# fxxJuses/MICFormer

Measured on AMD Instinct MI355X. Metric: train volumes/sec (128^3 CT+MRI pair), higher is better.
Workload: dtype bf16; 1 GPU; MicFormer base Head(embed_dim=48, depths 2-2-6-2, heads 3-6-12-24, window 2^3, 8 classes) full train step (fwd + MDiceLoss + bwd + Adam/cosine) on 128^3 CT+MR pairs, DropPath on; local_batch=2, global_batch=2, parallelism=dp1, launch=hipGraph replay (one graph)

## Files before the change

include/micformer_hip.h:

```cpp
#ifndef MICFORMER_HIP_H
#define MICFORMER_HIP_H

#include <stddef.h>
#include <stdint.h>

#ifdef __cplusplus
extern "C" {
#endif

typedef void* micf_stream_t;

#define MICF_OK 0
#define MICF_EINVAL (-1)
#define MICF_EUNSUPPORTED (-2)
#define MICF_ELAUNCH (-3)

#define MICF_ABI_VERSION 1

#define MICF_DTYPE_F32 0
#define MICF_DTYPE_BF16 1
#define MICF_DTYPE_BF16_ATTN_FP8 2

int micf_abi_version(void);
const char* micf_strerror(int code);
// ... 137 lines not shown
                            micf_stream_t stream);
int micf_conv_down_bwd_weight(const float* dy, const float* x, float* dw, float* dbias, int B, int D, int H, int W,
                              int C, int N, micf_stream_t stream);
int micf_space_to_depth(const float* x, float* a, int B, int D, int H, int W, int C, int k, int64_t batch_stride,
                        micf_stream_t stream);
int micf_depth_to_space(const float* a, const float* bias, float* y, int B, int D, int H, int W, int C, int k,
                        micf_stream_t stream);
int micf_depth_to_space_add(const float* a, const float* bias, const float* add, float* y, int B, int D, int H, int W, int C,
                            int k, micf_stream_t stream);
int micf_colsum(const float* x, float* out, int64_t M, int N, micf_stream_t stream);
int micf_conv_up_fwd(const float* x, const float* w, const float* bias, float* y, int B, int D, int H, int W, int C,
                     int N, int k, micf_stream_t stream);
int micf_conv_up_bwd_data(const float* dy, const float* w, float* dx, int B, int D, int H, int W, int C, int N, int k,
                          micf_stream_t stream);
int micf_conv_up_bwd_weight(const float* dy, const float* x, float* dw, float* dbias, int B, int D, int H, int W,
                            int C, int N, int k, micf_stream_t stream);

int micf_sw_window(const float* vol, float* win, int C, int D, int H, int W, int rd, int rh, int rw, int z0, int y0, int x0,
                   micf_stream_t stream);
int micf_sw_accumulate(const float* pred, float* out, float* count, int K, int D, int H, int W, int rd, int rh, int rw, int z0,
                       int y0, int x0, micf_stream_t stream);
int micf_sw_normalize(float* out, const float* count, int K, int64_t V, micf_stream_t stream);
int micf_sw_window_batch(const float* vol, float* win, const int32_t* coords, int n, int B, int C, int D, int H, int W, int rd,
                         int rh, int rw, micf_stream_t stream);
int micf_sw_accumulate_batch(const float* pred, float* out, float* count, const int32_t* coords, int n, int B, int K, int D, int H,
                             int W, int rd, int rh, int rw, micf_stream_t stream);

int micf_intensity_stats(const void* vol, int is_half, double* sums, int B, int Cm, int64_t V, micf_stream_t stream);
int micf_patch_rows_prepared(const void* vol, int is_half, const double* sums, const float* params, float* rows0, float* rows1, int B,
                             int Cm, int D, int H, int W, int k, micf_stream_t stream);
int micf_input_prepare(const void* vol, int is_half, const double* sums, const float* params, float* out, const uint8_t* label_in,
                       uint8_t* label_out, int B, int Cm, int D, int H, int W, micf_stream_t stream);

int micf_pad3d(const float* src, float* dst, int B, int D, int H, int W, int Dp, int Hp, int Wp, int C,
               micf_stream_t stream);
int micf_crop3d(const float* src, float* dst, int B, int D, int H, int W, int Dp, int Hp, int Wp, int C,
                int accumulate, micf_stream_t stream);
int micf_resize_trilinear_fwd(const float* src, float* dst, int B, int D, int H, int W, int Do, int Ho, int Wo, int C,
                              micf_stream_t stream);
int micf_resize_trilinear_bwd(const float* ddst, float* dsrc, int B, int D, int H, int W, int Do, int Ho, int Wo,
                              int C, micf_stream_t stream);

int micf_dice_bce_fwd(const float* logits, const float* target, double* sums, float* loss, int B, int K, int64_t V,
                      micf_stream_t stream);
int micf_dice_bce_bwd(const float* logits, const float* target, const double* sums, const float* grad_out,
                      float* dlogits, int B, int K, int64_t V, micf_stream_t stream);
int micf_dice_bce_label_fwd(const float* logits, const uint8_t* label, double* sums, float* loss, int B, int K, int64_t V,
                            micf_stream_t stream);
int micf_dice_bce_label_bwd(const float* logits, const uint8_t* label, const double* sums, const float* grad_out,
                            float* dlogits, int B, int K, int64_t V, micf_stream_t stream);
int micf_argmax_meandice(const float* logits, const uint8_t* label, uint8_t* mask_out, int64_t* counts, double* out,
                         int B, int K, int64_t V, micf_stream_t stream);

int micf_dice_metric(const float* logits, const void* target, int target_is_label, double* sums, float* out, int B, int K,
                     int64_t V, micf_stream_t stream);

int micf_adam_tick(void* state, double base_lr, double eta_min, int64_t t_max, micf_stream_t stream);
int micf_adam_step(float* p, const float* g, float* m, float* v, int64_t n, const void* state, float beta1,
                   float beta2, float eps, float grad_scale, void* p_bf16, micf_stream_t stream);


typedef struct micf_ln_pair_item {
  const float *x, *gamma, *beta;
  float *y, *mean, *rstd;
} micf_ln_pair_item;
typedef struct micf_ln_bwd_pair_item {
  const float *dy, *x, *mean, *rstd, *gamma;
  float *dx, *dgamma, *dbeta;
  const float* add;
  float* partials;
} micf_ln_bwd_pair_item;
int micf_layernorm_fwd_pair(const micf_ln_pair_item* items, int n, int64_t rows, int C, float eps, float* zero,
                            int64_t zero_floats, micf_stream_t stream);
int micf_layernorm_bwd_pair(const micf_ln_bwd_pair_item* items, int n, int64_t rows, int C, micf_stream_t stream);

typedef struct micf_offset_head_group {
  const float* xn;
  const float* xa;
  const float *conv_w, *conv_b;
  float* conv_ws;
  const float *ln_g, *ln_b, *w1;
  float *hid, *flow, *xs;
} micf_offset_head_group;
typedef struct micf_offset_head_bwd_group {
  const float* dxs;
  const float *hid, *flow, *xa, *ln_g, *ln_b, *w1, *conv_w;
  float* conv_ws;
  float* dxa;
  float* dxn;
  float* dhid;
  float *dln_g, *dln_b, *dw1;
} micf_offset_head_bwd_group;
int micf_offset_head_needs_zero(int B, int D, int H, int W, int C);
int micf_offset_head_fwd(const micf_offset_head_group* groups, int ngroups, int B, int D, int H, int W, int C, float eps,
                         int prepared, int hid_zeroed, int dtype, micf_stream_t stream);
int64_t micf_offset_head_bwd_workspace(int ngroups, int B, int D, int H, int W);
int micf_offset_head_bwd(const micf_offset_head_bwd_group* groups, int ngroups, int B, int D, int H, int W, int C, float eps,
                         int prepared, float* workspace, int64_t workspace_floats, int dtype, int defer_finish, micf_stream_t stream);
int micf_offset_head_finish_deferrable(int B, int D, int H, int W);
int micf_offset_head_bwd_finish(const micf_offset_head_bwd_group* groups, int ngroups, int B, int D, int H, int W, int C,
                                float* workspace, int64_t workspace_floats, micf_stream_t stream);
typedef struct micf_offset_head_finish_call {
  const micf_offset_head_bwd_group* groups;
  int32_t ngroups, B, D, H, W, C;
  float* workspace;
  int64_t workspace_floats;
} micf_offset_head_finish_call;
int micf_offset_head_bwd_finish_grouped(const micf_offset_head_finish_call* calls, int ncalls, micf_stream_t stream);

typedef struct micf_block_fwd_group {
  const float* x;
  const float* kvsrc;
  const float *ln1_g, *ln1_b, *bq, *bkv, *bp, *ln2_g, *ln2_b, *b1, *b2;
  const void *wq, *wkv, *wp, *w1, *w2;
  const float *s1, *s2;
  float* y;
  float *xn, *q, *kv, *o, *x1, *xn2;
  void* h;
  float* g;
  float* stats;
  void* kvs16;
  const float* hid;
  const float* samp_src;
  const float *ln16_g, *ln16_b, *w1c;
  float* flow;
  float* xs32;
  const float *nln_g, *nln_b;
  float *nln_y, *nln_mean, *nln_rstd;
  float* zero16;
} micf_block_fwd_group;
int micf_block_fuses_sampler(int C, int heads);
int micf_block_saves_bf16(int C, int heads, int dtype);
typedef struct micf_block_bwd_group {
  const float* dy;
  const float *x, *x1, *stats, *q, *kv;
  const void* h;
  const float *ln1_g, *ln2_g;
  const void *wqt, *wkvt, *wpt, *w1t, *w2t;
  const float *s1, *s2;
  float* dx;
  float* dxs;
  float *dx1, *dh, *dq, *dkv;
  float *ln1_part, *ln2_part;
  float* dx1_copy;
  void* dy16;
  const float* xn2;
  const void* w1;
  const float* b1;
  const float* pre_d;
  const float* pre_x;
  const float *pre_mean, *pre_rstd;
  const float* pre_g;
  float* pre_part;
} micf_block_bwd_group;
int micf_block_recomputes_h(int C, int heads);
int micf_block_tile_tokens(int B, int D, int H, int W, int C, int heads, int hidden, int backward);
int micf_block_fwd_persistent_probe(const micf_block_fwd_group* groups, int ngroups, int B, int D, int H, int W, int C, int heads,
                                    int hidden, float eps, float scale, int dtype, int repeats, int* sync_ws, micf_stream_t stream);
int micf_probe_mfma_chain(const void* a, const void* b, const void* c, const void* d, float* out, int form, micf_stream_t stream);
typedef struct micf_weight_prep_item {
  const float* src;
  void* dst;
  void* dst_t;
  int32_t rows, cols, bf16 , reserved;
} micf_weight_prep_item;
int micf_weight_prep_grouped(const micf_weight_prep_item* items, int n, micf_stream_t stream);
int micf_block_fwd(const micf_block_fwd_group* groups, int ngroups, int B, int D, int H, int W, int C, int heads,
                   int hidden, float eps, float scale, int dtype, micf_stream_t stream);
int micf_block_bwd(const micf_block_bwd_group* groups, int ngroups, int B, int D, int H, int W, int C, int heads,
                   int hidden, float scale, int dtype, micf_stream_t stream);

int micf_zero(void* p, int64_t bytes, micf_stream_t stream);
int micf_drop_path_draw(void* rng, const float* keep, float* out, int n, int B, micf_stream_t stream);


int micf_grad_wire_pack(const float* src, int64_t n, void* dst, int64_t padded, micf_stream_t stream);
int micf_grad_wire_sum(const void* recv, int ranks, int64_t shard, void* out, micf_stream_t stream);
int micf_grad_wire_unpack(const void* src, float* dst, int64_t n, micf_stream_t stream);

#ifdef __cplusplus
}
#endif
#endif
```

micformer_amd/_lib.py:

```python
import ctypes
import os

_PKT = "DEBUG_CLR_GRAPH_PACKET_CAPTURE"
_pkt_before = os.environ.get(_PKT)
if os.environ.get("MICF_SEGMENTED", "0") == "1":
    os.environ.setdefault(_PKT, "0")

import torch

GRAPH_SEGMENTS_OK = os.environ.get(_PKT) == "0" and (_pkt_before == "0" or not torch.cuda.is_initialized())

_HERE = os.path.dirname(os.path.abspath(__file__))
LIB_PATH = os.environ.get("MICF_LIB") or os.path.join(_HERE, "libmicformer_hip.so")

_P, _I, _L, _F, _D = ctypes.c_void_p, ctypes.c_int, ctypes.c_int64, ctypes.c_float, ctypes.c_double
_T = {"p": _P, "i": _I, "l": _L, "f": _F, "d": _D}

SIGNATURES = {
    "micf_layernorm_fwd": "ppippppplifp",
    "micf_layernorm_bwd": "pppippppppplippp",
    "micf_layernorm_bwd_partial_rows": "lii",
    "micf_layernorm_bwd_finish": "pip",
    "micf_linear_fwd": "ppipppplppliiiip",
    "micf_linear_bwd_data": "pplppppiiliiip",
    "micf_linear_bwd_weight": "pplppiippliiplip",
    "micf_linear_bwd_weight_workspace": "lii",
    "micf_linear_bwd_weight_grouped": "piplip",
    "micf_linear_bwd_weight_grouped_workspace": "pi",
    "micf_head_tail_compose": "pppppiiiipp",
    "micf_head_tail_col2im": "pppiiiiiip",
    "micf_head_tail_im2col": "ppiiiiiip",
    "micf_head_tail_col2im_sw": "pppppiiiiiiiiiip",
    "micf_head_tail_decompose": "pppppppppiiiipp",
    "micf_head_tail_fused_supported": "iiiiiii",
    "micf_head_tail_pack_bytes": "ii",
    "micf_head_tail_pack": "pppppiiip",
    "micf_head_tail_fwd_fused": "pppiiiiiiip",
    "micf_head_tail_fwd_fused_sw": "pppppiiiiiiiiiiip",
    "micf_head_tail_loss_parts": "iiii",
    "micf_head_tail_fwd_loss_fused": "ppppipppiiiiiiip",
    "micf_head_tail_bwd_data_fused": "pppiiiiiiip",
    "micf_head_tail_bwd_weight_fused": "pppppliiiiiiip",
    "micf_head_tail_bwd_weight_fused_workspace": "iiiii",
    "micf_sw_window": "ppiiiiiiiiiip",
    "micf_sw_accumulate": "pppiiiiiiiiiip",
    "micf_sw_normalize": "ppilp",
    "micf_window_attn_fwd": "pippipiiiiiiiiiifp",
    "micf_window_attn_fwd_fp8": "pippipiiiiiiiiiifp",
    "micf_window_attn_bwd": "pippipipippiiiiiiiiiifp",
    "micf_conv3_fwd": "pipipppiiiiiipliip",
    "micf_conv3_fwd_workspace": "iii",
    "micf_conv3_bwd_data": "pippiipiiiiiiipliip",
    "micf_conv3_weight_prep_grouped": "pip",
    "micf_layernorm_fwd_pair": "pilifplp",
    "micf_layernorm_bwd_pair": "pilip",
    "micf_offset_head_needs_zero": "iiiii",
    "micf_offset_head_fwd": "piiiiiifiiip",
    "micf_offset_head_bwd_workspace": "iiiii",
    "micf_offset_head_bwd": "piiiiiifipliip",
    "micf_offset_head_finish_deferrable": "iiii",
    "micf_offset_head_bwd_finish": "piiiiiiplp",
    "micf_offset_head_bwd_finish_grouped": "pip",
    "micf_conv3_bwd_data_workspace": "iii",
    "micf_conv3_bwd_weight": "pipipippiiiiiplip",
    "micf_conv3_bwd_weight_workspace": "iiiiiii",
    "micf_conv3_bwd_weight_grouped": "piiiiiiiiplip",
    "micf_conv3_bwd_weight_grouped_workspace": "iiiiiiii",
    "micf_offset_sample_fwd": "pppppppiiiiifp",
    "micf_offset_sample_bwd": "ppppppppppppiiiiifplp",
    "micf_offset_sample_bwd_workspace": "iiii",
    "micf_stn_fwd": "pppiiiiip",
    "micf_stn_bwd": "pppppiiiiip",
    "micf_patch_embed_fwd": "piipppiiiiiip",
    "micf_patch_embed_bwd_weight": "ppiippiiiiiip",
    "micf_conv_down_fwd": "ppppiiiiiip",
    "micf_conv_down_bwd_data": "pppiiiiiip",
    "micf_conv_down_bwd_weight": "ppppiiiiiip",
    "micf_conv_up_fwd": "ppppiiiiiiip",
    "micf_conv_up_bwd_data": "pppiiiiiiip",
    "micf_conv_up_bwd_weight": "ppppiiiiiiip",
    "micf_space_to_depth": "ppiiiiiilp",
    "micf_depth_to_space": "pppiiiiiip",
    "micf_depth_to_space_add": "ppppiiiiiip",
    "micf_colsum": "pplip",
    "micf_pad3d": "ppiiiiiiiip",
    "micf_crop3d": "ppiiiiiiiiip",
    "micf_resize_trilinear_fwd": "ppiiiiiiiip",
    "micf_resize_trilinear_bwd": "ppiiiiiiiip",
    "micf_dice_bce_fwd": "ppppiilp",
    "micf_dice_bce_bwd": "pppppiilp",
    "micf_dice_bce_label_fwd": "ppppiilp",
    "micf_dice_bce_label_bwd": "pppppiilp",
    "micf_argmax_meandice": "pppppiilp",
    "micf_adam_tick": "pddlp",
    "micf_adam_step": "pppplpffffpp",
    "micf_block_tile_tokens": "iiiiiiii",
    "micf_block_saves_bf16": "iii",
    "micf_block_fuses_sampler": "ii",
    "micf_block_recomputes_h": "ii",
    "micf_weight_prep_grouped": "pip",
    "micf_grad_wire_pack": "plplp",
    "micf_grad_wire_sum": "pilpp",
    "micf_grad_wire_unpack": "pplp",
    "micf_block_fwd": "piiiiiiiiffip",
    "micf_block_bwd": "piiiiiiiifip",
    "micf_block_fwd_persistent_probe": "piiiiiiiiffiipp",
    "micf_probe_mfma_chain": "pppppip",
    "micf_dice_metric": "ppippiilp",
    "micf_sw_window_batch": "pppiiiiiiiiip",
    "micf_sw_accumulate_batch": "ppppiiiiiiiiip",
    "micf_intensity_stats": "pipiilp",
    "micf_input_prepare": "pipppppiiiiip",
    "micf_patch_rows_prepared": "pippppiiiiiip",
    "micf_zero": "plp",
    "micf_drop_path_draw": "pppiip",
}


class WgradItem(ctypes.Structure):
    _fields_ = [("a", ctypes.c_void_p), ("dy", ctypes.c_void_p), ("dp_scale", ctypes.c_void_p), ("dw", ctypes.c_void_p),
                ("dbias", ctypes.c_void_p), ("M", ctypes.c_int64), ("rows_per_sample", ctypes.c_int64),
                ("N", ctypes.c_int32), ("K", ctypes.c_int32), ("operand_dtype", ctypes.c_int32), ("ldw", ctypes.c_int32)]


class Conv3WgradItem(ctypes.Structure):
    _fields_ = [("dy", ctypes.c_void_p), ("x1", ctypes.c_void_p), ("x2", ctypes.c_void_p), ("dw", ctypes.c_void_p),
                ("dbias", ctypes.c_void_p)]


class LnFinishItem(ctypes.Structure):
    _fields_ = [("partials", ctypes.c_void_p), ("dgamma", ctypes.c_void_p), ("dbeta", ctypes.c_void_p),
                ("blocks", ctypes.c_int32), ("C", ctypes.c_int32)]


_VP = ctypes.c_void_p


class BlockFwdGroup(ctypes.Structure):
    FIELDS = ("x", "kvsrc", "ln1_g", "ln1_b", "bq", "bkv", "bp", "ln2_g", "ln2_b", "b1", "b2", "wq", "wkv", "wp", "w1", "w2",
              "s1", "s2", "y", "xn", "q", "kv", "o", "x1", "xn2", "h", "g", "stats", "kvs16", "hid", "samp_src", "ln16_g", "ln16_b", "w1c", "flow", "xs32",
              "nln_g", "nln_b", "nln_y", "nln_mean", "nln_rstd", "zero16")
    _fields_ = [(n, _VP) for n in FIELDS]


class BlockBwdGroup(ctypes.Structure):
    FIELDS = ("dy", "x", "x1", "stats", "q", "kv", "h", "ln1_g", "ln2_g", "wqt", "wkvt", "wpt", "w1t", "w2t", "s1", "s2",
              "dx", "dxs", "dx1", "dh", "dq", "dkv", "ln1_part", "ln2_part", "dx1_copy", "dy16", "xn2", "w1", "b1",
              "pre_d", "pre_x", "pre_mean", "pre_rstd", "pre_g", "pre_part")
    _fields_ = [(n, _VP) for n in FIELDS]


class WeightPrepItem(ctypes.Structure):
    _fields_ = [("src", _VP), ("dst", _VP), ("dst_t", _VP), ("rows", ctypes.c_int32), ("cols", ctypes.c_int32),
                ("bf16", ctypes.c_int32), ("reserved", ctypes.c_int32)]


class LnPairItem(ctypes.Structure):
    FIELDS = ("x", "gamma", "beta", "y", "mean", "rstd")
    _fields_ = [(n, _VP) for n in FIELDS]


class LnBwdPairItem(ctypes.Structure):
    FIELDS = ("dy", "x", "mean", "rstd", "gamma", "dx", "dgamma", "dbeta", "add", "partials")
    _fields_ = [(n, _VP) for n in FIELDS]


class OffsetHeadGroup(ctypes.Structure):
    FIELDS = ("xn", "xa", "conv_w", "conv_b", "conv_ws", "ln_g", "ln_b", "w1", "hid", "flow", "xs")
    _fields_ = [(n, _VP) for n in FIELDS]


class OffsetHeadBwdGroup(ctypes.Structure):
    FIELDS = ("dxs", "hid", "flow", "xa", "ln_g", "ln_b", "w1", "conv_w", "conv_ws", "dxa", "dxn", "dhid", "dln_g", "dln_b", "dw1")
    _fields_ = [(n, _VP) for n in FIELDS]


class OffsetHeadFinishCall(ctypes.Structure):
    _fields_ = [("groups", _VP), ("ngroups", ctypes.c_int32), ("B", ctypes.c_int32), ("D", ctypes.c_int32), ("H", ctypes.c_int32),
                ("W", ctypes.c_int32), ("C", ctypes.c_int32), ("workspace", _VP), ("workspace_floats", ctypes.c_int64)]


class Conv3PrepItem(ctypes.Structure):
    _fields_ = [("w", _VP), ("fwd", _VP), ("bwd", _VP), ("N", ctypes.c_int32), ("Cin", ctypes.c_int32)]


class MicfError(RuntimeError):
    pass


def _load():
    if not os.path.exists(LIB_PATH):
        raise ImportError(
            f"{LIB_PATH} not found: build it with `python micformer_amd/build.py` (hipcc, gfx950). "
            "micformer_amd has no CPU / PyTorch fallback path.")
    lib = ctypes.CDLL(LIB_PATH)
    for name, sig in SIGNATURES.items():
        fn = getattr(lib, name)
        fn.argtypes = [_T[c] for c in sig]
        fn.restype = _I
    lib.micf_linear_bwd_weight_workspace.restype = _L
    lib.micf_linear_bwd_weight_grouped_workspace.restype = _L
    lib.micf_conv3_bwd_data_workspace.restype = _L
    lib.micf_offset_sample_bwd_workspace.restype = _L
    lib.micf_conv3_bwd_weight_workspace.restype = _L
    lib.micf_conv3_bwd_weight_grouped_workspace.restype = _L
    lib.micf_head_tail_pack_bytes.restype = _L
    lib.micf_head_tail_loss_parts.restype = _L
    lib.micf_head_tail_loss_parts.argtypes = [_I] * 4
    lib.micf_head_tail_bwd_weight_fused_workspace.restype = _L
    lib.micf_conv3_fwd_workspace.restype = _L
    lib.micf_offset_head_bwd_workspace.restype = _L
    lib.micf_block_tile_tokens.argtypes = [_I] * 8
    lib.micf_block_saves_bf16.argtypes = [_I] * 3
    lib.micf_offset_head_finish_deferrable.argtypes = [_I] * 4
    lib.micf_block_fuses_sampler.argtypes = [_I] * 2
    lib.micf_block_recomputes_h.argtypes = [_I] * 2
    lib.micf_strerror.argtypes = [_I]
    lib.micf_strerror.restype = ctypes.c_char_p
    lib.micf_set_option.argtypes = [ctypes.c_char_p, _I]
    lib.micf_set_option.restype = _I
    lib.micf_get_option.argtypes = [ctypes.c_char_p, ctypes.POINTER(_I)]
    lib.micf_get_option.restype = _I
    lib.micf_abi_version.argtypes = []
    lib.micf_abi_version.restype = _I
    if lib.micf_abi_version() != 1:
        raise ImportError("libmicformer_hip.so ABI version mismatch")
    return lib


lib = _load()


def get_option(name):
    v = _I(0)
    if lib.micf_get_option(name.encode(), ctypes.byref(v)) != 0:
        raise KeyError(f"unknown micformer option {name!r}")
    return v.value


def set_option(name, value):
    prev = get_option(name)
    if lib.micf_set_option(name.encode(), int(value)) != 0:
        raise KeyError(f"unknown micformer option {name!r}")
    return prev


class option:

    def __init__(self, name, value):
        self.name, self.value = name, value

    def __enter__(self):
        self.prev = set_option(self.name, self.value)

    def __exit__(self, *exc):
        set_option(self.name, self.prev)
        return False


def ptr(t):
    if t is None:
        return None
    if not t.is_cuda:
        raise MicfError("micformer_amd ops need CUDA (ROCm) tensors: there is no CPU path")
    if not t.is_contiguous():
        raise MicfError("micformer_amd ops need contiguous tensors")
    return t.data_ptr()


_raw_stream = getattr(torch._C, "_cuda_getCurrentRawStream", None)
_cur_device = getattr(torch._C, "_cuda_getDevice", None)


def stream():
    if _raw_stream is not None and _cur_device is not None:
        return _raw_stream(_cur_device())
    return torch.cuda.current_stream().cuda_stream


PROFILE = None
BLOCK_DEPTH = 0
UNIT = None


def set_unit(kind, groups, tokens, channels):
    global UNIT
    if PROFILE is not None:
        UNIT = f"{kind}|{groups}x{tokens}x{channels}"


class block_region:

    def __enter__(self):
        global BLOCK_DEPTH
        BLOCK_DEPTH += 1

    def __exit__(self, *exc):
        global BLOCK_DEPTH, UNIT
        BLOCK_DEPTH -= 1
        if BLOCK_DEPTH == 0:
            UNIT = None
# ... 58 lines not shown
```

micformer_amd/csrc/block_bwd.hip:

```cpp
#include "block_fused.h"
#include "attn_fp8.h"

namespace micf {

struct BlkBwdArgs {
  micf_block_bwd_group g[2];
  TileGeo geo;
  int G, tiles, C, heads, hidden;
  float scale;
  int attn_mfma;
};

template <int TM, int NW, int X4>
struct RowRegs {
  static constexpr int RPP = 4 * NW, NPASS = (TM + RPP - 1) / RPP, K = (X4 + 15) / 16;
  float4 v[NPASS][K];
  template <class Addr>
  __device__ __forceinline__ void load(const int* tok, int tk0, const Addr addr) {
    const int lane = threadIdx.x & 63, wave = threadIdx.x >> 6, l16 = lane & 15, rg = lane >> 4;
#pragma unroll
    for (int pass = 0; pass < NPASS; ++pass) {
      const int row = pass * RPP + wave * 4 + rg;
      const int tk = row < TM ? tok[row] : -1;
#pragma unroll
      for (int k = 0; k < K; ++k) {
        const int c4 = l16 + 16 * k;
        const bool ok = tk >= 0 && c4 < X4;
        const float4 t = ld4g(addr(tk >= 0 ? (uint32_t)(tk - tk0) : 0u, (uint32_t)(c4 < X4 ? c4 : X4 - 1)));
        v[pass][k] = ok ? t : make_float4(0.f, 0.f, 0.f, 0.f);
      }
    }
  }
  __device__ __forceinline__ void commit(float* dst, int stride) const {
    const int lane = threadIdx.x & 63, wave = threadIdx.x >> 6, l16 = lane & 15, rg = lane >> 4;
#pragma unroll
    for (int pass = 0; pass < NPASS; ++pass) {
      const int row = pass * RPP + wave * 4 + rg;
      if (row >= TM) continue;
#pragma unroll
      for (int k = 0; k < K; ++k) {
        const int c4 = l16 + 16 * k;
        if (c4 < X4) *reinterpret_cast<float4*>(dst + row * stride + 4 * c4) = v[pass][k];
      }
    }
  }
  __device__ __forceinline__ void store_b16(const int* tok, int tk0, void* base) const {
    const int lane = threadIdx.x & 63, wave = threadIdx.x >> 6, l16 = lane & 15, rg = lane >> 4;
#pragma unroll
    for (int pass = 0; pass < NPASS; ++pass) {
      const int row = pass * RPP + wave * 4 + rg;
      const int tk = row < TM ? tok[row] : -1;
      if (tk < 0) continue;
#pragma unroll
      for (int k = 0; k < K; ++k) {
        const int c4 = l16 + 16 * k;
        if (c4 < X4) st_h4_32<true>(base, (uint32_t)(tk - tk0) * (4 * X4) + 4 * c4, v[pass][k]);
      }
    }
  }
};
template <int TM, int NW, int X4, bool BF16>
struct HRegs {
  static constexpr int RPP = 4 * NW, NPASS = (TM + RPP - 1) / RPP, K = (X4 + 15) / 16, ES = BF16 ? 2 : 4;
  using V = typename std::conditional<BF16, uint2, float4>::type;
  V v[NPASS][K];
  __device__ __forceinline__ void load(const int* tok, int tk0, const char* base, uint32_t ld) {
    const int lane = threadIdx.x & 63, wave = threadIdx.x >> 6, l16 = lane & 15, rg = lane >> 4;
#pragma unroll
    for (int pass = 0; pass < NPASS; ++pass) {
      const int row = pass * RPP + wave * 4 + rg;
      const int tk = row < TM ? tok[row] : -1;
      const uint32_t rel = tk >= 0 ? (uint32_t)(tk - tk0) : 0u;
#pragma unroll
      for (int k = 0; k < K; ++k) {
        const int c4 = l16 + 16 * k;
        const bool ok = tk >= 0 && c4 < X4;
        const V t = *reinterpret_cast<const V*>(base + (rel * ld + 4u * (uint32_t)(c4 < X4 ? c4 : X4 - 1)) * (uint32_t)ES);
        v[pass][k] = ok ? t : V{};
      }
    }
  }
  __device__ __forceinline__ void commit(float* dst, int stride) const {
    const int lane = threadIdx.x & 63, wave = threadIdx.x >> 6, l16 = lane & 15, rg = lane >> 4;
#pragma unroll
    for (int pass = 0; pass < NPASS; ++pass) {
      const int row = pass * RPP + wave * 4 + rg;
      if (row >= TM) continue;
#pragma unroll
      for (int k = 0; k < K; ++k) {
        const int c4 = l16 + 16 * k;
        if (c4 >= X4) continue;
        float4 f;
        if constexpr (BF16) f = unpack4_bf16(v[pass][k]); else f = v[pass][k];
        *reinterpret_cast<float4*>(dst + row * stride + 4 * c4) = f;
      }
    }
  }
};
template <int TM, int NW, int C>
struct LnRegs {
  RowRegs<TM, NW, C / 4> x;
  float mu[RowRegs<TM, NW, C / 4>::NPASS], rs[RowRegs<TM, NW, C / 4>::NPASS];
  float4 gm[(C + 63) / 64];
  __device__ __forceinline__ void load(const int* tok, int tk0, const float* __restrict__ xsrc, const float* __restrict__ mean,
                                       const float* __restrict__ rstd, const float* __restrict__ gamma) {
    constexpr int RPP = 4 * NW, NPASS = RowRegs<TM, NW, C / 4>::NPASS;
    const int lane = threadIdx.x & 63, wave = threadIdx.x >> 6, l16 = lane & 15, rg = lane >> 4;
    x.load(tok, tk0, [&](uint32_t rel, uint32_t c4) { return at32(xsrc, (rel * C + 4 * c4) * 4u); });
#pragma unroll
    for (int pass = 0; pass < NPASS; ++pass) {
      const int row = pass * RPP + wave * 4 + rg;
      const int tk = row < TM ? tok[row] : -1;
      const uint32_t rel = tk >= 0 ? (uint32_t)(tk - tk0) : 0u;
      const float m = *at32(mean, rel * 4u), r = *at32(rstd, rel * 4u);
      mu[pass] = tk >= 0 ? m : 0.f; rs[pass] = tk >= 0 ? r : 0.f;
    }
#pragma unroll
    for (int k = 0; k < (C + 63) / 64; ++k) {
      const int c4 = l16 + 16 * k;
      const float4 t = ld4g(gamma + 4 * (c4 < C / 4 ? c4 : C / 4 - 1));
      gm[k] = c4 < C / 4 ? t : make_float4(0.f, 0.f, 0.f, 0.f);
    }
  }
  __device__ __forceinline__ void park(float* stash) const {
    constexpr int NPASS = RowRegs<TM, NW, C / 4>::NPASS;
    x.commit(stash, C);
    float* mine = stash + TM * C + threadIdx.x;
#pragma unroll
    for (int pass = 0; pass < NPASS; ++pass) { mine[(2 * pass) * 64 * NW] = mu[pass]; mine[(2 * pass + 1) * 64 * NW] = rs[pass]; }
  }
  __device__ __forceinline__ void unpark(const float* stash, const float* __restrict__ gamma) {
    constexpr int RPP = 4 * NW, NPASS = RowRegs<TM, NW, C / 4>::NPASS, K = RowRegs<TM, NW, C / 4>::K;
    const int lane = threadIdx.x & 63, wave = threadIdx.x >> 6, l16 = lane & 15, rg = lane >> 4;
    const float* mine = stash + TM * C + threadIdx.x;
#pragma unroll
    for (int pass = 0; pass < NPASS; ++pass) {
      const int row = pass * RPP + wave * 4 + rg;
      mu[pass] = mine[(2 * pass) * 64 * NW]; rs[pass] = mine[(2 * pass + 1) * 64 * NW];
#pragma unroll
      for (int k = 0; k < K; ++k) {
        const int c4 = l16 + 16 * k;
        x.v[pass][k] = (row < TM && c4 < C / 4) ? *reinterpret_cast<const float4*>(stash + row * C + 4 * c4) : make_float4(0.f, 0.f, 0.f, 0.f);
      }
    }
#pragma unroll
    for (int k = 0; k < (C + 63) / 64; ++k) {
      const int c4 = l16 + 16 * k;
      const float4 t = ld4g(gamma + 4 * (c4 < C / 4 ? c4 : C / 4 - 1));
      gm[k] = c4 < C / 4 ? t : make_float4(0.f, 0.f, 0.f, 0.f);
    }
  }
};

template <int TJ, int VPL, int NW, int C, bool H16 = false>
__device__ __forceinline__ void ln_bwd_tile(const float* D, float* A, int S, const LnRegs<16 * TJ, NW, C>& in, const int* tok,
                                            int tk0, void* __restrict__ hout, float* __restrict__ hout2, float* scratch,
                                            float* __restrict__ part) {
  constexpr int TM = 16 * TJ, NTHR = 64 * NW, RPP = 4 * NW, NPASS = (TM + RPP - 1) / RPP, NPR = RPP < TM ? RPP : TM;
  const int tid = threadIdx.x, lane = tid & 63, wave = tid >> 6, l16 = lane & 15, rg = lane >> 4;
  constexpr int C4 = C >> 2;
  const float invC = 1.0f / (float)C;
  float4 ag[VPL], ab[VPL], gm[VPL];
#pragma unroll
// ... 302 lines not shown
          const float ds = p[j] * (dp[j] - dot);
          if (j / (8 / SP) == sub) {
            PS[pair * 16 + j] = p[j];
            PS[pair * 16 + 8 + j] = ds;
          }
          const float* kp = U + (r0 + j) * SU + C + hoff;
          const float dss = ds * a.scale;
#pragma unroll
          for (int d = 0; d < HP; d += 4) {
            const float4 t = *reinterpret_cast<const float4*>(kp + d);
            dq[d] += dss * t.x; dq[d + 1] += dss * t.y; dq[d + 2] += dss * t.z; dq[d + 3] += dss * t.w;
          }
        }
      }
      lds_barrier();
      if (active) {
#pragma unroll
        for (int d = 0; d < HP; ++d) { dk[d] = 0.f; dv[d] = 0.f; }
        const int base = pair - i * heads;
#pragma unroll
        for (int m = 0; m < 8; ++m) {
          const float pm = PS[(base + m * heads) * 16 + i];
          const float dsm = PS[(base + m * heads) * 16 + 8 + i] * a.scale;
          const float* qp = U + (r0 + m) * SU + hoff;
          const float* dop = A2 + (r0 + m) * S + hoff;
#pragma unroll
          for (int d = 0; d < HP; d += 4) {
            const float4 t = *reinterpret_cast<const float4*>(qp + d);
            dk[d] += dsm * t.x; dk[d + 1] += dsm * t.y; dk[d + 2] += dsm * t.z; dk[d + 3] += dsm * t.w;
            const float4 u = *reinterpret_cast<const float4*>(dop + d);
            dv[d] += pm * u.x; dv[d + 1] += pm * u.y; dv[d + 2] += pm * u.z; dv[d + 3] += pm * u.w;
          }
        }
      }
      lds_barrier();
      if (active) {
#pragma unroll
        for (int d = 0; d < HP; d += 4) {
          *reinterpret_cast<float4*>(U + row * SU + hoff + d) = make_float4(dq[d], dq[d + 1], dq[d + 2], dq[d + 3]);
          *reinterpret_cast<float4*>(U + row * SU + C + hoff + d) = make_float4(dk[d], dk[d + 1], dk[d + 2], dk[d + 3]);
          *reinterpret_cast<float4*>(U + row * SU + 2 * C + hoff + d) = make_float4(dv[d], dv[d + 1], dv[d + 2], dv[d + 3]);
        }
      }
      lds_barrier();
    }
  }

#pragma unroll 1
  for (int pass = 0; pass < NPASS; ++pass) {
    const int row = pass * RPP + wave * 4 + rg;
    if (row >= TM) continue;
    const int tk = tok[row];
    if (tk < 0) continue;
    const uint32_t rel = (uint32_t)(tk - tk0);
    for (int c4 = l16; c4 < 3 * C4; c4 += 16) {
      const float4 v = *reinterpret_cast<const float4*>(U + row * SU + 4 * c4);
      if (c4 < C4) st_h4_32<BF16>(dq0, rel * C + 4 * c4, v);
      else st_h4_32<BF16>(dkv0, rel * 2 * C + 4 * (c4 - C4), v);
    }
  }

  if (!g.dxs) {
    if (PARK) r_ln1.unpark(stash, g.ln1_g);
    gemm_phase<TJ, NSLK, NKK, C, NW, BF16>(wqt, C, U, nullptr, 0, nullptr, SU, A2, S, EpiStore{});
    gemm_phase<TJ, NSLK, 2 * NKK, 2 * C, NW, BF16>(wkvt, C, U + C, nullptr, 0, nullptr, SU, A2, S, EpiAcc{});
    ln_bwd_tile<TJ, VPL, NW, C>(A2, A1, S, r_ln1, tok, tk0, dx0, nullptr, U, g.ln1_part ? g.ln1_part + (int64_t)tile * 2 * C : nullptr);
  } else {
    gemm_phase<TJ, NSLK, NKK, C, NW, BF16>(wqt, C, U, nullptr, 0, nullptr, SU, A2, S, EpiStore{});
#pragma unroll 1
    for (int pass = 0; pass < NPASS; ++pass) {
      const int row = pass * RPP + wave * 4 + rg;
      if (row >= TM) continue;
      const int tk = tok[row];
      if (tk < 0) continue;
      for (int c4 = l16; c4 < C4; c4 += 16)
        st4g(at32(dx0, ((uint32_t)(tk - tk0) * C + 4 * c4) * 4u), *reinterpret_cast<const float4*>(A2 + row * S + 4 * c4));
    }
    lds_barrier();
    gemm_phase<TJ, NSLK, 2 * NKK, 2 * C, NW, BF16>(wkvt, C, U + C, nullptr, 0, nullptr, SU, A2, S, EpiStore{});
#pragma unroll 1
    for (int pass = 0; pass < NPASS; ++pass) {
      const int row = pass * RPP + wave * 4 + rg;
      if (row >= TM) continue;
      const int tk = tok[row];
      if (tk < 0) continue;
      for (int c4 = l16; c4 < C4; c4 += 16)
        st4g(at32(g.dxs + (int64_t)tk0 * C, ((uint32_t)(tk - tk0) * C + 4 * c4) * 4u), *reinterpret_cast<const float4*>(A2 + row * S + 4 * c4));
    }
  }
}

template <int C, int HD, int TJ>
static int launch_bwd(const BlkBwdArgs& a, int dtype, hipStream_t s) {
  constexpr int TM = 16 * TJ, NW = C >= 192 ? 8 : 4;
  const bool recomp = a.g[0].h == nullptr;
  const size_t lds = block_lds_floats(TM, C, block_bwd_scratch_floats(TM, C / HD, 64 * NW),
                                      block_bwd_park_floats(TM, C, 64 * NW) + (recomp ? 4 * C : 0)) * sizeof(float);
  if (lds > 160 * 1024) return MICF_EUNSUPPORTED;
  const unsigned grid = a.G == 2 ? (unsigned)((a.tiles + 3) / 4 * 8) : (unsigned)a.tiles;
  static std::once_flag once;
  std::call_once(once, [] {
    (void)hipFuncSetAttribute(reinterpret_cast<const void*>(&block_bwd_kernel<C, HD, TJ, NW, true, false>), hipFuncAttributeMaxDynamicSharedMemorySize, 160 * 1024);
    (void)hipFuncSetAttribute(reinterpret_cast<const void*>(&block_bwd_kernel<C, HD, TJ, NW, false, false>), hipFuncAttributeMaxDynamicSharedMemorySize, 160 * 1024);
    (void)hipFuncSetAttribute(reinterpret_cast<const void*>(&block_bwd_kernel<C, HD, TJ, NW, true, true>), hipFuncAttributeMaxDynamicSharedMemorySize, 160 * 1024);
    (void)hipFuncSetAttribute(reinterpret_cast<const void*>(&block_bwd_kernel<C, HD, TJ, NW, false, true>), hipFuncAttributeMaxDynamicSharedMemorySize, 160 * 1024);
  });
  if (dtype == MICF_DTYPE_BF16) {
    if (recomp) hipLaunchKernelGGL((block_bwd_kernel<C, HD, TJ, NW, true, true>), dim3(grid), dim3(64 * NW), lds, s, a);
    else hipLaunchKernelGGL((block_bwd_kernel<C, HD, TJ, NW, true, false>), dim3(grid), dim3(64 * NW), lds, s, a);
  } else {
    if (recomp) hipLaunchKernelGGL((block_bwd_kernel<C, HD, TJ, NW, false, true>), dim3(grid), dim3(64 * NW), lds, s, a);
    else hipLaunchKernelGGL((block_bwd_kernel<C, HD, TJ, NW, false, false>), dim3(grid), dim3(64 * NW), lds, s, a);
  }
  MICF_RETURN_LAUNCH();
}

}

#include "block_wave_bwd.h"

using namespace micf;

extern "C" int micf_block_bwd(const micf_block_bwd_group* groups, int ngroups, int B, int D, int H, int W, int C, int heads,
                              int hidden, float scale, int dtype, micf_stream_t stream) {
  if (!groups || ngroups < 1 || ngroups > 2) return MICF_EINVAL;
  const int TM = micf_block_tile_tokens(B, D, H, W, C, heads, hidden, 1);
  if (TM == 0) return MICF_EUNSUPPORTED;
  if (dtype != MICF_DTYPE_F32 && dtype != MICF_DTYPE_BF16) return MICF_EINVAL;
  BlkBwdArgs a;
  for (int i = 0; i < ngroups; ++i) {
    const micf_block_bwd_group& g = groups[i];
    const void* need[] = {g.dy, g.x1, g.stats, g.q, g.kv, g.ln2_g, g.wqt, g.wkvt, g.wpt, g.w1t, g.w2t, g.dx, g.dx1, g.dh, g.dq, g.dkv};
    for (const void* p : need)
      if (!p || (reinterpret_cast<uintptr_t>(p) & 15)) return MICF_EINVAL;
    if (g.h) {
      if (reinterpret_cast<uintptr_t>(g.h) & 15) return MICF_EINVAL;
    } else {
      const void* re[] = {g.xn2, g.w1, g.b1};
      for (const void* p : re)
        if (!p || (reinterpret_cast<uintptr_t>(p) & 15)) return MICF_EINVAL;
      if (!micf_block_recomputes_h(C, heads)) return MICF_EINVAL;
    }
    if (i > 0 && (g.h == nullptr) != (groups[0].h == nullptr)) return MICF_EINVAL;
    if (g.pre_d) {
      const void* pr[] = {g.pre_d, g.pre_x, g.pre_mean, g.pre_rstd, g.pre_g, g.pre_part, g.dy16};
      for (const void* p : pr)
        if (!p || (reinterpret_cast<uintptr_t>(p) & 15)) return MICF_EINVAL;
      if (g.dxs || dtype != MICF_DTYPE_BF16 || block_wide_tile_tokens(C, C / heads)) return MICF_EINVAL;
    }
    if (!g.dxs && (!g.x || !g.ln1_g)) return MICF_EINVAL;
    const void* opt[] = {g.x, g.ln1_g, g.dxs, g.ln1_part, g.ln2_part, g.dx1_copy, g.dy16};
    for (const void* p : opt)
      if (p && (reinterpret_cast<uintptr_t>(p) & 15)) return MICF_EINVAL;
    a.g[i] = g;
  }
  if (ngroups == 1) a.g[1] = a.g[0];
  a.geo = make_tile_geo(B, D, H, W);
  a.G = ngroups; a.C = C; a.heads = heads; a.hidden = hidden; a.scale = scale;
  a.tiles = (a.geo.nwin + TM / 8 - 1) / (TM / 8);
  a.attn_mfma = dtype == MICF_DTYPE_BF16 ? 1 : 0;
  hipStream_t s = (hipStream_t)stream;
  const int hd = C / heads, tj = TM / 16;
  if ((int64_t)2 * H * W * (TM / 8 + 1) * hidden * (int64_t)sizeof(float) >= (int64_t)1 << 32) return MICF_EUNSUPPORTED;
  if (block_wide_tile_tokens(C, hd)) return block_bwd_wide(groups, ngroups, B, D, H, W, C, heads, scale, dtype, s);
  {
    if (options().block_wave != 0 && C == 48 && hd == 16 && tj == 2 && dtype == MICF_DTYPE_BF16 && a.attn_mfma && a.g[0].h && a.g[1].h && (a.g[0].dxs != nullptr) == (a.g[1].dxs != nullptr) &&
        (a.g[0].pre_d != nullptr) == (a.g[1].pre_d != nullptr) && !(a.g[0].dxs && a.g[0].pre_d) &&
        a.geo.T * (int64_t)hidden * 2 < ((int64_t)1 << 31))
    {
      if (options().block_debug & 1) a.attn_mfma |= 2;
      return wave48::launch_bwd_wave48(a, s);
    }
  }
#define MICF_BB(C_, HD_, TJ_) if (C == C_ && hd == HD_ && tj == TJ_) return launch_bwd<C_, HD_, TJ_>(a, dtype, s)
  MICF_BB(48, 16, 2); MICF_BB(96, 16, 2); MICF_BB(192, 16, 1);
  MICF_BB(96, 32, 1); MICF_BB(192, 32, 1); MICF_BB(384, 32, 1);
#undef MICF_BB
  return MICF_EUNSUPPORTED;
}
```

micformer_amd/csrc/block_wave_bwd.h:

```cpp
#pragma once

#include "block_wave.h"

namespace micf {
namespace wave48 {

constexpr int kB2 = 0;
constexpr int kB2h = kB2 + 12 * 1024;
constexpr int kB1 = kB2h + 12 * 512;
constexpr int kBP = kB1 + 18 * 1024;
constexpr int kBPh = kBP + 3 * 1024;
constexpr int kBQ = kBPh + 3 * 512;
constexpr int kBKV = kBQ + 9 * 512;
constexpr int kBVec = kBKV + 18 * 512;
constexpr int kBPark = kBVec + 3 * C * 4;
constexpr int kParkFloats = 4 * (16 * 12 + 8);
constexpr int kBwdLdsBytes = kBPark + NWAVE * kParkFloats * 4;

__device__ __forceinline__ void stage_weights_bwd(char* lds, const micf_block_bwd_group& g) {
  const uint16_t* wqt = static_cast<const uint16_t*>(g.wqt), *wkvt = static_cast<const uint16_t*>(g.wkvt), *wpt = static_cast<const uint16_t*>(g.wpt),
                 *w1t = static_cast<const uint16_t*>(g.w1t), *w2t = static_cast<const uint16_t*>(g.w2t);
  const int tid = threadIdx.x;
  for (int s = tid; s < 12 * 64; s += NTHR) {
    const int j = s >> 6, li = s & 15, lr = (s >> 4) & 3, row = row_p192(j, li);
    *reinterpret_cast<u32x4v*>(lds + kB2 + s * 16) = *reinterpret_cast<const u32x4v*>(w2t + k16(row, 8 * lr, 3));
    *reinterpret_cast<u32x2v*>(lds + kB2h + s * 8) = *reinterpret_cast<const u32x2v*>(w2t + k16(row, 32 + 4 * lr, 3));
  }
  for (int s = tid; s < 18 * 64; s += NTHR) {
    const int f = s >> 6, j = f / 6, kc = f - 6 * j, li = s & 15, lr = (s >> 4) & 3;
    *reinterpret_cast<u32x4v*>(lds + kB1 + s * 16) = *reinterpret_cast<const u32x4v*>(w1t + k16(row_p48(j, li), 32 * kc + 8 * lr, 12));
  }
  for (int s = tid; s < 3 * 64; s += NTHR) {
    const int j = s >> 6, li = s & 15, lr = (s >> 4) & 3, row = 16 * j + li;
    *reinterpret_cast<u32x4v*>(lds + kBP + s * 16) = *reinterpret_cast<const u32x4v*>(wpt + k16(row, 8 * lr, 3));
    *reinterpret_cast<u32x2v*>(lds + kBPh + s * 8) = *reinterpret_cast<const u32x2v*>(wpt + k16(row, 32 + 4 * lr, 3));
  }
  for (int s = tid; s < 9 * 64; s += NTHR) {
    const int f = s >> 6, j = f / 3, h = f - 3 * j, li = s & 15, lr = (s >> 4) & 3;
    *reinterpret_cast<u32x2v*>(lds + kBQ + s * 8) = *reinterpret_cast<const u32x2v*>(wqt + k16(row_p48(j, li), 16 * h + 4 * lr, 3));
  }
  for (int s = tid; s < 18 * 64; s += NTHR) {
    const int f = s >> 6, j = f / 6, h = f - 6 * j, li = s & 15, lr = (s >> 4) & 3;
    *reinterpret_cast<u32x2v*>(lds + kBKV + s * 8) = *reinterpret_cast<const u32x2v*>(wkvt + k16(row_p48(j, li), 16 * h + 4 * lr, 6));
  }
  float* PV = reinterpret_cast<float*>(lds + kBVec);
  for (int e = tid; e < 3 * C; e += NTHR) {
    const float* src = e < C ? g.ln1_g : (e < 2 * C ? g.ln2_g : g.pre_g);
    PV[e] = src ? src[e % C] : 0.f;
  }
}

__device__ __forceinline__ void park12(float* tile, int lr, int li, const float (&v)[12]) {
  float* p = tile + lr * 200 + li * 12;
  *reinterpret_cast<float4*>(p) = make_float4(v[0], v[1], v[2], v[3]);
  *reinterpret_cast<float4*>(p + 4) = make_float4(v[4], v[5], v[6], v[7]);
  *reinterpret_cast<float4*>(p + 8) = make_float4(v[8], v[9], v[10], v[11]);
}
__device__ __forceinline__ void unpark12(const float* tile, int lr, int li, float (&v)[12]) {
  const float* p = tile + lr * 200 + li * 12;
  const float4 a = *reinterpret_cast<const float4*>(p), b = *reinterpret_cast<const float4*>(p + 4), c = *reinterpret_cast<const float4*>(p + 8);
  v[0] = a.x; v[1] = a.y; v[2] = a.z; v[3] = a.w; v[4] = b.x; v[5] = b.y; v[6] = b.z; v[7] = b.w; v[8] = c.x; v[9] = c.y; v[10] = c.z; v[11] = c.w;
}
__device__ __forceinline__ float colsum16(const float* tile, int lane) {
  const int c = lane < 48 ? lane : 0;
  const float* p = tile + (c < 32 ? (c >> 3) * 200 + (c & 7) : ((c - 32) >> 2) * 200 + 8 + (c & 3));
  float s0 = 0.f, s1 = 0.f;
#pragma unroll
  for (int t = 0; t < 16; t += 2) { s0 += p[12 * t]; s1 += p[12 * t + 12]; }
  return s0 + s1;
}

__device__ __forceinline__ void ln_bwd12(const float (&d)[12], const Row12& xin, float mu, float rs, const float* gam, int lr, int li,
                                         int lane, float* tile, const Row12& add, Row12& out, float& pg, float& pb) {
  float gm[12], dxh[12];
  vec12(gam, lr, gm);
  float sa = 0.f, sb = 0.f;
#pragma unroll
  for (int e = 0; e < 12; e += 4) {
    float g4[4], xh[4];
#pragma unroll
    for (int r = 0; r < 4; ++r) { xh[r] = (xin.v[e + r] - mu) * rs; g4[r] = gm[e + r] * d[e + r]; dxh[e + r] = d[e + r] * xh[r]; }
    sa += (g4[0] + g4[1]) + (g4[2] + g4[3]);
    sb += (g4[0] * xh[0] + g4[1] * xh[1]) + (g4[2] * xh[2] + g4[3] * xh[3]);
  }
  const float Am = sum4(sa) * (1.0f / C), Bm = sum4(sb) * (1.0f / C);
  park12(tile, lr, li, dxh);
#pragma unroll
  for (int e = 0; e < 12; ++e) out.v[e] = add.v[e] + rs * (gm[e] * d[e] - Am - ((xin.v[e] - mu) * rs) * Bm);
  pg += colsum16(tile, lane);
  asm volatile("" : "+v"(pg));
  park12(tile, lr, li, d);
  pb += colsum16(tile, lane);
  asm volatile("" : "+v"(pb));
}

__device__ __forceinline__ void unpack8(const u32x4v& u, float (&o)[8]) {
#pragma unroll
  for (int w = 0; w < 4; ++w) { o[2 * w] = __uint_as_float(u[w] << 16); o[2 * w + 1] = __uint_as_float(u[w] & 0xFFFF0000u); }
}

template <bool CROSS, bool PRE>
__global__ void __launch_bounds__(NTHR) __attribute__((amdgpu_waves_per_eu(4, 4))) block_bwd_wave48_kernel(const BlkBwdArgs a) {
  extern __shared__ __attribute__((aligned(1024))) char wlds[];
  const unsigned bid = blockIdx.x;
  int grp, wg, nwg;
  if (a.G == 2) { const int xcd = bid & 7; grp = xcd >> 2; wg = (int)(bid >> 3) * 4 + (xcd & 3); nwg = (int)(gridDim.x >> 3) * 4; }
  else { grp = 0; wg = bid; nwg = gridDim.x; }
  const micf_block_bwd_group& g = a.g[grp];
  stage_weights_bwd(wlds, g);
  const int tid = threadIdx.x, lane0 = tid & 63, wave = __builtin_amdgcn_readfirstlane(tid >> 6);
  const float* PV = reinterpret_cast<const float*>(wlds + kBVec);
  const float *p_ln1g = PV, *p_ln2g = PV + C, *p_preg = PV + 2 * C;
  const uint32_t T = (uint32_t)a.geo.T;
  const int ngroup16 = (a.geo.nwin + 1) >> 1;
  constexpr bool cross = CROSS, pre = PRE;
  const f32x4 z4 = {0.f, 0.f, 0.f, 0.f};
  lds_barrier();

  for (int unit = wg * NWAVE + wave; unit < a.tiles; unit += nwg * NWAVE) {
    float pg_pre = 0.f, pb_pre = 0.f, pg2 = 0.f, pb2 = 0.f, pg1 = 0.f, pb1 = 0.f;
#pragma unroll 1
    for (int sub = 0; sub < 2; ++sub) {
      const int gt = 2 * unit + sub;
      if (gt >= ngroup16) break;
      asm volatile("" ::: "memory");
      int lane = lane0;
      asm volatile("" : "+v"(lane));
      const int li = lane & 15, lr = lane >> 4;
      const bf16x4_t ident = pack4_bf16v(4 * lr == li ? 1.f : 0.f, 4 * lr + 1 == li ? 1.f : 0.f, 4 * lr + 2 == li ? 1.f : 0.f, 4 * lr + 3 == li ? 1.f : 0.f);
      const bool valid = (lr >> 1) == (li >> 3);
      float* tile = reinterpret_cast<float*>(wlds + kBPark) + wave * kParkFloats;
      const int win = 2 * gt + (li >> 3);
      const bool live0 = win < a.geo.nwin, live = live0 && !(a.attn_mfma & 2);
      int b = 0, d_ = 0, hh = 0, w = 0;
      a.geo.coords(live0 ? win : 0, li & 7, b, d_, hh, w);
      const uint32_t tk = (uint32_t)(((b * a.geo.D + d_) * a.geo.H + hh) * a.geo.W + w);
      const float s1v = g.s1 ? g.s1[b] : 1.f, s2v = g.s2 ? g.s2[b] : 1.f;
      const uint32_t rowC = tk * C;

      Row12 dy;
      dy.load(at32(g.dy, rowC * 4u), lr);
      if (!live) dy.zero();
      if (pre) {
        Row12 pd, px;
        pd.load(at32(g.pre_d, rowC * 4u), lr);
        px.load(at32(g.pre_x, rowC * 4u), lr);
        float pm = *at32(g.pre_mean, tk * 4u), pr = *at32(g.pre_rstd, tk * 4u);
        if (!live) { pd.zero(); px.zero(); pm = 0.f; pr = 0.f; }
        Row12 t;
        ln_bwd12(pd.v, px, pm, pr, p_preg, lr, li, lane, tile, dy, t, pg_pre, pb_pre);
        dy = t;
        if (!live) dy.zero();
      }
      const bf16x8 dyA = dy.lo();
      const bf16x4_t dyB = dy.hi();
      park12(tile, lr, li, dy.v);
      u32x4v hreg[6];
      {
        const uint16_t* hp = static_cast<const uint16_t*>(g.h);
#pragma unroll
        for (int c = 0; c < 6; ++c) {
          hreg[c] = *reinterpret_cast<const u32x4v*>(at32(hp, (tk * HID + 32 * c + 8 * lr) * 2u));
          if (!live) hreg[c] = u32x4v{0u, 0u, 0u, 0u};
        }
      }

      f32x4 dn2[3] = {z4, z4, z4};
      bf16x8 dhs[6];
      {
#pragma unroll
        for (int c = 0; c < 6; ++c) {
          float h8[8];
          unpack8(hreg[c], h8);
          float4 dv[2];
#pragma unroll
          for (int u = 0; u < 2; ++u) {
            const int j = 2 * c + u;
            const f32x4 acc = mfma48(frag32(wlds, kB2, j, lane), frag16(wlds, kB2h, j, lane), dyA, dyB);
            dv[u] = make_float4(s2v * acc[0] * gelu_grad_t<true>(h8[4 * u]), s2v * acc[1] * gelu_grad_t<true>(h8[4 * u + 1]),
                                s2v * acc[2] * gelu_grad_t<true>(h8[4 * u + 2]), s2v * acc[3] * gelu_grad_t<true>(h8[4 * u + 3]));
          }
          dhs[c] = to_bf16x8(dv[0], dv[1]);
#pragma unroll
          for (int j = 0; j < 3; ++j) dn2[j] = mfma32(frag32(wlds, kB1, 6 * j + c, lane), dhs[c], dn2[j]);
          __builtin_amdgcn_sched_barrier(0);
        }
      }
      const uint16_t* qp = reinterpret_cast<const uint16_t*>(g.q);
      const uint16_t* kp = reinterpret_cast<const uint16_t*>(g.kv);
      bf16x4_t qn, kn, vn;
      auto load_head = [&](int h) {
        qn = *reinterpret_cast<const bf16x4_t*>(at32(qp, (rowC + 16 * h + 4 * lr) * 2u));
        kn = *reinterpret_cast<const bf16x4_t*>(at32(kp, (2 * rowC + 16 * h + 4 * lr) * 2u));
        vn = *reinterpret_cast<const bf16x4_t*>(at32(kp, (2 * rowC + C + 16 * h + 4 * lr) * 2u));
        if (!live) { qn = bf16x4_t{0, 0, 0, 0}; kn = qn; vn = qn; }
      };
      load_head(0);
      Row12 x1;
      x1.load(at32(g.x1, rowC * 4u), lr);
      float mu2 = *at32(g.stats, (2 * T + tk) * 4u), rs2 = *at32(g.stats, (3 * T + tk) * 4u);
      if (!live) { x1.zero(); mu2 = 0.f; rs2 = 0.f; }
      Row12 x;
      float mu1 = 0.f, rs1 = 0.f;

      asm volatile("" ::: "memory");
      if (live) {
        if (g.dy16) {
          uint16_t* o = static_cast<uint16_t*>(g.dy16);
          st4u(at32(o, (rowC + 8 * lr) * 2u), dyA); st2u(at32(o, (rowC + 32 + 4 * lr) * 2u), dyB);
        }
        uint16_t* dho = reinterpret_cast<uint16_t*>(g.dh);
#pragma unroll
        for (int c = 0; c < 6; ++c) st4u(at32(dho, (tk * HID + 32 * c + 8 * lr) * 2u), dhs[c]);
      }

      __builtin_amdgcn_sched_barrier(0);
      Row12 dx1;
      {
        float d[12];
#pragma unroll
        for (int j = 0; j < 3; ++j)
#pragma unroll
          for (int r = 0; r < 4; ++r) d[4 * j + r] = dn2[j][r];
        Row12 dyp;
        unpark12(tile, lr, li, dyp.v);
        ln_bwd12(d, x1, mu2, rs2, p_ln2g, lr, li, lane, tile, dyp, dx1, pg2, pb2);
        if (!live) dx1.zero();
      }
      const bf16x8 d1A = dx1.lo();
      const bf16x4_t d1B = dx1.hi();
      if (live) {
        uint16_t* o = reinterpret_cast<uint16_t*>(g.dx1);
        st4u(at32(o, (rowC + 8 * lr) * 2u), d1A); st2u(at32(o, (rowC + 32 + 4 * lr) * 2u), d1B);
        if (g.dx1_copy) dx1.store(at32(g.dx1_copy, rowC * 4u), lr);
      }

      bf16x4_t dqf[3], dkf[3], dvf[3];
      {
        uint16_t* dqo = reinterpret_cast<uint16_t*>(g.dq);
        uint16_t* dko = reinterpret_cast<uint16_t*>(g.dkv);
#pragma unroll
        for (int h = 0; h < 3; ++h) {
          const bf16x4_t qcur = qn, kf = kn, vf = vn;
          if (h < 2) load_head(h + 1);
          else if (!cross) {
            x.load(at32(g.x, rowC * 4u), lr);
            mu1 = *at32(g.stats, tk * 4u); rs1 = *at32(g.stats, (T + tk) * 4u);
            if (!live) { x.zero(); mu1 = 0.f; rs1 = 0.f; }
          }
          const f32x4 dacc = mfma48(frag32(wlds, kBP, h, lane), frag16(wlds, kBPh, h, lane), d1A, d1B);
          const bf16x4_t of = pack4_bf16v(s1v * dacc[0], s1v * dacc[1], s1v * dacc[2], s1v * dacc[3]);
          const uint2 qu = __builtin_bit_cast(uint2, qcur);
          const bf16x4_t qf = pack4_bf16v(__uint_as_float(qu.x << 16) * a.scale, __uint_as_float(qu.x & 0xFFFF0000u) * a.scale,
                                          __uint_as_float(qu.y << 16) * a.scale, __uint_as_float(qu.y & 0xFFFF0000u) * a.scale);
          const f32x4 s1 = mfma16(kf, qf, z4);
          const f32x4 p1 = mfma16(vf, of, z4);
          const f32x4 s2 = mfma16(qf, kf, z4);
          const f32x4 p2 = mfma16(of, vf, z4);
          float m = valid ? fmaxf(fmaxf(s1[0], s1[1]), fmaxf(s1[2], s1[3])) : -INFINITY;
          m = fmaxf(m, __shfl_xor(m, 16, 64));
          float e[4];
#pragma unroll
          for (int r = 0; r < 4; ++r) e[r] = valid ? expf(s1[r] - m) : 0.f;
          float sum = (e[0] + e[1]) + (e[2] + e[3]);
          sum += __shfl_xor(sum, 16, 64);
          const float inv = valid ? 1.0f / sum : 0.f;
          float dot = 0.f;
#pragma unroll
          for (int r = 0; r < 4; ++r) { e[r] *= inv; dot += valid ? e[r] * p1[r] : 0.f; }
          dot += __shfl_xor(dot, 16, 64);
          float ds1[4];
#pragma unroll
          for (int r = 0; r < 4; ++r) ds1[r] = valid ? e[r] * (p1[r] - dot) : 0.f;
          const bf16x4_t dsf1 = pack4_bf16v(ds1[0], ds1[1], ds1[2], ds1[3]);
          float e2[4], ds2[4];
#pragma unroll
          for (int r = 0; r < 4; ++r) {
            const int qi = 4 * lr + r, src = qi + 16 * (2 * (qi >> 3));
            const float mq = __shfl(m, src, 64), iq = __shfl(inv, src, 64), dq_ = __shfl(dot, src, 64);
            e2[r] = valid ? expf(s2[r] - mq) * iq : 0.f;
            ds2[r] = valid ? e2[r] * (p2[r] - dq_) : 0.f;
          }
          const bf16x4_t pf2 = pack4_bf16v(e2[0], e2[1], e2[2], e2[3]);
          const bf16x4_t dsf2 = pack4_bf16v(ds2[0], ds2[1], ds2[2], ds2[3]);
          const bf16x4_t kt = pack4q(mfma16(kf, ident, z4)), qt = pack4q(mfma16(qf, ident, z4)), ot = pack4q(mfma16(of, ident, z4));
          const f32x4 ga = mfma16(kt, dsf1, z4);
          const f32x4 gb = mfma16(qt, dsf2, z4);
          const f32x4 gc = mfma16(ot, pf2, z4);
          dqf[h] = pack4_bf16v(ga[0] * a.scale, ga[1] * a.scale, ga[2] * a.scale, ga[3] * a.scale);
          dkf[h] = pack4q(gb);
          dvf[h] = pack4q(gc);
          if (live) {
            st2u(at32(dqo, (rowC + 16 * h + 4 * lr) * 2u), dqf[h]);
            st2u(at32(dko, (2 * rowC + 16 * h + 4 * lr) * 2u), dkf[h]);
            st2u(at32(dko, (2 * rowC + C + 16 * h + 4 * lr) * 2u), dvf[h]);
          }
          __builtin_amdgcn_sched_barrier(0);
        }
      }

      __builtin_amdgcn_sched_barrier(0);
      if (!cross) {
        float d[12];
#pragma unroll
        for (int j = 0; j < 3; ++j) {
          f32x4 acc = z4;
#pragma unroll
          for (int h = 0; h < 3; ++h) acc = mfma16(frag16(wlds, kBQ, 3 * j + h, lane), dqf[h], acc);
#pragma unroll
          for (int h = 0; h < 6; ++h) acc = mfma16(frag16(wlds, kBKV, 6 * j + h, lane), h < 3 ? dkf[h] : dvf[h - 3], acc);
#pragma unroll
          for (int r = 0; r < 4; ++r) d[4 * j + r] = acc[r];
        }
        Row12 dx;
        ln_bwd12(d, x, mu1, rs1, p_ln1g, lr, li, lane, tile, dx1, dx, pg1, pb1);
        if (live) dx.store(at32(g.dx, rowC * 4u), lr);
      } else {
        Row12 dxq, dxs;
#pragma unroll
        for (int j = 0; j < 3; ++j) {
          f32x4 acc = z4, acs = z4;
#pragma unroll
          for (int h = 0; h < 3; ++h) acc = mfma16(frag16(wlds, kBQ, 3 * j + h, lane), dqf[h], acc);
#pragma unroll
          for (int h = 0; h < 6; ++h) acs = mfma16(frag16(wlds, kBKV, 6 * j + h, lane), h < 3 ? dkf[h] : dvf[h - 3], acs);
#pragma unroll
          for (int r = 0; r < 4; ++r) { dxq.v[4 * j + r] = acc[r]; dxs.v[4 * j + r] = acs[r]; }
        }
        if (live) {
          dxq.store(at32(g.dx, rowC * 4u), lr);
          dxs.store(at32(g.dxs, rowC * 4u), lr);
        }
      }
    }
    if (lane0 < C) {
      const int64_t row = (int64_t)unit * 2 * C;
      if (g.ln2_part) { g.ln2_part[row + lane0] = pg2; g.ln2_part[row + C + lane0] = pb2; }
      if (!cross && g.ln1_part) { g.ln1_part[row + lane0] = pg1; g.ln1_part[row + C + lane0] = pb1; }
      if (pre) { g.pre_part[row + lane0] = pg_pre; g.pre_part[row + C + lane0] = pb_pre; }
    }
  }
}

static int launch_bwd_wave48(const BlkBwdArgs& a, hipStream_t s) {
  int nwg = (a.tiles + NWAVE - 1) / NWAVE;
  if (nwg > 256) nwg = 256;
  const unsigned grid = a.G == 2 ? (unsigned)((nwg + 3) / 4 * 8) : (unsigned)nwg;
  static std::once_flag once;
  std::call_once(once, [] {
    (void)hipFuncSetAttribute(reinterpret_cast<const void*>(&block_bwd_wave48_kernel<true, false>), hipFuncAttributeMaxDynamicSharedMemorySize, 160 * 1024);
    (void)hipFuncSetAttribute(reinterpret_cast<const void*>(&block_bwd_wave48_kernel<false, true>), hipFuncAttributeMaxDynamicSharedMemorySize, 160 * 1024);
    (void)hipFuncSetAttribute(reinterpret_cast<const void*>(&block_bwd_wave48_kernel<false, false>), hipFuncAttributeMaxDynamicSharedMemorySize, 160 * 1024);
  });
  const bool cross = a.g[0].dxs != nullptr, pre = a.g[0].pre_d != nullptr;
  if (cross) hipLaunchKernelGGL((block_bwd_wave48_kernel<true, false>), dim3(grid), dim3(NTHR), kBwdLdsBytes, s, a);
  else if (pre) hipLaunchKernelGGL((block_bwd_wave48_kernel<false, true>), dim3(grid), dim3(NTHR), kBwdLdsBytes, s, a);
  else hipLaunchKernelGGL((block_bwd_wave48_kernel<false, false>), dim3(grid), dim3(NTHR), kBwdLdsBytes, s, a);
  MICF_RETURN_LAUNCH();
}

}
}
```

micformer_amd/csrc/common.h:

```cpp
#pragma once
#include <hip/hip_runtime.h>
#include <stdint.h>

#include "../../include/micformer_hip.h"
#include "gemm_core.h"

#define MICF_RETURN_LAUNCH()                          \
  do {                                                \
    return hipGetLastError() == hipSuccess ? MICF_OK : MICF_ELAUNCH; \
  } while (0)

namespace micf {

struct Options {
  int block_wave = 1;
  int block_recompute_h = 0;
  int block_debug = 0;
  int sample_tile = 1;
  int sample_e = -1;
  int cell_cap = -1;
  int tile_cap_hits = -1, tile_cap_cell = -1, tile_cap_voxel = -1;
};
Options& options();

struct Geo {
  int B, D, H, W;
  FastDiv fW, fH, fD;
  Geo() {}
  Geo(int B_, int D_, int H_, int W_) : B(B_), D(D_), H(H_), W(W_), fW((uint32_t)W_), fH((uint32_t)H_), fD((uint32_t)D_) {}
  __host__ __device__ int64_t tokens() const { return (int64_t)B * D * H * W; }
  __device__ __forceinline__ void decode(int t, int& b, int& d, int& h, int& w) const {
    uint32_t q, r;
    fW.divmod((uint32_t)t, q, r); w = (int)r;
    fH.divmod(q, q, r); h = (int)r;
    fD.divmod(q, q, r); d = (int)r; b = (int)q;
  }
  __device__ __forceinline__ int token(int b, int d, int h, int w) const { return ((b * D + d) * H + h) * W + w; }
};

__device__ __forceinline__ float wave_sum(float v) {
#pragma unroll
  for (int o = 32; o > 0; o >>= 1) v += __shfl_xor(v, o, 64);
  return v;
}

int colsum_atomic(const float* dy, const float* scale, int64_t rps, float* out, int64_t M, int N, hipStream_t s);

constexpr int kOffsetHidden = 16;
struct CellLists {
  int* count;
  int* ovf_count;
  int* list;
  int* ovf;
  int cap;
  float* w8;
};
struct SampleFwdSet { const float *h, *ln_g, *ln_b, *w1, *xa; float *flow, *xs; };
struct SampleBwdSet {
  const float *dxs, *h, *ln_g, *ln_b, *w1, *xa, *flow;
  float *dxa, *dh, *dln_g, *dln_b, *dw1;
  CellLists cl;
  float* partials;
};
int offset_sample_fwd_groups(const SampleFwdSet* sets, int n, int B, int D, int H, int W, int C, float eps, hipStream_t stream);
int offset_sample_bwd_groups(SampleBwdSet* sets, int n, int B, int D, int H, int W, int C, float eps, float* workspace,
                             int64_t workspace_floats, hipStream_t s, int phase = 0);
struct SampleFinishCall { const SampleBwdSet* sets; int n, B, D, H, W, C; float* workspace; int64_t workspace_floats; };
int offset_sample_finish_many(const SampleFinishCall* calls, int ncalls, hipStream_t s);

struct Conv3FwdSet { const float* x1; const float* x2; const float* w; const float* bias; float* y; float* wt; };
struct Conv3BwdSet { const float* dy; const float* w; float* wt; float* dx1; float* dx2; };
int conv3_fwd_x_groups(const Conv3FwdSet* sets, int n, int c1, int c2, int B, int D, int H, int W, int N, hipStream_t stream, int dtype,
                       int prepared, int y_zeroed);
bool conv3_fwd_x_splits(int B, int D, int H, int W, int c1, int c2);
int conv3_bwd_data_x_groups(const Conv3BwdSet* sets, int ng, int c1, int acc1, int c2, int acc2, int B, int D, int H, int W, int N,
                            hipStream_t stream, int dtype, int prepared);

int conv3_bwd_data_x(const float* dy, const float* w, float* wt, float* dx1, int c1, int acc1, float* dx2, int c2, int acc2, int B,
                     int D, int H, int W, int N, hipStream_t stream, int dtype = 0, int prepared = 0);

int64_t conv3_fwdx_workspace(int N, int c1, int c2);
int conv3_fwd_x(const float* x1, int c1, const float* x2, int c2, const float* w, const float* bias, float* y, float* wt, int B, int D,
                int H, int W, int N, hipStream_t stream, int dtype = 0, int prepared = 0);
int64_t conv3_wgradx_workspace(int B, int D, int H, int W, int N, int c1, int c2, int items = 1);
int conv3_wgradx_items(const float* const* dy, const float* const* x1, const float* const* x2, float* const* dw, float* const* dbias,
                       int n, int c1, int c2, int B, int D, int H, int W, int N, float* ws, int64_t ws_floats, hipStream_t stream,
                       int dtype);
int conv3_wgradx(const float* dy, const float* x1, int c1, const float* x2, int c2, float* dw, float* dbias, int B, int D, int H,
                 int W, int N, float* ws, int64_t ws_floats, hipStream_t stream, int dtype = 0);

}
```

micformer_amd/csrc/misc.hip:

```cpp
#include <hip/hip_fp16.h>

#include "common.h"
#include <string.h>

namespace micf {

__global__ void __launch_bounds__(256) pad3d_kernel(const float* __restrict__ src, float* __restrict__ dst, int B, int D, int H,
                                                    int W, int Dp, int Hp, int Wp, int C, int64_t total) {
  for (int64_t i = (int64_t)blockIdx.x * 256 + threadIdx.x; i < total; i += (int64_t)gridDim.x * 256) {
    int64_t t = i / C; const int c = (int)(i - t * C);
    const int w = (int)(t % Wp); t /= Wp; const int h = (int)(t % Hp); t /= Hp; const int d = (int)(t % Dp); const int b = (int)(t / Dp);
    dst[i] = (d < D && h < H && w < W) ? src[((((int64_t)b * D + d) * H + h) * W + w) * C + c] : 0.f;
  }
}
__global__ void __launch_bounds__(256) crop3d_kernel(const float* __restrict__ src, float* __restrict__ dst, int B, int D, int H,
                                                     int W, int Dp, int Hp, int Wp, int C, int accumulate, int64_t total) {
  for (int64_t i = (int64_t)blockIdx.x * 256 + threadIdx.x; i < total; i += (int64_t)gridDim.x * 256) {
    int64_t t = i / C; const int c = (int)(i - t * C);
    const int w = (int)(t % W); t /= W; const int h = (int)(t % H); t /= H; const int d = (int)(t % D); const int b = (int)(t / D);
    const float v = src[((((int64_t)b * Dp + d) * Hp + h) * Wp + w) * C + c];
    dst[i] = accumulate ? dst[i] + v : v;
  }
}

__device__ __forceinline__ void ac_coord(int o, int Sin, int Sout, int& i0, int& i1, float& f) {
  const float scale = Sout > 1 ? (float)(Sin - 1) / (float)(Sout - 1) : 0.f;
  const float s = scale * (float)o;
  i0 = (int)s; if (i0 > Sin - 1) i0 = Sin - 1;
  i1 = i0 + (i0 < Sin - 1 ? 1 : 0);
  f = s - (float)i0;
}
template <bool BWD>
__global__ void __launch_bounds__(256) resize_kernel(const float* __restrict__ a, float* __restrict__ o, int B, int D, int H, int W,
                                                     int Do, int Ho, int Wo, int C, int64_t total) {
  for (int64_t i = (int64_t)blockIdx.x * 256 + threadIdx.x; i < total; i += (int64_t)gridDim.x * 256) {
    int64_t t = i / C; const int c = (int)(i - t * C);
    const int w = (int)(t % Wo); t /= Wo; const int h = (int)(t % Ho); t /= Ho; const int d = (int)(t % Do); const int b = (int)(t / Do);
    int d0, d1, h0, h1, w0, w1; float fd, fh, fw;
    ac_coord(d, D, Do, d0, d1, fd); ac_coord(h, H, Ho, h0, h1, fh); ac_coord(w, W, Wo, w0, w1, fw);
    float acc = 0.f;
    const float gv = BWD ? a[i] : 0.f;
#pragma unroll
    for (int q = 0; q < 8; ++q) {
      const int dd = (q & 4) ? d1 : d0, hh = (q & 2) ? h1 : h0, ww = (q & 1) ? w1 : w0;
      const float wt = ((q & 4) ? fd : 1.f - fd) * ((q & 2) ? fh : 1.f - fh) * ((q & 1) ? fw : 1.f - fw);
      const int64_t s = ((((int64_t)b * D + dd) * H + hh) * W + ww) * C + c;
      if (BWD) atomicAdd(o + s, wt * gv); else acc += wt * a[s];
    }
    if (!BWD) o[i] = acc;
  }
}


__global__ void __launch_bounds__(256) sw_window_kernel(const float* __restrict__ vol, float* __restrict__ win, int C, int D, int H,
                                                        int W, int rd, int rh, int rw, int z0, int y0, int x0, int64_t total) {
  for (int64_t i = (int64_t)blockIdx.x * 256 + threadIdx.x; i < total; i += (int64_t)gridDim.x * 256) {
    const int x = (int)(i % rw); int64_t r = i / rw;
    const int y = (int)(r % rh); r /= rh;
    const int z = (int)(r % rd); const int c = (int)(r / rd);
    win[i] = vol[(((int64_t)c * D + z0 + z) * H + y0 + y) * W + x0 + x];
  }
}
__global__ void __launch_bounds__(256) sw_accumulate_kernel(const float* __restrict__ pred, float* __restrict__ out,
                                                            float* __restrict__ count, int K, int D, int H, int W, int rd, int rh,
                                                            int rw, int z0, int y0, int x0, int64_t total) {
  for (int64_t i = (int64_t)blockIdx.x * 256 + threadIdx.x; i < total; i += (int64_t)gridDim.x * 256) {
    const int x = (int)(i % rw); int64_t r = i / rw;
    const int y = (int)(r % rh); r /= rh;
    const int z = (int)(r % rd); const int k = (int)(r / rd);
    const int64_t v = ((int64_t)(z0 + z) * H + y0 + y) * W + x0 + x;
    out[(int64_t)k * D * H * W + v] += pred[i];
    if (k == 0) count[v] += 1.f;
  }
}
__global__ void __launch_bounds__(256) sw_normalize_kernel(float* __restrict__ out, const float* __restrict__ count, int64_t V,
                                                           int64_t total) {
  for (int64_t i = (int64_t)blockIdx.x * 256 + threadIdx.x; i < total; i += (int64_t)gridDim.x * 256) out[i] /= count[i % V];
}

}
using namespace micf;

extern "C" int micf_abi_version(void) { return MICF_ABI_VERSION; }

micf::Options& micf::options() {
  static Options o;
  return o;
}

static int* option_slot(const char* name) {
  if (!name) return nullptr;
  Options& o = micf::options();
  const struct { const char* n; int* v; } table[] = {
      {"block_wave", &o.block_wave}, {"block_recompute_h", &o.block_recompute_h}, {"block_debug", &o.block_debug},
      {"sample_tile", &o.sample_tile}, {"sample_e", &o.sample_e}, {"cell_cap", &o.cell_cap},
      {"tile_cap_hits", &o.tile_cap_hits}, {"tile_cap_cell", &o.tile_cap_cell}, {"tile_cap_voxel", &o.tile_cap_voxel}};
  for (const auto& e : table)
    if (!strcmp(name, e.n)) return e.v;
  return nullptr;
}

extern "C" int micf_set_option(const char* name, int value) {
  int* slot = option_slot(name);
  if (!slot) return MICF_EINVAL;
  *slot = value;
  return MICF_OK;
}

extern "C" int micf_get_option(const char* name, int* value) {
  const int* slot = option_slot(name);
  if (!slot || !value) return MICF_EINVAL;
  *value = *slot;
  return MICF_OK;
}

extern "C" const char* micf_strerror(int code) {
  switch (code) {
    case MICF_OK: return "ok";
    case MICF_EINVAL: return "invalid argument (null pointer, bad size or misaligned buffer)";
    case MICF_EUNSUPPORTED: return "shape not supported by the HIP kernels";
    case MICF_ELAUNCH: return "HIP kernel launch failed";
    default: return "unknown micf error code";
  }
}

static int grid_for(int64_t total) { int64_t b = (total + 255) / 256; return (int)(b > 16384 ? 16384 : (b < 1 ? 1 : b)); }

extern "C" int micf_pad3d(const float* src, float* dst, int B, int D, int H, int W, int Dp, int Hp, int Wp, int C,
                          micf_stream_t stream) {
  if (!src || !dst || B <= 0 || D <= 0 || H <= 0 || W <= 0 || C <= 0 || Dp < D || Hp < H || Wp < W) return MICF_EINVAL;
  const int64_t total = (int64_t)B * Dp * Hp * Wp * C;
  hipLaunchKernelGGL(pad3d_kernel, dim3(grid_for(total)), dim3(256), 0, (hipStream_t)stream, src, dst, B, D, H, W, Dp, Hp, Wp, C, total);
  MICF_RETURN_LAUNCH();
}
extern "C" int micf_crop3d(const float* src, float* dst, int B, int D, int H, int W, int Dp, int Hp, int Wp, int C, int accumulate,
                           micf_stream_t stream) {
  if (!src || !dst || B <= 0 || D <= 0 || H <= 0 || W <= 0 || C <= 0 || Dp < D || Hp < H || Wp < W) return MICF_EINVAL;
  const int64_t total = (int64_t)B * D * H * W * C;
  hipLaunchKernelGGL(crop3d_kernel, dim3(grid_for(total)), dim3(256), 0, (hipStream_t)stream, src, dst, B, D, H, W, Dp, Hp, Wp, C,
                     accumulate, total);
  MICF_RETURN_LAUNCH();
}
extern "C" int micf_resize_trilinear_fwd(const float* src, float* dst, int B, int D, int H, int W, int Do, int Ho, int Wo, int C,
                                         micf_stream_t stream) {
  if (!src || !dst || B <= 0 || D <= 0 || H <= 0 || W <= 0 || Do <= 0 || Ho <= 0 || Wo <= 0 || C <= 0) return MICF_EINVAL;
  const int64_t total = (int64_t)B * Do * Ho * Wo * C;
  hipLaunchKernelGGL(resize_kernel<false>, dim3(grid_for(total)), dim3(256), 0, (hipStream_t)stream, src, dst, B, D, H, W, Do, Ho, Wo, C, total);
  MICF_RETURN_LAUNCH();
}
extern "C" int micf_resize_trilinear_bwd(const float* ddst, float* dsrc, int B, int D, int H, int W, int Do, int Ho, int Wo, int C,
                                         micf_stream_t stream) {
  if (!ddst || !dsrc || B <= 0 || D <= 0 || H <= 0 || W <= 0 || Do <= 0 || Ho <= 0 || Wo <= 0 || C <= 0) return MICF_EINVAL;
  hipStream_t s = (hipStream_t)stream;
  if (hipMemsetAsync(dsrc, 0, sizeof(float) * (size_t)B * D * H * W * C, s) != hipSuccess) return MICF_ELAUNCH;
  const int64_t total = (int64_t)B * Do * Ho * Wo * C;
  hipLaunchKernelGGL(resize_kernel<true>, dim3(grid_for(total)), dim3(256), 0, s, ddst, dsrc, B, D, H, W, Do, Ho, Wo, C, total);
  MICF_RETURN_LAUNCH();
}

extern "C" int micf_sw_window(const float* vol, float* win, int C, int D, int H, int W, int rd, int rh, int rw, int z0, int y0,
                              int x0, micf_stream_t stream) {
  if (!vol || !win || C <= 0 || rd <= 0 || rh <= 0 || rw <= 0 || z0 < 0 || y0 < 0 || x0 < 0 || z0 + rd > D || y0 + rh > H ||
      x0 + rw > W)
    return MICF_EINVAL;
  const int64_t total = (int64_t)C * rd * rh * rw;
  hipLaunchKernelGGL(sw_window_kernel, dim3(grid_for(total)), dim3(256), 0, (hipStream_t)stream, vol, win, C, D, H, W, rd, rh, rw, z0,
                     y0, x0, total);
  MICF_RETURN_LAUNCH();
}
extern "C" int micf_sw_accumulate(const float* pred, float* out, float* count, int K, int D, int H, int W, int rd, int rh, int rw,
                                  int z0, int y0, int x0, micf_stream_t stream) {
  if (!pred || !out || !count || K <= 0 || rd <= 0 || rh <= 0 || rw <= 0 || z0 < 0 || y0 < 0 || x0 < 0 || z0 + rd > D ||
      y0 + rh > H || x0 + rw > W)
    return MICF_EINVAL;
  const int64_t total = (int64_t)K * rd * rh * rw;
  hipLaunchKernelGGL(sw_accumulate_kernel, dim3(grid_for(total)), dim3(256), 0, (hipStream_t)stream, pred, out, count, K, D, H, W, rd,
                     rh, rw, z0, y0, x0, total);
  MICF_RETURN_LAUNCH();
}
extern "C" int micf_sw_normalize(float* out, const float* count, int K, int64_t V, micf_stream_t stream) {
  if (!out || !count || K <= 0 || V <= 0) return MICF_EINVAL;
  const int64_t total = (int64_t)K * V;
  hipLaunchKernelGGL(sw_normalize_kernel, dim3(grid_for(total)), dim3(256), 0, (hipStream_t)stream, out, count, V, total);
  MICF_RETURN_LAUNCH();
}

extern "C" int micf_zero(void* p, int64_t bytes, micf_stream_t stream) {
  if (!p || bytes < 0) return MICF_EINVAL;
  if (bytes == 0) return MICF_OK;
  return hipMemsetAsync(p, 0, (size_t)bytes, (hipStream_t)stream) == hipSuccess ? MICF_OK : MICF_ELAUNCH;
}

namespace micf {
__device__ __forceinline__ uint64_t mix64(uint64_t z) {
  z += 0x9E3779B97F4A7C15ull;
  z = (z ^ (z >> 30)) * 0xBF58476D1CE4E5B9ull;
  z = (z ^ (z >> 27)) * 0x94D049BB133111EBull;
  return z ^ (z >> 31);
}
__global__ void __launch_bounds__(256) drop_path_draw_kernel(uint64_t* __restrict__ rng, const float* __restrict__ keep,
                                                             float* __restrict__ out, int n, int B) {
  const uint64_t seed = rng[0], ctr = rng[1];
  for (int e = threadIdx.x; e < n * B; e += 256) {
    const float k = keep[e / B];
    const uint64_t h = mix64(mix64(seed ^ mix64(ctr)) + (uint64_t)e);
    const float u = (float)(h >> 40) * (1.0f / 16777216.0f);
    out[e] = (u < k) ? 1.0f / k : 0.0f;
  }
  __syncthreads();
  if (threadIdx.x == 0) rng[1] = ctr + 1;
}
}

extern "C" int micf_drop_path_draw(void* rng, const float* keep, float* out, int n, int B, micf_stream_t stream) {
  if (!rng || !keep || !out || n < 0 || B <= 0) return MICF_EINVAL;
  if (n == 0) return MICF_OK;
  hipLaunchKernelGGL(micf::drop_path_draw_kernel, dim3(1), dim3(256), 0, (hipStream_t)stream, static_cast<uint64_t*>(rng), keep, out, n, B);
  MICF_RETURN_LAUNCH();
}

namespace micf {
constexpr int kPrepMax = 64;
struct PrepArgs {
  int n;
  int end[kPrepMax];
  const float* src[kPrepMax]; void* dst[kPrepMax]; void* dst_t[kPrepMax];
  int rows[kPrepMax], cols[kPrepMax], bf16[kPrepMax];
};
__device__ __forceinline__ unsigned pack_bf16(float a, float b) {
  typedef __bf16 bf16x2_hw __attribute__((ext_vector_type(2)));
  typedef float f32x2_hw __attribute__((ext_vector_type(2)));
  const f32x2_hw f = {a, b};
  return __builtin_bit_cast(unsigned, __builtin_convertvector(f, bf16x2_hw));
}
__device__ __forceinline__ void prep_store4(void* base, int64_t idx, bool bf16, bool vec, int valid, float4 v) {
  if (bf16) {
    uint16_t* d = static_cast<uint16_t*>(base) + idx;
    if (vec) { *reinterpret_cast<uint2*>(d) = make_uint2(pack_bf16(v.x, v.y), pack_bf16(v.z, v.w)); return; }
    const float e[4] = {v.x, v.y, v.z, v.w};
    for (int i = 0; i < valid; ++i) d[i] = (uint16_t)(pack_bf16(e[i], 0.f) & 0xFFFFu);
  } else {
    float* d = static_cast<float*>(base) + idx;
    if (vec) { *reinterpret_cast<float4*>(d) = v; return; }
    const float e[4] = {v.x, v.y, v.z, v.w};
    for (int i = 0; i < valid; ++i) d[i] = e[i];
  }
}
// ... 260 lines not shown
```

micformer_amd/csrc/offset_head.hip:

```cpp
#include "common.h"

using namespace micf;

extern "C" int micf_offset_head_needs_zero(int B, int D, int H, int W, int C) {
  if (B <= 0 || D <= 0 || H <= 0 || W <= 0 || C <= 0 || (C & 3) || W < 4) return 0;
  return conv3_fwd_x_splits(B, D, H, W, C, C) ? 1 : 0;
}

extern "C" int micf_offset_head_fwd(const micf_offset_head_group* groups, int ngroups, int B, int D, int H, int W, int C, float eps,
                                    int prepared, int hid_zeroed, int dtype, micf_stream_t stream) {
  if (!groups || ngroups < 1 || ngroups > 2 || B <= 0 || D <= 0 || H <= 0 || W <= 0 || C <= 0) return MICF_EINVAL;
  if (dtype != MICF_DTYPE_F32 && dtype != MICF_DTYPE_BF16) return MICF_EINVAL;
  hipStream_t s = (hipStream_t)stream;
  Conv3FwdSet cs[2];
  SampleFwdSet ss[2];
  bool conv_only = true;
  for (int i = 0; i < ngroups; ++i) {
    const micf_offset_head_group& g = groups[i];
    if (!g.xn || !g.xa || !g.conv_w || !g.hid) return MICF_EINVAL;
    conv_only = conv_only && !g.flow && !g.xs;
    if (!conv_only && (!g.ln_g || !g.ln_b || !g.w1 || !g.flow || !g.xs)) return MICF_EINVAL;
    cs[i] = Conv3FwdSet{g.xn, g.xa, g.conv_w, g.conv_b, g.hid, g.conv_ws};
    ss[i] = SampleFwdSet{g.hid, g.ln_g, g.ln_b, g.w1, g.xa, g.flow, g.xs};
  }
  int rc = MICF_EUNSUPPORTED;
  if (groups[0].conv_ws && (ngroups == 1 || groups[1].conv_ws))
    rc = conv3_fwd_x_groups(cs, ngroups, C, C, B, D, H, W, kOffsetHidden, s, dtype, prepared, hid_zeroed);
  if (rc == MICF_EUNSUPPORTED) {
    for (int i = 0; i < ngroups; ++i) {
      rc = micf_conv3_fwd(cs[i].x1, C, cs[i].x2, C, cs[i].w, cs[i].bias, cs[i].y, 0, B, D, H, W, kOffsetHidden, nullptr, 0, 0, dtype, stream);
      if (rc != MICF_OK) return rc;
    }
  }
  if (rc != MICF_OK || conv_only) return rc;
  return offset_sample_fwd_groups(ss, ngroups, B, D, H, W, C, eps, s);
}

extern "C" int64_t micf_offset_head_bwd_workspace(int ngroups, int B, int D, int H, int W) {
  return ngroups > 0 ? ngroups * micf_offset_sample_bwd_workspace(B, D, H, W) : 0;
}

static int head_bwd_sets(const micf_offset_head_bwd_group* groups, int ngroups, SampleBwdSet* ss) {
  for (int i = 0; i < ngroups; ++i) {
    const micf_offset_head_bwd_group& g = groups[i];
    if (!g.dxs || !g.hid || !g.flow || !g.xa || !g.ln_g || !g.ln_b || !g.w1 || !g.conv_w || !g.dxa || !g.dxn || !g.dhid || !g.dln_g ||
        !g.dln_b || !g.dw1)
      return MICF_EINVAL;
    ss[i] = SampleBwdSet{g.dxs, g.hid, g.ln_g, g.ln_b, g.w1, g.xa, g.flow, g.dxa, g.dhid, g.dln_g, g.dln_b, g.dw1,
                         CellLists{nullptr, nullptr, nullptr, nullptr, 0, nullptr}, nullptr};
  }
  return MICF_OK;
}

extern "C" int micf_offset_head_bwd_finish(const micf_offset_head_bwd_group* groups, int ngroups, int B, int D, int H, int W, int C,
                                           float* workspace, int64_t workspace_floats, micf_stream_t stream) {
  if (!groups || ngroups < 1 || ngroups > 2 || !micf_offset_head_finish_deferrable(B, D, H, W)) return MICF_EINVAL;
  SampleBwdSet ss[2];
  const int rc = head_bwd_sets(groups, ngroups, ss);
  if (rc != MICF_OK) return rc;
  return offset_sample_bwd_groups(ss, ngroups, B, D, H, W, C, 0.f, workspace, workspace_floats, (hipStream_t)stream, 2);
}

extern "C" int micf_offset_head_bwd_finish_grouped(const micf_offset_head_finish_call* calls, int ncalls, micf_stream_t stream) {
  constexpr int kMax = 16;
  if (!calls || ncalls < 1 || ncalls > kMax) return MICF_EINVAL;
  SampleBwdSet ss[kMax][2];
  SampleFinishCall fc[kMax];
  for (int c = 0; c < ncalls; ++c) {
    const micf_offset_head_finish_call& q = calls[c];
    if (!q.groups || q.ngroups < 1 || q.ngroups > 2 || !micf_offset_head_finish_deferrable(q.B, q.D, q.H, q.W)) return MICF_EINVAL;
    const int rc = head_bwd_sets(q.groups, q.ngroups, ss[c]);
    if (rc != MICF_OK) return rc;
    fc[c] = SampleFinishCall{ss[c], q.ngroups, q.B, q.D, q.H, q.W, q.C, q.workspace, q.workspace_floats};
  }
  return offset_sample_finish_many(fc, ncalls, (hipStream_t)stream);
}

extern "C" int micf_offset_head_bwd(const micf_offset_head_bwd_group* groups, int ngroups, int B, int D, int H, int W, int C,
                                    float eps, int prepared, float* workspace, int64_t workspace_floats, int dtype,
                                    int defer_finish, micf_stream_t stream) {
  if (!groups || ngroups < 1 || ngroups > 2 || B <= 0 || D <= 0 || H <= 0 || W <= 0 || C <= 0) return MICF_EINVAL;
  if (dtype != MICF_DTYPE_F32 && dtype != MICF_DTYPE_BF16) return MICF_EINVAL;
  hipStream_t s = (hipStream_t)stream;
  SampleBwdSet ss[2];
  Conv3BwdSet cs[2];
  for (int i = 0; i < ngroups; ++i) {
    const micf_offset_head_bwd_group& g = groups[i];
    if (!g.dxs || !g.hid || !g.flow || !g.xa || !g.ln_g || !g.ln_b || !g.w1 || !g.conv_w || !g.dxa || !g.dxn || !g.dhid || !g.dln_g ||
        !g.dln_b || !g.dw1)
      return MICF_EINVAL;
    ss[i] = SampleBwdSet{g.dxs, g.hid, g.ln_g, g.ln_b, g.w1, g.xa, g.flow, g.dxa, g.dhid, g.dln_g, g.dln_b, g.dw1,
                         CellLists{nullptr, nullptr, nullptr, nullptr, 0, nullptr}, nullptr};
    cs[i] = Conv3BwdSet{g.dhid, g.conv_w, g.conv_ws, g.dxn, g.dxa};
  }
  int rc = offset_sample_bwd_groups(ss, ngroups, B, D, H, W, C, eps, workspace, workspace_floats, s, defer_finish ? 1 : 0);
  if (rc != MICF_OK) return rc;
  rc = MICF_EUNSUPPORTED;
  if (groups[0].conv_ws && (ngroups == 1 || groups[1].conv_ws))
    rc = conv3_bwd_data_x_groups(cs, ngroups, C, 1, C, 1, B, D, H, W, kOffsetHidden, s, dtype, prepared);
  if (rc == MICF_EUNSUPPORTED) {
    for (int i = 0; i < ngroups; ++i) {
      rc = micf_conv3_bwd_data(cs[i].dy, 0, cs[i].w, cs[i].dx1, C, 1, cs[i].dx2, C, 1, B, D, H, W, kOffsetHidden, nullptr, 0, 0, dtype, stream);
      if (rc != MICF_OK) return rc;
    }
  }
  return rc;
}
```

micformer_amd/csrc/offset_sample.hip:

```cpp
#include <stdio.h>
#include <stdlib.h>

#include "common.h"
#include "sampler_common.h"

namespace micf {

static inline int tok_per_wave(int64_t T) { return T >= 32768 ? 8 : (T >= 4096 ? 2 : 1); }
static inline int quads_per_wave(int64_t T) { return T >= 32768 ? 2 : 1; }
static inline int quad_waves_per_block(int64_t T) { return T >= 16384 ? 4 : 1; }

__device__ __forceinline__ void offset_sample_fwd_body(const float* __restrict__ h, const float* __restrict__ ln_g,
                                                                const float* __restrict__ ln_b, const float* __restrict__ w1,
                                                                const float* __restrict__ xa, float* __restrict__ flow_out,
                                                                float* __restrict__ xs, Geo g, int C, float eps, int tpw) {
  const int lane = threadIdx.x & 63, wave = threadIdx.x >> 6, k = lane & 15;
  const int64_t T = g.tokens();
  for (int it = 0; it < tpw; ++it) {
    const int64_t t = ((int64_t)blockIdx.x * 4 + wave) * tpw + it;
    if (t >= T) return;
    float xh, rs, ln, gl, off[3];
    head_fwd(h + t * kHid, ln_g, ln_b, w1, eps, k, xh, rs, ln, gl, off);
    int b, d, hh, w; g.decode((int)t, b, d, hh, w);
    float fl[3];
// ... 460 lines not shown
  const int z_lo = max(oz - E, 0), y_lo = max(oy - E, 0), x_lo = max(ox - E, 0);
  const int nzc = min(oz + ez - 1 + E, g.D - 1) - z_lo + 1, nyc = min(oy + ey - 1 + E, g.H - 1) - y_lo + 1,
            nxc = min(ox + ex - 1 + E, g.W - 1) - x_lo + 1, ncand = nzc * nyc * nxc;
  const float fz0 = (float)oz, fz1 = (float)(oz + ez - 1), fy0 = (float)oy, fy1 = (float)(oy + ey - 1), fx0 = (float)ox,
              fx1 = (float)(ox + ex - 1);
  bool spilled = false;
  for (int i0 = tid; i0 < ncand; i0 += 256 * 4) {
    int tk[4], cd[4], ch[4], cw[4];
    float fl[4][3];
#pragma unroll
    for (int u = 0; u < 4; ++u) {
      const int i = i0 + 256 * u, ic = i < ncand ? i : i0;
      const int x = ic % nxc, r = ic / nxc;
      cd[u] = z_lo + r / nyc; ch[u] = y_lo + r % nyc; cw[u] = x_lo + x;
      tk[u] = g.token(b, cd[u], ch[u], cw[u]);
      const float* f = q.flow + (int64_t)tk[u] * 3;
      fl[u][0] = f[0]; fl[u][1] = f[1]; fl[u][2] = f[2];
    }
#pragma unroll
    for (int u = 0; u < 4; ++u) {
      if (i0 + 256 * u >= ncand) continue;
      const Taps tp = make_taps(cd[u], ch[u], cw[u], fl[u], g.D, g.H, g.W);
      if (!near_token(tp, cd[u], ch[u], cw[u], E)) continue;
      if (!(tp.z0 + 1.f >= fz0 && tp.z0 <= fz1 && tp.y0 + 1.f >= fy0 && tp.y0 <= fy1 && tp.x0 + 1.f >= fx0 && tp.x0 <= fx1)) continue;
      const float4 hr = make_float4(__int_as_float(tk[u]), tp.cz, tp.cy, tp.cx);
      const int slot = atomicAdd(cnt, 1);
      if (slot < ts.hit_cap) {
        hits[slot] = hr;
        const int cell = (((int)tp.z0 - oz + 1) * cy_n + ((int)tp.y0 - oy + 1)) * cx_n + ((int)tp.x0 - ox + 1);
        const int cs = atomicAdd(ccnt + cell, 1);
        if (cs < ts.cell_cap) clist[cell * kCellCap2 + cs] = (unsigned short)slot;
        continue;
      }
      spilled = true;
      const int64_t boff = (int64_t)b * g.D * g.H * g.W * C;
#pragma unroll
      for (int c = 0; c < 8; ++c) {
        const int dz = c >> 2, dy = (c >> 1) & 1, dx = c & 1;
        const float z = tp.z0 + dz, y = tp.y0 + dy, xx = tp.x0 + dx;
        if (!(z >= fz0 && z <= fz1 && y >= fy0 && y <= fy1 && xx >= fx0 && xx <= fx1)) continue;
        const float wq = corner_weight(hr, dz, dy, dx);
        float* dst = q.dxa + boff + (int64_t)(((int)z * g.H + (int)y) * g.W + (int)xx) * C;
        const float* src = q.dxs + (int64_t)tk[u] * C;
        for (int cc = 0; cc < C; ++cc) atomicAdd(dst + cc, wq * src[cc]);
      }
    }
  }
  if (__syncthreads_or(spilled)) __threadfence();
  const int nh = min(cnt[0], ts.hit_cap);
  for (int i = tid; i < 2 * nvox; i += 256) {
    const int v = i >> 1, dz = i & 1;
    const int lx = v % ex, r = v / ex;
    const int ly = r % ey, lz = r / ey;
    float2* seg = vlist + (v * 2 + dz) * kVoxSeg;
    int n = 0;
    bool over = false;
#pragma unroll
    for (int c = 0; c < 4; ++c) {
      const int dy = c >> 1, dx = c & 1;
      const int cell = ((lz - dz + 1) * cy_n + (ly - dy + 1)) * cx_n + (lx - dx + 1);
      const int cn = ccnt[cell];
      over = over || cn > ts.cell_cap;
      for (int j = 0; j < min(cn, ts.cell_cap); ++j) {
        const float4 hr = hits[clist[cell * kCellCap2 + j]];
        if (n < ts.seg_cap) seg[n] = make_float2(hr.x, corner_weight(hr, dz, dy, dx));
        ++n;
      }
    }
    vcnt[v * 2 + dz] = (over || n > ts.seg_cap) ? -1 : n;
  }
  __syncthreads();
  const int nitem = nvox * q4;
  for (int i0 = tid; i0 < nitem; i0 += 512) {
    float4 acc[2];
    int vv[2], cc4[2];
#pragma unroll
    for (int w = 0; w < 2; ++w) {
      const int i = i0 + 256 * w < nitem ? i0 + 256 * w : i0;
      vv[w] = i / q4; cc4[w] = (i - vv[w] * q4) * 4;
      acc[w] = make_float4(0.f, 0.f, 0.f, 0.f);
    }
    const int n00 = vcnt[2 * vv[0]], n01 = vcnt[2 * vv[0] + 1], n10 = vcnt[2 * vv[1]], n11 = vcnt[2 * vv[1] + 1];
    if (n00 >= 0 && n01 >= 0 && n10 >= 0 && n11 >= 0) {
      const int na = n00 + n01, nb = n10 + n11;
      for (int base = 0; base < max(na, nb); base += 8) {
        float4 go[2][8]; float wq[2][8];
#pragma unroll
        for (int w = 0; w < 2; ++w) {
          const float2* l0 = vlist + vv[w] * 2 * kVoxSeg;
          const int n0 = w ? n10 : n00, n = w ? nb : na;
#pragma unroll
          for (int u = 0; u < 8; ++u) {
            const int idx = base + u;
            const bool on = idx < n;
            const float2 e = l0[on ? (idx < n0 ? idx : kVoxSeg + idx - n0) : 0];
            wq[w][u] = on ? e.y : 0.f;
            go[w][u] = ld4(q.dxs + (int64_t)(on ? __float_as_int(e.x) : 0) * C + cc4[w]);
          }
        }
#pragma unroll
        for (int w = 0; w < 2; ++w)
#pragma unroll
          for (int u = 0; u < 8; ++u) {
            acc[w].x += wq[w][u] * go[w][u].x; acc[w].y += wq[w][u] * go[w][u].y;
            acc[w].z += wq[w][u] * go[w][u].z; acc[w].w += wq[w][u] * go[w][u].w;
          }
      }
    } else {
#pragma unroll
      for (int w = 0; w < 2; ++w) {
        const int lx = vv[w] % ex, r = vv[w] / ex;
        const float vz = (float)(oz + r / ey), vy = (float)(oy + r % ey), vx = (float)(ox + lx);
        for (int j = 0; j < nh; ++j) {
          const float4 hr = hits[j];
          const float dz = vz - floorf(hr.y), dy = vy - floorf(hr.z), dx = vx - floorf(hr.w);
          if (!(dz >= 0.f && dz <= 1.f && dy >= 0.f && dy <= 1.f && dx >= 0.f && dx <= 1.f)) continue;
          const float wq = corner_weight(hr, (int)dz, (int)dy, (int)dx);
          const float4 go = ld4(q.dxs + (int64_t)__float_as_int(hr.x) * C + cc4[w]);
          acc[w].x += wq * go.x; acc[w].y += wq * go.y; acc[w].z += wq * go.z; acc[w].w += wq * go.w;
        }
      }
    }
#pragma unroll
    for (int w = 0; w < 2; ++w) {
      if (i0 + 256 * w >= nitem) continue;
      const int lx = vv[w] % ex, r = vv[w] / ex;
      const int64_t tok = g.token(b, oz + r / ey, oy + r % ey, ox + lx);
      float4* dst = reinterpret_cast<float4*>(q.dxa + tok * C + cc4[w]);
      float4 o = *dst;
      o.x += acc[w].x; o.y += acc[w].y; o.z += acc[w].z; o.w += acc[w].w;
      *dst = o;
    }
  }
}

__global__ void __launch_bounds__(256) sample_gather_tile_kernel(const SampleBwdSets p, Geo g, int C, TileShape ts) {
  gather_tile_body(p.s[blockIdx.y], g, C, ts, (int)blockIdx.x);
}

template <bool QUAD>
__global__ void __launch_bounds__(256) sample_bwd_fused_kernel(const SampleBwdSets p, Geo g, int C, float eps, int tpw, int nwaves,
                                                               TileShape ts, int token_blocks) {
  const SampleBwdSet& q = p.s[blockIdx.y];
  if ((int)blockIdx.x >= token_blocks)
    gather_tile_body(q, g, C, ts, (int)blockIdx.x - token_blocks);
  else if (QUAD)
    offset_sample_bwd4_body<kTile>(q.dxs, q.h, q.ln_g, q.ln_b, q.w1, q.xa, q.flow, q.dxa, q.dh, q.dln_g, q.dln_b, q.dw1, g, C, eps, tpw, q.cl,
                                   q.partials, nwaves, ts.e, (int)blockIdx.x);
  else
    offset_sample_bwd_body<kTile>(q.dxs, q.h, q.ln_g, q.ln_b, q.w1, q.xa, q.flow, q.dxa, q.dh, q.dln_g, q.dln_b, q.dw1, g, C, eps, tpw, q.cl,
                                  q.partials, nwaves, ts.e, (int)blockIdx.x);
}

__global__ void __launch_bounds__(256) sample_gather_kernel(const SampleBwdSets p, Geo g, int C) {
  const SampleBwdSet& q = p.s[blockIdx.y];
  sample_gather_body(q.dxs, q.flow, q.dxa, g, C, q.cl);
}
__global__ void __launch_bounds__(256) sample_finish_kernel(const SampleBwdSets p, Geo g, int C, int nwaves) {
  const SampleBwdSet& q = p.s[blockIdx.y];
  sample_finish_body(q.dxs, q.flow, q.dxa, g, C, q.cl, q.partials, nwaves, q.dw1, q.dln_g, q.dln_b);
}

constexpr int kFinishMany = 32;
struct FinishSets { const float* partials[kFinishMany]; float* dw1[kFinishMany]; float* dln_g[kFinishMany]; float* dln_b[kFinishMany]; int nwaves[kFinishMany]; };
__global__ void __launch_bounds__(256) sample_finish_many_kernel(const FinishSets f, const Geo unit) {
  const int k = blockIdx.y;
  const CellLists none{nullptr, nullptr, nullptr, nullptr, 0, nullptr};
  sample_finish_body(nullptr, nullptr, nullptr, unit, 0, none, f.partials[k], f.nwaves[k], f.dw1[k], f.dln_g[k], f.dln_b[k]);
}

__global__ void __launch_bounds__(256) stn_fwd_kernel(const float* __restrict__ src, const float* __restrict__ flow,
                                                      float* __restrict__ out, Geo g, int C) {
  const int lane = threadIdx.x & 63, wave = threadIdx.x >> 6;
  const int64_t t = (int64_t)blockIdx.x * 4 + wave;
  if (t >= g.tokens()) return;
  int b, d, hh, w; g.decode((int)t, b, d, hh, w);
  const float fl[3] = {flow[t * 3 + 0], flow[t * 3 + 1], flow[t * 3 + 2]};
  const Taps tp = make_taps(d, hh, w, fl, g.D, g.H, g.W);
  const float* base = src + (int64_t)b * g.D * g.H * g.W * C;
  int lin[8]; float wgt[8]; bool ok[8];
#pragma unroll
  for (int q = 0; q < 8; ++q) {
    const int dz = q >> 2, dy = (q >> 1) & 1, dx = q & 1;
    ok[q] = tp.finite && corner(tp, dz, dy, dx, g.D, g.H, g.W, lin[q]);
    const float wx = dx ? tp.cx - tp.x0 : (tp.x0 + 1.f) - tp.cx;
    const float wy = dy ? tp.cy - tp.y0 : (tp.y0 + 1.f) - tp.cy;
    const float wz = dz ? tp.cz - tp.z0 : (tp.z0 + 1.f) - tp.cz;
    wgt[q] = wx * wy * wz;
  }
  for (int c = lane; c < C; c += 64) {
    float acc = 0.f;
#pragma unroll
    for (int q = 0; q < 8; ++q)
      if (ok[q]) acc += base[(int64_t)lin[q] * C + c] * wgt[q];
    out[t * C + c] = acc;
  }
}

__global__ void __launch_bounds__(256) stn_bwd_kernel(const float* __restrict__ dout, const float* __restrict__ src,
                                                      const float* __restrict__ flow, float* __restrict__ dsrc,
                                                      float* __restrict__ dflow, Geo g, int C) {
  const int lane = threadIdx.x & 63, wave = threadIdx.x >> 6;
  const int64_t t = (int64_t)blockIdx.x * 4 + wave;
  if (t >= g.tokens()) return;
  int b, d, hh, w; g.decode((int)t, b, d, hh, w);
  const float fl[3] = {flow[t * 3 + 0], flow[t * 3 + 1], flow[t * 3 + 2]};
  const Taps tp = make_taps(d, hh, w, fl, g.D, g.H, g.W);
  const int64_t boff = (int64_t)b * g.D * g.H * g.W * C;
  int lin[8]; bool ok[8]; float wx[8], wy[8], wz[8];
#pragma unroll
  for (int q = 0; q < 8; ++q) {
    const int dz = q >> 2, dy = (q >> 1) & 1, dx = q & 1;
    ok[q] = tp.finite && corner(tp, dz, dy, dx, g.D, g.H, g.W, lin[q]);
    wx[q] = dx ? tp.cx - tp.x0 : (tp.x0 + 1.f) - tp.cx;
    wy[q] = dy ? tp.cy - tp.y0 : (tp.y0 + 1.f) - tp.cy;
    wz[q] = dz ? tp.cz - tp.z0 : (tp.z0 + 1.f) - tp.cz;
  }
  float gz = 0.f, gy = 0.f, gx = 0.f;
  for (int c = lane; c < C; c += 64) {
    const float go = dout[t * C + c];
#pragma unroll
    for (int q = 0; q < 8; ++q) {
      if (!ok[q]) continue;
      const int dz = q >> 2, dy = (q >> 1) & 1, dx = q & 1;
      const int64_t a = boff + (int64_t)lin[q] * C + c;
      if (dsrc) atomicAdd(dsrc + a, wx[q] * wy[q] * wz[q] * go);
      const float val = src[a] * go;
      gx += (dx ? val : -val) * wy[q] * wz[q];
      gy += (dy ? val : -val) * wx[q] * wz[q];
      gz += (dz ? val : -val) * wx[q] * wy[q];
    }
  }
  gz = wave_sum(gz); gy = wave_sum(gy); gx = wave_sum(gx);
  if (dflow && lane == 0) {
    dflow[t * 3 + 0] = (2.f * ((float)g.D / 2.f * gz)) / (float)(g.D - 1);
    dflow[t * 3 + 1] = (2.f * ((float)g.H / 2.f * gy)) / (float)(g.H - 1);
    dflow[t * 3 + 2] = (2.f * ((float)g.W / 2.f * gx)) / (float)(g.W - 1);
  }
}

}
using namespace micf;

int micf::offset_sample_fwd_groups(const SampleFwdSet* sets, int n, int B, int D, int H, int W, int C, float eps, hipStream_t stream) {
  if (!sets || n < 1 || n > 2 || B <= 0 || D <= 0 || H <= 0 || W <= 0 || C <= 0) return MICF_EINVAL;
  SampleFwdSets p;
  bool al = true;
  for (int i = 0; i < 2; ++i) {
    p.s[i] = sets[i < n ? i : 0];
    const SampleFwdSet& q = p.s[i];
    if (!q.h || !q.ln_g || !q.ln_b || !q.w1 || !q.xa || !q.flow || !q.xs) return MICF_EINVAL;
    al = al && aligned16(q.xa) && aligned16(q.xs);
  }
  const Geo g{B, D, H, W};
  if (g.tokens() >= (1LL << 31)) return MICF_EUNSUPPORTED;
  if (g.tokens() >= 4096 && C % 4 == 0 && al) {
    const int qpw = quads_per_wave(g.tokens());
    const int wpb = quad_waves_per_block(g.tokens());
    hipLaunchKernelGGL(offset_sample_fwd4_kernel, dim3(ceil_div(g.tokens(), 4 * wpb * qpw), n), dim3(64 * wpb), 0, stream, p, g, C, eps, qpw);
    MICF_RETURN_LAUNCH();
  }
  const int tpw = tok_per_wave(g.tokens());
  const int blocks = ceil_div(g.tokens(), 4 * tpw);
  hipLaunchKernelGGL(offset_sample_fwd_kernel, dim3(blocks, n), dim3(256), 0, stream, p, g, C, eps, tpw);
  MICF_RETURN_LAUNCH();
}

extern "C" int micf_offset_sample_fwd(const float* h, const float* ln_g, const float* ln_b, const float* w1,
                                      const float* xa, float* flow, float* xs, int B, int D, int H, int W, int C,
                                      float eps, micf_stream_t stream) {
  const SampleFwdSet one{h, ln_g, ln_b, w1, xa, flow, xs};
  return offset_sample_fwd_groups(&one, 1, B, D, H, W, C, eps, (hipStream_t)stream);
}

static int64_t cell_count(int B, int D, int H, int W) { return (int64_t)B * (D + 1) * (H + 1) * (W + 1); }
static int64_t partial_floats(int64_t T) {
  const int64_t waves = ceil_div(T, (int64_t)4 * tok_per_wave(T)) * 4;
  return (5 * kHid * waves + 3) / 4 * 4;
}
static bool use_cells(int64_t T) { return T >= 4096; }

static bool tile_shape(const Geo& g, int C, TileShape& ts, size_t& lds_bytes) {
  const Options& opt = options();
  if (opt.sample_tile == 0) return false;
  const bool e_hook = opt.sample_e >= 0;
  const int e_env = e_hook ? opt.sample_e : 3;
  const int64_t T = g.tokens();
  int td = 4, th = 4, tw = 8;
  if (T < 32768) td = 2;
  if (T < 4096) { th = 2; tw = 4; }
  ts.td = td < g.D ? td : g.D; ts.th = th < g.H ? th : g.H; ts.tw = tw < g.W ? tw : g.W;
  ts.e = e_env < 0 ? 0 : (e_env > 8 ? 8 : e_env);
  ts.whole = (!e_hook && (int64_t)g.D * g.H * g.W <= (int64_t)kHitCap) ? 1 : 0;
  if (ts.whole) ts.e = g.D > g.H ? (g.D > g.W ? g.D : g.W) : (g.H > g.W ? g.H : g.W);
  ts.nz = ceil_div(g.D, ts.td); ts.ny = ceil_div(g.H, ts.th); ts.nx = ceil_div(g.W, ts.tw);
  const int64_t nt = (int64_t)g.B * ts.nz * ts.ny * ts.nx;
  if (nt >= (1LL << 28)) return false;
  ts.ntiles = (int)nt;
  auto cap = [](int hook, int full) { return hook < 0 ? full : (hook > full ? full : hook); };
  ts.hit_cap = cap(opt.tile_cap_hits, kHitCap); ts.seg_cap = cap(opt.tile_cap_voxel, kVoxSeg); ts.cell_cap = cap(opt.tile_cap_cell, kCellCap2);
  const size_t maxvox = (size_t)ts.td * ts.th * ts.tw, maxcell = (size_t)(ts.td + 1) * (ts.th + 1) * (ts.tw + 1);
  lds_bytes = (size_t)kHitCap * 16 + maxvox * 2 * kVoxSeg * 8 + maxvox * 2 * 4 + maxcell * 4 + 16 + maxcell * kCellCap2 * 2 + 16;
  return true;
}

struct BwdShape { bool quad, tiles, fused; int tpw, wpb, blocks; TileShape ts; size_t tile_lds; };
static void bwd_shape(const Geo& g, int C, bool al, BwdShape& sh) {
  const int64_t T = g.tokens();
  sh.quad = T >= 4096 && (C % 4 == 0) && al;
  sh.tile_lds = 0;
  sh.tiles = (C % 4 == 0) && al && tile_shape(g, C, sh.ts, sh.tile_lds);
  sh.fused = sh.tiles && sh.ts.whole;
  sh.tpw = sh.quad ? quads_per_wave(T) : tok_per_wave(T);
  sh.wpb = sh.quad ? (sh.fused ? 4 : quad_waves_per_block(T)) : 4;
  sh.blocks = ceil_div(T, (sh.quad ? 4 * sh.wpb : 4) * sh.tpw);
}

extern "C" int64_t micf_offset_sample_bwd_workspace(int B, int D, int H, int W) {
  if (B <= 0 || D <= 0 || H <= 0 || W <= 0) return 0;
  const int64_t T = (int64_t)B * D * H * W;
  int64_t need = partial_floats(T);
  if (use_cells(T)) {
    const int64_t nc = (cell_count(B, D, H, W) + 3) / 4 * 4;
    need += nc + 4 + nc * kCellCap + T + 8 * T;
  }
  return need;
}

int micf::offset_sample_bwd_groups(SampleBwdSet* sets, int n, int B, int D, int H, int W, int C, float eps, float* workspace,
                             int64_t workspace_floats, hipStream_t s, int phase) {
  if (!sets || n < 1 || n > 2 || B <= 0 || D <= 0 || H <= 0 || W <= 0 || C <= 0) return MICF_EINVAL;
  const Geo g{B, D, H, W};
  const int64_t T = g.tokens();
  if (T >= (1LL << 31) / 4) return MICF_EUNSUPPORTED;
  if ((int64_t)D * H * W * C >= (1LL << 31)) return MICF_EUNSUPPORTED;
  bool al = true;
  for (int i = 0; i < n; ++i) {
    const SampleBwdSet& q = sets[i];
    if (!q.dxs || !q.h || !q.ln_g || !q.ln_b || !q.w1 || !q.xa || !q.flow || !q.dxa || !q.dh || !q.dln_g || !q.dln_b || !q.dw1)
      return MICF_EINVAL;
    al = al && aligned16(q.dxs) && aligned16(q.xa) && aligned16(q.dxa);
  }
  BwdShape sh;
  bwd_shape(g, C, al, sh);
  const bool quad = sh.quad, tiles = sh.tiles, fused = sh.fused;
  const int tpw = sh.tpw, wpb = sh.wpb, blocks = sh.blocks, nwaves = sh.blocks * sh.wpb;
  const TileShape& ts = sh.ts;
  const size_t tile_lds = sh.tile_lds;
  const CellLists none{nullptr, nullptr, nullptr, nullptr, 0, nullptr};
  const int64_t per = micf_offset_sample_bwd_workspace(B, D, H, W);
  const bool have_ws = workspace && workspace_floats >= per * n && aligned16(workspace);
  const bool cells = !tiles && have_ws && use_cells(T) && quad && cell_count(B, D, H, W) * kCellCap < (1LL << 31);
  SampleBwdSets p;
  const int64_t nc = (cell_count(B, D, H, W) + 3) / 4 * 4;
  int* counters = have_ws ? reinterpret_cast<int*>(workspace + n * partial_floats(T)) : nullptr;
  int* lists = counters ? counters + n * (nc + 4) : nullptr;
  int cap = options().cell_cap;
  cap = cap < 0 ? kCellCap : (cap > kCellCap ? kCellCap : cap);
  for (int i = 0; i < 2; ++i) {
    const int k = i < n ? i : 0;
    p.s[i] = sets[k];
    p.s[i].partials = have_ws ? workspace + k * partial_floats(T) : nullptr;
    p.s[i].cl = none;
    if (cells) {
      int* cnt = counters + k * (nc + 4);
      int* ls = lists + k * (nc * kCellCap + T);
      float* w8 = reinterpret_cast<float*>(lists + n * (nc * kCellCap + T)) + (int64_t)k * 8 * T;
      p.s[i].cl = CellLists{cnt, cnt + nc, ls, ls + nc * kCellCap, cap, w8};
    }
  }
  if (phase == 2) {
    if (!have_ws) return MICF_EINVAL;
    hipLaunchKernelGGL(sample_finish_kernel, dim3(5 * kHid, n), dim3(256), 0, s, p, g, C, nwaves);
    MICF_RETURN_LAUNCH();
  }
  if (cells && hipMemsetAsync(counters, 0, sizeof(int) * (size_t)(n * (nc + 4)), s) != hipSuccess) return MICF_ELAUNCH;
  const int mode = tiles ? kTile : (cells ? kCells : kScatter);
  const dim3 grid(blocks, n), blk(64 * wpb);
  if (fused) {
    const int tb = 8 * ((ts.ntiles + 7) / 8);
    if (quad) hipLaunchKernelGGL(sample_bwd_fused_kernel<true>, dim3(blocks + tb, n), dim3(256), tile_lds, s, p, g, C, eps, tpw, nwaves, ts, blocks);
    else hipLaunchKernelGGL(sample_bwd_fused_kernel<false>, dim3(blocks + tb, n), dim3(256), tile_lds, s, p, g, C, eps, tpw, nwaves, ts, blocks);
    if (hipGetLastError() != hipSuccess) return MICF_ELAUNCH;
    if (!have_ws || phase == 1) return MICF_OK;
    hipLaunchKernelGGL(sample_finish_kernel, dim3(5 * kHid, n), dim3(256), 0, s, p, g, C, nwaves);
    MICF_RETURN_LAUNCH();
  }
  if (quad) {
    if (mode == kTile) hipLaunchKernelGGL(offset_sample_bwd4_kernel<kTile>, grid, blk, 0, s, p, g, C, eps, tpw, nwaves, ts.e);
    else if (mode == kCells) hipLaunchKernelGGL(offset_sample_bwd4_kernel<kCells>, grid, blk, 0, s, p, g, C, eps, tpw, nwaves, 0);
    else hipLaunchKernelGGL(offset_sample_bwd4_kernel<kScatter>, grid, blk, 0, s, p, g, C, eps, tpw, nwaves, 0);
  } else {
    if (mode == kTile) hipLaunchKernelGGL(offset_sample_bwd_kernel<kTile>, grid, blk, 0, s, p, g, C, eps, tpw, nwaves, ts.e);
    else hipLaunchKernelGGL(offset_sample_bwd_kernel<kScatter>, grid, blk, 0, s, p, g, C, eps, tpw, nwaves, 0);
  }
  if (hipGetLastError() != hipSuccess) return MICF_ELAUNCH;
  if (tiles) {
    hipLaunchKernelGGL(sample_gather_tile_kernel, dim3((unsigned)(8 * ((ts.ntiles + 7) / 8)), n), dim3(256), tile_lds, s, p, g, C, ts);
    if (hipGetLastError() != hipSuccess) return MICF_ELAUNCH;
  }
  if (!have_ws) return MICF_OK;
  if (cells) {
    const int64_t threads = T * (C / 4);
    hipLaunchKernelGGL(sample_gather_kernel, dim3((unsigned)((threads + 255) / 256), n), dim3(256), 0, s, p, g, C);
    if (hipGetLastError() != hipSuccess) return MICF_ELAUNCH;
  }
  if (phase == 1) return MICF_OK;
  hipLaunchKernelGGL(sample_finish_kernel, dim3(5 * kHid, n), dim3(256), 0, s, p, g, C, nwaves);
  MICF_RETURN_LAUNCH();
}

extern "C" int micf_offset_head_finish_deferrable(int B, int D, int H, int W) {
  return (B <= 0 || D <= 0 || H <= 0 || W <= 0) ? 0 : 1;
}

extern "C" int micf_offset_sample_bwd(const float* dxs, const float* h, const float* ln_g, const float* ln_b,
                                      const float* w1, const float* xa, const float* flow, float* dxa, float* dh,
                                      float* dln_g, float* dln_b, float* dw1, int B, int D, int H, int W, int C, float eps,
                                      float* workspace, int64_t workspace_floats, micf_stream_t stream) {
  SampleBwdSet one{dxs, h, ln_g, ln_b, w1, xa, flow, dxa, dh, dln_g, dln_b, dw1, CellLists{nullptr, nullptr, nullptr, nullptr, 0, nullptr}, nullptr};
  return offset_sample_bwd_groups(&one, 1, B, D, H, W, C, eps, workspace, workspace_floats, (hipStream_t)stream);
}

extern "C" int micf_stn_fwd(const float* src, const float* flow, float* out, int B, int D, int H, int W, int C,
                            micf_stream_t stream) {
  if (!src || !flow || !out || B <= 0 || D <= 0 || H <= 0 || W <= 0 || C <= 0) return MICF_EINVAL;
  const Geo g{B, D, H, W};
  if (g.tokens() >= (1LL << 31)) return MICF_EUNSUPPORTED;
  hipLaunchKernelGGL(stn_fwd_kernel, dim3(ceil_div(g.tokens(), 4)), dim3(256), 0, (hipStream_t)stream, src, flow, out, g, C);
  MICF_RETURN_LAUNCH();
}

extern "C" int micf_stn_bwd(const float* dout, const float* src, const float* flow, float* dsrc, float* dflow, int B, int D,
                            int H, int W, int C, micf_stream_t stream) {
  if (!dout || !src || !flow || (!dsrc && !dflow) || B <= 0 || D <= 0 || H <= 0 || W <= 0 || C <= 0) return MICF_EINVAL;
  const Geo g{B, D, H, W};
  if (g.tokens() >= (1LL << 31)) return MICF_EUNSUPPORTED;
  hipLaunchKernelGGL(stn_bwd_kernel, dim3(ceil_div(g.tokens(), 4)), dim3(256), 0, (hipStream_t)stream, dout, src, flow, dsrc,
                     dflow, g, C);
  MICF_RETURN_LAUNCH();
}

int micf::offset_sample_finish_many(const SampleFinishCall* calls, int ncalls, hipStream_t s) {
  if (!calls || ncalls < 1) return MICF_EINVAL;
  FinishSets f;
  int total = 0;
  for (int c = 0; c < ncalls; ++c) {
    const SampleFinishCall& q = calls[c];
    if (!q.sets || q.n < 1 || q.n > 2 || q.B <= 0 || q.D <= 0 || q.H <= 0 || q.W <= 0) return MICF_EINVAL;
    const Geo g{q.B, q.D, q.H, q.W};
    const int64_t T = g.tokens();
    const int64_t per = micf_offset_sample_bwd_workspace(q.B, q.D, q.H, q.W);
    if (!q.workspace || q.workspace_floats < per * q.n || !aligned16(q.workspace)) return MICF_EINVAL;
    bool al = true;
    for (int i = 0; i < q.n; ++i) al = al && aligned16(q.sets[i].dxs) && aligned16(q.sets[i].xa) && aligned16(q.sets[i].dxa);
    BwdShape sh;
    bwd_shape(g, q.C, al, sh);
    const int blocks = sh.blocks, wpb = sh.wpb;
    for (int i = 0; i < q.n; ++i) {
      if (total == kFinishMany) {
        hipLaunchKernelGGL(sample_finish_many_kernel, dim3(5 * kHid, total), dim3(256), 0, s, f, Geo{1, 1, 1, 1});
        if (hipGetLastError() != hipSuccess) return MICF_ELAUNCH;
        total = 0;
      }
      f.partials[total] = q.workspace + i * partial_floats(T);
      f.dw1[total] = q.sets[i].dw1; f.dln_g[total] = q.sets[i].dln_g; f.dln_b[total] = q.sets[i].dln_b;
      f.nwaves[total] = blocks * wpb;
      ++total;
    }
  }
  hipLaunchKernelGGL(sample_finish_many_kernel, dim3(5 * kHid, total), dim3(256), 0, s, f, Geo{1, 1, 1, 1});
  MICF_RETURN_LAUNCH();
}
```

micformer_amd/functional.py:

```python
import torch

from . import ops
from . import _lib
from ._lib import block_region

_zl = torch.zeros_like


def _in_block(fn):
    import functools

    @functools.wraps(fn)
    def wrapped(*a, **k):
        with block_region():
            return fn(*a, **k)
    return wrapped


def effective_window(dims, window):
    return tuple(d if d <= w else w for d, w in zip(dims, window))


def _padded(dims, ws):
    return tuple(d + (-d) % w for d, w in zip(dims, ws))
# ... 875 lines not shown
        return 0
    return ops.block_tile_tokens(dims, C, heads, P["mlp.fc1.weight"].shape[0])


import os as _os
FUSE_BLOCKS = True


def _queue_block_wgrads(side, P, G, attn, sv, bo, dy, xn, kv_in, s1, s2, rps):
    if bo.get("dy16") is not None:
        dy, xn = bo["dy16"], sv["xn"]
        kv_in = sv["kvs16"] if sv.get("kvs16") is not None else sv["xn"]
    _lin_wgrad(side, dy, sv["g"], G["mlp.fc2.weight"], G["mlp.fc2.bias"], s2, rps)
    _lin_wgrad(side, bo["dh"], sv["xn2"], G["mlp.fc1.weight"], G["mlp.fc1.bias"])
    _lin_wgrad(side, bo["dx1"], sv["o"], G[f"{attn}.proj.weight"], G[f"{attn}.proj.bias"], s1, rps)
    _lin_wgrad(side, bo["dq"], xn, G[f"{attn}.q.weight"], G[f"{attn}.q.bias"])
    _lin_wgrad(side, bo["dkv"], kv_in, G[f"{attn}.kv.weight"], G[f"{attn}.kv.bias"])


def _ln_partials(side, part, tiles, C, dg, db):
    item = (part, tiles, C, dg, db)
    lst = _ln_defer(side)
    if lst is not None:
        lst.append(item)
    elif _LOCAL is not None:
        _LOCAL[1].append(item)
    else:
        ops.layernorm_bwd_finish([item])


FUSE_NEXT_LN = True


def _self_fwd_fused(xs, Ps, scales, dims, heads, eps, save=True, next_ln=None):
    C = xs[0].shape[1]
    groups = [{"x": x, "kvsrc": None, "P": P, "attn": "self_attn", "s1": s[0], "s2": s[1]} for x, P, s in zip(xs, Ps, scales)]
    if next_ln is None:
        return ops.block_fwd(groups, dims, C, heads, eps, (C // heads) ** -0.5, save=save)
    hid = None
    if ops.offset_head_needs_zero(dims, C):
        hid = torch.empty((len(xs), xs[0].shape[0], 16), dtype=torch.float32, device=xs[0].device)
    for i, gd in enumerate(groups):
        gd["next_ln"] = (next_ln[i][0], next_ln[i][1], hid[i] if hid is not None else None)
    return ops.block_fwd(groups, dims, C, heads, eps, (C // heads) ** -0.5, save=save), hid


LAZY_LN_DEFAULT = True


def lazy_ln_pending():
    return len(CTX.lazy_ln)


def _self_bwd_fused(dys, xs, svs, Ps, Gs, scales, dims, heads, sides):
    C = xs[0].shape[1]
    rps = dims[1] * dims[2] * dims[3]
    groups = [{"dy": dy, "x": x, "x1": sv["x1"], "stats": sv["stats"], "q": sv["q"], "kv": sv["kv"], "h": sv["h"], "xn2": sv["xn2"], "P": P,
               "attn": "self_attn", "s1": s[0], "s2": s[1], "cross": False} for dy, x, sv, P, s in zip(dys, xs, svs, Ps, scales)]
    pres = [CTX.lazy_ln.pop(dy.data_ptr(), None) for dy in dys]
    for gd, pre in zip(groups, pres):
        if pre is not None:
            if tuple(pre["d"].shape) != tuple(gd["dy"].shape):
                raise RuntimeError("parked LayerNorm backward does not match the gradient it was parked for")
            gd["pre"] = pre
    bos = ops.block_bwd(groups, dims, C, heads, (C // heads) ** -0.5)
    for bo, pre in zip(bos, pres):
        if pre is not None:
            _ln_partials(pre["side"], bo["pre_part"], bo["tiles"], C, pre["dgamma"], pre["dbeta"])
    for dy, sv, bo, P, G, s, side in zip(dys, svs, bos, Ps, Gs, scales, sides):
        _queue_block_wgrads(side, P, G, "self_attn", sv, bo, dy, sv["xn"], sv["xn"], s[0], s[1], rps)
        _ln_partials(side, bo["ln2_part"], bo["tiles"], C, G["norm2.weight"], G["norm2.bias"])
        _ln_partials(side, bo["ln1_part"], bo["tiles"], C, G["norm1.weight"], G["norm1.bias"])
    return [bo["dx"] for bo in bos]


_SV_KEYS = ("xn", "q", "kv", "o", "x1", "xn2", "h", "g", "stats")


class SelfPairFn(torch.autograd.Function):

    @staticmethod
    @_in_block
    def forward(ctx, x, xa, sa1, sa2, sb1, sb2, heads, eps, grad_mode, *params):
        n = len(SELF_KEYS)
        Ps = [dict(zip(SELF_KEYS, params[:n])), dict(zip(SELF_KEYS, params[n:]))]
        x, xa = _c(x), _c(xa)
        B, D, H, W, C = x.shape
        dims = (B, D, H, W)
        xs = [x.reshape(-1, C), xa.reshape(-1, C)]
        _lib.set_unit("self_fwd", 2, xs[0].shape[0], C)
        scales = [(sa1, sa2), (sb1, sb2)]
        save = bool(grad_mode) and any(ctx.needs_input_grad)
        nl, CTX.next_ln, CTX.next_ln_out = CTX.next_ln, None, None
        if nl is not None and FUSE_NEXT_LN and GROUP_CROSS_HEADS and ops.block_fuses_sampler(C, heads) \
                and all(t.numel() == C and t.device == x.device for pr in nl for t in pr):
            svs, hid = _self_fwd_fused(xs, Ps, scales, dims, heads, eps, save=save, next_ln=nl)
            CTX.next_ln_out = ((svs[0]["y"].data_ptr(), svs[1]["y"].data_ptr()), [svs[0]["nln"], svs[1]["nln"]], hid)
        else:
            svs = _self_fwd_fused(xs, Ps, scales, dims, heads, eps, save=save)
        if save:
            ctx.save_for_backward(*xs, *[sv[k] for sv in svs for k in _SV_KEYS], sa1, sa2, sb1, sb2, *params)
            ctx.meta = (dims, heads)
            ctx.tg = _targets(params)
        return svs[0]["y"].reshape(x.shape), svs[1]["y"].reshape(x.shape)

    @staticmethod
    @_in_block
    def backward(ctx, dy, dya):
        sv = ctx.saved_tensors
        dims, heads = ctx.meta
        n, m = len(SELF_KEYS), len(_SV_KEYS)
        xs = list(sv[:2])
        svs = [dict(zip(_SV_KEYS, sv[2:2 + m])), dict(zip(_SV_KEYS, sv[2 + m:2 + 2 * m]))]
        sa1, sa2, sb1, sb2 = sv[2 + 2 * m:6 + 2 * m]
        params = sv[6 + 2 * m:]
        Ps = [dict(zip(SELF_KEYS, params[:n])), dict(zip(SELF_KEYS, params[n:]))]
        tgs = [ctx.tg[:n], ctx.tg[n:]]
        Gs = [_grad_bufs(P, tg) for P, tg in zip(Ps, tgs)]
        sides = [all(t is not None for t in tg) for tg in tgs]
        C = xs[0].shape[1]
        _lib.set_unit("self_bwd", 2, xs[0].shape[0], C)
        dys = [_c(dy).reshape(-1, C), _c(dya).reshape(-1, C)]
        with _local_batch():
            dxs = _self_bwd_fused(dys, xs, svs, Ps, Gs, [(sa1, sa2), (sb1, sb2)], dims, heads, sides)
        shape = dims + (C,)
        grads = tuple(_ret(t, G[k]) for G, tg in zip(Gs, tgs) for k, t in zip(SELF_KEYS, tg))
        return (dxs[0].reshape(shape), dxs[1].reshape(shape), None, None, None, None, None, None, None) + grads


def _cross_head_fwd(xf, xaf, P, dims, eps):
    xn, m1, r1 = ops.layernorm_fwd(xf, P["norm1.weight"], P["norm1.bias"], eps)
    hid = ops.conv3_fwd(xn, P["conv_offset.0.weight"], P["conv_offset.0.bias"], dims, x2=xaf)
    flow, xs = ops.offset_sample_fwd(hid, P["conv_offset.1.norm.weight"], P["conv_offset.1.norm.bias"], P["conv_offset.3.weight"], xaf,
                                     dims, eps)
    return xn, m1, r1, hid, flow, xs


def _cross_head_bwd(side, P, G, dims, eps, xf, xaf, xn, m1, r1, hid, flow, dxq, dxs, dxa_acc, add, out=None):
    C = xf.shape[1]
    dhid = ops.offset_sample_bwd(dxs, hid, P["conv_offset.1.norm.weight"], P["conv_offset.1.norm.bias"], P["conv_offset.3.weight"],
                                 xaf, flow, dxa_acc, G["conv_offset.1.norm.weight"], G["conv_offset.1.norm.bias"],
                                 G["conv_offset.3.weight"], dims, eps)
    _defer_conv_wgrad(side, dhid, xn, xaf, G["conv_offset.0.weight"], G["conv_offset.0.bias"], dims)
    ops.conv3_bwd_data(dhid, P["conv_offset.0.weight"], dims, C, C, dx1=dxq, dx2=dxa_acc, acc1=True, acc2=True)
    return ops.layernorm_bwd(dxq, xf, m1, r1, P["norm1.weight"], G["norm1.weight"], G["norm1.bias"], add=add, defer=_ln_defer(side),
                             out=out)


_CSV_KEYS = ("q", "kv", "o", "x1", "xn2", "h", "g", "stats", "xn", "kvs16")

OVERLAP_CROSS_HEADS = True
GROUP_CROSS_HEADS = True
FUSE_SAMPLER = True


def _conv_offset_wgrad(side, dhid, xn, xa, G, dims):
    _defer_conv_wgrad(side, dhid, xn, xa, G["conv_offset.0.weight"], G["conv_offset.0.bias"], dims)
_SIDE = {}


def _side_stream(device):
    st = _SIDE.get(device)
    if st is None:
        st = _SIDE[device] = torch.cuda.Stream(device=device)
    return st


def _cross_head_adjoint(i, hds, bos, Ps, Gs, xs, acc, dims, eps, C, sides):
    xn, m1, r1, hid, flow, xsamp = hds[i]
    dhid = ops.offset_sample_bwd(bos[i]["dxs"], hid, Ps[i]["conv_offset.1.norm.weight"], Ps[i]["conv_offset.1.norm.bias"],
                                 Ps[i]["conv_offset.3.weight"], xs[1 - i], flow, acc[1 - i], Gs[i]["conv_offset.1.norm.weight"],
                                 Gs[i]["conv_offset.1.norm.bias"], Gs[i]["conv_offset.3.weight"], dims, eps)
    _defer_conv_wgrad(sides[i], dhid, xn, xs[1 - i], Gs[i]["conv_offset.0.weight"], Gs[i]["conv_offset.0.bias"], dims)
    ops.conv3_bwd_data(dhid, Ps[i]["conv_offset.0.weight"], dims, C, C, dx1=bos[i]["dx"], dx2=acc[1 - i], acc1=True, acc2=True)


class CrossPairFn(torch.autograd.Function):

    @staticmethod
    @_in_block
    def forward(ctx, x, xa, sa1, sa2, sb1, sb2, heads, eps, grad_mode, *params):
        n = len(CROSS_KEYS)
        Ps = [dict(zip(CROSS_KEYS, params[:n])), dict(zip(CROSS_KEYS, params[n:]))]
        x, xa = _c(x), _c(xa)
        ctx.lazy_ln = CTX.cross_after_self == (x.data_ptr(), xa.data_ptr())
        CTX.cross_after_self = None
        B, D, H, W, C = x.shape
        dims = (B, D, H, W)
        xs = [x.reshape(-1, C), xa.reshape(-1, C)]
        _lib.set_unit("cross_fwd", 2, xs[0].shape[0], C)
        fuse_sampler = GROUP_CROSS_HEADS and FUSE_SAMPLER and ops.block_fuses_sampler(C, heads)
        if GROUP_CROSS_HEADS:
            pre, CTX.next_ln_out = CTX.next_ln_out, None
            if pre is not None and pre[0] == (xs[0].data_ptr(), xs[1].data_ptr()):
                lns, hid = pre[1], pre[2]
            else:
                hid = None
                if ops.offset_head_needs_zero(dims, C):
                    hid = torch.empty((2, xs[0].shape[0], 16), dtype=torch.float32, device=x.device)
                lns = ops.layernorm_fwd_pair(xs, [P["norm1.weight"] for P in Ps], [P["norm1.bias"] for P in Ps], eps, zero=hid)
            outs = ops.offset_head_fwd([{"xn": lns[i][0], "xa": xs[1 - i], "P": Ps[i]} for i in (0, 1)], dims, eps, hid,
                                       sample=not fuse_sampler)
            heads_ = [lns[i] + outs[i] for i in (0, 1)]
        elif OVERLAP_CROSS_HEADS:
            main, side = torch.cuda.current_stream(), _side_stream(x.device)
            side.wait_stream(main)
            h0 = _cross_head_fwd(xs[0], xs[1], Ps[0], dims, eps)
            with torch.cuda.stream(side):
                h1 = _cross_head_fwd(xs[1], xs[0], Ps[1], dims, eps)
            main.wait_stream(side)
            for t in h1:
                t.record_stream(main)
            heads_ = [h0, h1]
        else:
            heads_ = [_cross_head_fwd(xs[i], xs[1 - i], Ps[i], dims, eps) for i in (0, 1)]
        scales = [(sa1, sa2), (sb1, sb2)]
        groups = [{"x": xs[i], "kvsrc": heads_[i][5], "P": Ps[i], "attn": "cross_attn", "s1": scales[i][0], "s2": scales[i][1],
                   "want_xn": False} for i in (0, 1)]
        if fuse_sampler:
            for i in (0, 1):
                groups[i].update(kvsrc=None, hid=heads_[i][3], samp_src=xs[1 - i])
        save = bool(grad_mode) and any(ctx.needs_input_grad)
        svs = ops.block_fwd(groups, dims, C, heads, eps, (C // heads) ** -0.5, save=save)
        if not save:
            return svs[0]["y"].reshape(x.shape), svs[1]["y"].reshape(x.shape)
        if fuse_sampler:
            heads_ = [heads_[i][:4] + (svs[i]["flow"], svs[i]["xs32"]) for i in (0, 1)]
        ctx.save_for_backward(*xs, *[t for hd in heads_ for t in hd], *[sv[k] for sv in svs for k in _CSV_KEYS], sa1, sa2, sb1, sb2,
                              *params)
        ctx.meta = (dims, heads, eps)
        ctx.tg = _targets(params)
        return svs[0]["y"].reshape(x.shape), svs[1]["y"].reshape(x.shape)

    @staticmethod
    @_in_block
    @_batched
    def backward(ctx, dy, dya):
        sv = ctx.saved_tensors
        dims, heads, eps = ctx.meta
        n, m = len(CROSS_KEYS), len(_CSV_KEYS)
        xs = list(sv[:2])
        hds = [sv[2:8], sv[8:14]]
        svs = [dict(zip(_CSV_KEYS, sv[14:14 + m])), dict(zip(_CSV_KEYS, sv[14 + m:14 + 2 * m]))]
        sa1, sa2, sb1, sb2 = sv[14 + 2 * m:18 + 2 * m]
        scales = [(sa1, sa2), (sb1, sb2)]
        params = sv[18 + 2 * m:]
        Ps = [dict(zip(CROSS_KEYS, params[:n])), dict(zip(CROSS_KEYS, params[n:]))]
        tgs = [ctx.tg[:n], ctx.tg[n:]]
        Gs = [_grad_bufs(P, tg) for P, tg in zip(Ps, tgs)]
        sides = [all(t is not None for t in tg) for tg in tgs]
        C = xs[0].shape[1]
        _lib.set_unit("cross_bwd", 2, xs[0].shape[0], C)
        rps = dims[1] * dims[2] * dims[3]
        dys = [_c(dy).reshape(-1, C), _c(dya).reshape(-1, C)]
        groups = [{"dy": dys[i], "x": None, "x1": svs[i]["x1"], "stats": svs[i]["stats"], "q": svs[i]["q"], "kv": svs[i]["kv"],
                   "h": svs[i]["h"], "xn2": svs[i]["xn2"], "P": Ps[i], "attn": "cross_attn", "s1": scales[i][0], "s2": scales[i][1], "cross": True,
                   "want_copy": True} for i in (0, 1)]
        bos = ops.block_bwd(groups, dims, C, heads, (C // heads) ** -0.5)
        acc = [bos[0]["dx1_copy"], bos[1]["dx1_copy"]]
        for i in (0, 1):
            xn, m1, r1, hid, flow, xsamp = hds[i]
            _queue_block_wgrads(sides[i], Ps[i], Gs[i], "cross_attn", svs[i], bos[i], dys[i], xn, xsamp, scales[i][0], scales[i][1], rps)
            _ln_partials(sides[i], bos[i]["ln2_part"], bos[i]["tiles"], C, Gs[i]["norm2.weight"], Gs[i]["norm2.bias"])
        if GROUP_CROSS_HEADS:
            hgroups = [{"dxs": bos[i]["dxs"], "hid": hds[i][3], "flow": hds[i][4], "xa": xs[1 - i], "P": Ps[i],
                        "G": Gs[i], "dxa": acc[1 - i], "dxn": bos[i]["dx"]} for i in (0, 1)]
            defer_ws = None
            if all(sides) and CTX.defer_calls and CTX.defer_wgrad and ops.offset_head_finish_deferrable(dims):
                defer_ws = torch.empty(ops.offset_head_bwd_workspace(2, dims), dtype=torch.float32, device=xs[0].device)
            dhids = ops.offset_head_bwd(hgroups, dims, eps, defer_ws=defer_ws)
            if defer_ws is not None:
                def fin():
                    ops.offset_head_bwd_finish(hgroups, dhids, dims, defer_ws)
                fin.finish = (hgroups, dhids, tuple(dims), defer_ws)
                _defer(True, fin, defer_ws, *dhids)
            for i in (0, 1):
                _conv_offset_wgrad(sides[i], dhids[i], hds[i][0], xs[1 - i], Gs[i], dims)
        else:
            main = torch.cuda.current_stream()
            side = _side_stream(dys[0].device) if OVERLAP_CROSS_HEADS else None
            if side is not None:
                side.wait_stream(main)
            for i in (0, 1):
                with torch.cuda.stream(side if (i == 1 and side is not None) else main):
                    _cross_head_adjoint(i, hds, bos, Ps, Gs, xs, acc, dims, eps, C, sides)
            if side is not None:
                main.wait_stream(side)
        lazy = (ctx.lazy_ln and CTX.lazy_ln_ok and GROUP_CROSS_HEADS and all(sides) and CTX.defer_wgrad and bos[0].get("dy16") is not None
                and ops.block_fuses_sampler(C, heads))
        if lazy:
            for i in (0, 1):
                CTX.lazy_ln[acc[i].data_ptr()] = {"d": bos[i]["dx"], "x": xs[i], "mean": hds[i][1], "rstd": hds[i][2],
                                               "gamma": Ps[i]["norm1.weight"], "dgamma": Gs[i]["norm1.weight"],
                                               "dbeta": Gs[i]["norm1.bias"], "side": sides[i]}
        elif GROUP_CROSS_HEADS:
            ops.layernorm_bwd_pair([{"dy": bos[i]["dx"], "x": xs[i], "mean": hds[i][1], "rstd": hds[i][2], "gamma": Ps[i]["norm1.weight"],
                                     "dgamma": Gs[i]["norm1.weight"], "dbeta": Gs[i]["norm1.bias"], "add": acc[i], "out": acc[i]}
                                    for i in (0, 1)], [_ln_defer(sides[i]) for i in (0, 1)])
        else:
            for i in (0, 1):
                xn, m1, r1 = hds[i][:3]
                ops.layernorm_bwd(bos[i]["dx"], xs[i], m1, r1, Ps[i]["norm1.weight"], Gs[i]["norm1.weight"], Gs[i]["norm1.bias"],
                                  add=acc[i], defer=_ln_defer(sides[i]), out=acc[i])
        shape = dims + (C,)
        grads = tuple(_ret(t, G[k]) for G, tg in zip(Gs, tgs) for k, t in zip(CROSS_KEYS, tg))
        return (acc[0].reshape(shape), acc[1].reshape(shape), None, None, None, None, None, None, None) + grads


PATCH_GEMM = True
class PatchEmbedFn(torch.autograd.Function):

    @staticmethod
    def forward(ctx, vol, mod, w, b, p):
        vol = _c(vol)
        B, nmod, D, H, W = vol.shape
        E = w.shape[0]
        if PATCH_GEMM and w.shape[1] == 1 and p in (2, 4):
            a = ops.space_to_depth(vol, (B, D, H, W), 1, p, batch_stride=nmod * D * H * W, offset=mod * D * H * W)
            y = ops.linear_fwd(a, w.reshape(E, p ** 3), b).reshape(B, -(-D // p), -(-H // p), -(-W // p), E)
            ctx.save_for_backward(a, w)
        else:
            y = ops.patch_embed_fwd(vol, mod, w, b, p)
            ctx.save_for_backward(vol, w)
        ctx.meta = (mod, p, PATCH_GEMM and w.shape[1] == 1 and p in (2, 4))
        ctx.tg = _targets((w, b))
        return y

    @staticmethod
    def backward(ctx, dy):
        vol, w = ctx.saved_tensors
        mod, p, gemm = ctx.meta
        dw = _grad_buf(ctx.tg[0], w)
        db = ctx.tg[1] if ctx.tg[1] is not None else torch.zeros(w.shape[0], dtype=w.dtype, device=w.device)
        dy = _c(dy)
        if gemm:
            _lin_wgrad(ctx.tg[0] is not None and ctx.tg[1] is not None, dy.reshape(-1, w.shape[0]), vol, dw.view(w.shape[0], -1), db)
        else:
            _defer(ctx.tg[0] is not None and ctx.tg[1] is not None, lambda: ops.patch_embed_bwd_weight(dy, vol, mod, dw, db, p), dy, vol)
        return None, None, _ret(ctx.tg[0], dw), _ret(ctx.tg[1], db), None


class PatchRowsEmbedFn(torch.autograd.Function):

    @staticmethod
    def forward(ctx, a, w, b):
        E = w.shape[0]
        ctx.save_for_backward(a, w)
        ctx.tg = _targets((w, b))
        return ops.linear_fwd(a, w.reshape(E, -1), b)

    @staticmethod
    def backward(ctx, dy):
        a, w = ctx.saved_tensors
        dw = _grad_buf(ctx.tg[0], w)
        db = ctx.tg[1] if ctx.tg[1] is not None else torch.zeros(w.shape[0], dtype=w.dtype, device=w.device)
        _lin_wgrad(ctx.tg[0] is not None and ctx.tg[1] is not None, _c(dy).reshape(-1, w.shape[0]), a, dw.view(w.shape[0], -1), db)
        return None, _ret(ctx.tg[0], dw), _ret(ctx.tg[1], db)


class PatchEmbedPairFn(torch.autograd.Function):

    @staticmethod
    def forward(ctx, vol, w, b, p):
        vol = _c(vol)
        B, nmod, D, H, W = vol.shape
        E = w.shape[0]
        rows = B * (-(-D // p)) * (-(-H // p)) * (-(-W // p))
        a = torch.empty((2 * rows, p ** 3), dtype=torch.float32, device=vol.device)
        for m in (0, 1):
            ops.space_to_depth(vol, (B, D, H, W), 1, p, batch_stride=nmod * D * H * W, offset=m * D * H * W, out=a[m * rows:(m + 1) * rows])
        ctx.save_for_backward(a, w)
        ctx.tg = _targets((w, b))
        return ops.linear_fwd(a, w.reshape(E, p ** 3), b).reshape(2 * B, -(-D // p), -(-H // p), -(-W // p), E)

    @staticmethod
    def backward(ctx, dy):
        a, w = ctx.saved_tensors
        dw = _grad_buf(ctx.tg[0], w)
        db = ctx.tg[1] if ctx.tg[1] is not None else torch.zeros(w.shape[0], dtype=w.dtype, device=w.device)
        _lin_wgrad(ctx.tg[0] is not None and ctx.tg[1] is not None, _c(dy).reshape(-1, w.shape[0]), a, dw.view(w.shape[0], -1), db)
        return None, _ret(ctx.tg[0], dw), _ret(ctx.tg[1], db), None


SKIP_MAIL = True


class _SkipToken:
    __slots__ = ("grad", "mailed", "received", "consumed")

    def __init__(self):
        self.grad = None
        self.mailed = self.received = 0
        self.consumed = False


def clear_skip_tokens():
    CTX.skip_tokens.clear()


def skip_token(t):
    return CTX.skip_tokens.get((t.data_ptr(), tuple(t.shape))) if SKIP_MAIL else None


class SkipMailFn(torch.autograd.Function):
    @staticmethod
    def forward(ctx, t, token):
        ctx.token = token
        token.mailed += 1
        return t.view_as(t)

    @staticmethod
    def backward(ctx, g):
        tok = ctx.token
        if tok.consumed:
            raise RuntimeError("SkipMailFn.backward ran after the PatchMerging backward that should have added its gradient "
                               "(set functional.SKIP_MAIL = False for backward passes in a non-standard order)")
        tok.grad = g if tok.grad is None else tok.grad + g
        tok.received += 1
        return None, None


class ConvDownFn(torch.autograd.Function):

# ... 207 lines not shown
```

micformer_amd/ops.py:

```python
import ctypes

import torch

from . import _lib
from ._lib import call, f32, ptr


DETAIL = False

_COMPUTE_DTYPE = "fp32"


def compute_dtype():
    return _COMPUTE_DTYPE


def _dt():
    return 1 if _COMPUTE_DTYPE == "bf16" else 0


def set_compute_dtype(name):
    global _COMPUTE_DTYPE, _ATTN_FP8
    if name not in ("fp32", "bf16", "bf16+fp8attn"):
        raise ValueError("compute dtype must be 'fp32', 'bf16' or 'bf16+fp8attn'")
# ... 302 lines not shown
    need = 0 if ncdhw else _lib.lib.micf_conv3_bwd_data_workspace(N, c1, c2)
    ws = _conv_layouts(w)[1] if need > 0 else None
    prepared = 1 if ws is not None else 0
    if ws is None and need > 0:
        ws = scratch(dy.device, need)
    call("micf_conv3_bwd_data", f32(dy), 1 if ncdhw else 0, f32(w), f32(dx1), c1, 1 if acc1 else 0, f32(dx2), c2,
         1 if acc2 else 0, B, D, H, W, N, f32(ws), ws.numel() if ws is not None else 0, prepared, _dt(),
         cost=_cost(2 * T * 27 * (c1 + c2) * N, dy, w, dx1, dx2))
    return dx1, dx2


def conv3_bwd_weight(dy, x1, dw, dbias, dims, x2=None, ncdhw=False):
    B, D, H, W = dims
    c1 = x1.shape[-1]
    c2 = x2.shape[-1] if x2 is not None else 0
    N = dw.shape[0]
    need = 0 if ncdhw else _lib.lib.micf_conv3_bwd_weight_workspace(B, D, H, W, N, c1, c2)
    ws = scratch(dy.device, need) if need > 0 else None
    call("micf_conv3_bwd_weight", f32(dy), 1 if ncdhw else 0, f32(x1), c1, f32(x2), c2, f32(dw), f32(dbias), B, D, H, W, N,
         f32(ws), ws.numel() if ws is not None else 0, _dt(),
         cost=_cost(2 * B * D * H * W * 27 * (c1 + c2) * N, dy, x1, x2, dw))


def conv3_bwd_weight_grouped(items, dims):
    if len(items) == 1:
        dy, x1, x2, dw, db = items[0]
        return conv3_bwd_weight(dy, x1, dw, db, dims, x2=x2)
    B, D, H, W = dims
    dy0, x10, x20, dw0, _ = items[0]
    c1 = x10.shape[-1]
    c2 = x20.shape[-1] if x20 is not None else 0
    N = dw0.shape[0]
    n = len(items)
    arr = (_lib.Conv3WgradItem * n)()
    for k, (dy, x1, x2, dw, db) in enumerate(items):
        assert dy.shape == dy0.shape and x1.shape == x10.shape and dw.shape == dw0.shape
        arr[k].dy, arr[k].x1, arr[k].x2 = f32(dy), f32(x1), f32(x2)
        arr[k].dw, arr[k].dbias = f32(dw), f32(db)
    need = _lib.lib.micf_conv3_bwd_weight_grouped_workspace(n, B, D, H, W, N, c1, c2)
    ws = scratch(dy0.device, need) if need > 0 else None
    flat = [t for it in items for t in it if t is not None]
    call("micf_conv3_bwd_weight_grouped", ctypes.addressof(arr), n, c1, c2, B, D, H, W, N, f32(ws),
         ws.numel() if ws is not None else 0, _dt(),
         cost=_cost(2 * n * B * D * H * W * 27 * (c1 + c2) * N, *flat))


def offset_sample_fwd(h, ln_g, ln_b, w1, xa, dims, eps):
    B, D, H, W = dims
    T, C = xa.shape
    flow = _new(xa, T, 3)
    xs = _new(xa, T, C)
    call("micf_offset_sample_fwd", f32(h), f32(ln_g), f32(ln_b), f32(w1), f32(xa), f32(flow), f32(xs), B, D, H, W, C,
         float(eps),
         cost=_cost(T * (16 * C + 400), h, xa, flow, xs))
    return flow, xs


def offset_sample_bwd(dxs, h, ln_g, ln_b, w1, xa, flow, dxa, dln_g, dln_b, dw1, dims, eps):
    B, D, H, W = dims
    T, C = xa.shape
    dh = _new(xa, T, h.shape[1])
    need = _lib.lib.micf_offset_sample_bwd_workspace(B, D, H, W)
    ws = scratch(xa.device, need) if need > 0 else None
    call("micf_offset_sample_bwd", f32(dxs), f32(h), f32(ln_g), f32(ln_b), f32(w1), f32(xa), f32(flow), f32(dxa), f32(dh),
         f32(dln_g), f32(dln_b), f32(dw1), B, D, H, W, C, float(eps), f32(ws), ws.numel() if ws is not None else 0,
         cost=_cost(T * (40 * C + 800), dxs, h, xa, flow, dxa, dxa, dh))
    return dh


def offset_head_bwd_workspace(n, dims):
    return int(_lib.lib.micf_offset_head_bwd_workspace(n, *dims))


def offset_head_needs_zero(dims, C):
    B, D, H, W = dims
    return bool(_lib.lib.micf_offset_head_needs_zero(B, D, H, W, C))


def offset_head_fwd(groups, dims, eps, hid=None, sample=True):
    B, D, H, W = dims
    T, C = groups[0]["xn"].shape
    n = len(groups)
    zeroed = hid is not None
    if hid is None:
        hid = _new(groups[0]["xn"], n, T, 16)
    arr = (_lib.OffsetHeadGroup * 2)()
    outs, keep, prepared = [], [], None
    for i, (it, gd) in enumerate(zip(arr, groups)):
        P = gd["P"]
        w = P["conv_offset.0.weight"]
        ws = _conv_layouts(w)[0]
        prepared = (ws is not None) if prepared is None else (prepared and ws is not None)
        if ws is None:
            need = _lib.lib.micf_conv3_fwd_workspace(16, C, C)
            ws = _new(w, need) if need > 0 else None
        keep.append(ws)
        flow, xs = (_new(gd["xn"], T, 3), _new(gd["xn"], T, C)) if sample else (None, None)
        it.xn, it.xa, it.conv_w, it.conv_b, it.conv_ws = f32(gd["xn"]), f32(gd["xa"]), f32(w), f32(P["conv_offset.0.bias"]), f32(ws)
        it.ln_g, it.ln_b, it.w1 = f32(P["conv_offset.1.norm.weight"]), f32(P["conv_offset.1.norm.bias"]), f32(P["conv_offset.3.weight"])
        it.hid, it.flow, it.xs = f32(hid[i]), f32(flow), f32(xs)
        outs.append((hid[i], flow, xs))
    if not prepared:
        for it, gd in zip(arr, groups):
            need = _lib.lib.micf_conv3_fwd_workspace(16, C, C)
            ws = _new(gd["xn"], need) if need > 0 else None
            keep.append(ws)
            it.conv_ws = f32(ws)
    call("micf_offset_head_fwd", ctypes.cast(arr, ctypes.c_void_p), n, B, D, H, W, C, float(eps), 1 if prepared else 0,
         1 if zeroed else 0, _dt(), cost=_cost(n * (2 * T * 27 * 2 * C * 16 + (T * (20 * C + 400) if sample else 0)), *[g["xn"] for g in groups],
                                                *[g["xa"] for g in groups], *[o[2] for o in outs], *[o[0] for o in outs]))
    del keep
    return outs


def offset_head_finish_deferrable(dims):
    return bool(_lib.lib.micf_offset_head_finish_deferrable(*dims))


def _head_bwd_array(groups, dhids):
    arr = (_lib.OffsetHeadBwdGroup * 2)()
    for it, gd, dhid in zip(arr, groups, dhids):
        P, G = gd["P"], gd["G"]
        it.dxs, it.hid, it.flow, it.xa = f32(gd["dxs"]), f32(gd["hid"]), f32(gd["flow"]), f32(gd["xa"])
        it.ln_g, it.ln_b, it.w1 = f32(P["conv_offset.1.norm.weight"]), f32(P["conv_offset.1.norm.bias"]), f32(P["conv_offset.3.weight"])
        it.conv_w = f32(P["conv_offset.0.weight"])
        it.dxa, it.dxn, it.dhid = f32(gd["dxa"]), f32(gd["dxn"]), f32(dhid)
        it.dln_g, it.dln_b, it.dw1 = f32(G["conv_offset.1.norm.weight"]), f32(G["conv_offset.1.norm.bias"]), f32(G["conv_offset.3.weight"])
    return arr


def offset_head_bwd_finish(groups, dhids, dims, ws):
    B, D, H, W = dims
    C = groups[0]["xa"].shape[1]
    arr = _head_bwd_array(groups, dhids)
    call("micf_offset_head_bwd_finish", ctypes.cast(arr, ctypes.c_void_p), len(groups), B, D, H, W, C, f32(ws), ws.numel())


def offset_head_bwd_finish_grouped(calls):
    for first in range(0, len(calls), 16):
        part = calls[first:first + 16]
        arr = (_lib.OffsetHeadFinishCall * len(part))()
        keep = []
        for it, (groups, dhids, dims, ws) in zip(arr, part):
            ga = _head_bwd_array(groups, dhids)
            keep.append(ga)
            it.groups = ctypes.cast(ga, ctypes.c_void_p)
            it.ngroups = len(groups)
            it.B, it.D, it.H, it.W = dims
            it.C = groups[0]["xa"].shape[1]
            it.workspace, it.workspace_floats = f32(ws), ws.numel()
        call("micf_offset_head_bwd_finish_grouped", ctypes.addressof(arr), len(part))


def offset_head_bwd(groups, dims, eps, defer_ws=None):
    B, D, H, W = dims
    T, C = groups[0]["xa"].shape
    n = len(groups)
    arr = (_lib.OffsetHeadBwdGroup * 2)()
    outs, keep, prepared = [], [], None
    for it, gd in zip(arr, groups):
        P, G = gd["P"], gd["G"]
        w = P["conv_offset.0.weight"]
        ws = _conv_layouts(w)[1]
        prepared = (ws is not None) if prepared is None else (prepared and ws is not None)
        keep.append(ws)
        dhid = _new(gd["xa"], T, 16)
        it.dxs, it.hid, it.flow, it.xa = f32(gd["dxs"]), f32(gd["hid"]), f32(gd["flow"]), f32(gd["xa"])
        it.ln_g, it.ln_b, it.w1 = f32(P["conv_offset.1.norm.weight"]), f32(P["conv_offset.1.norm.bias"]), f32(P["conv_offset.3.weight"])
        it.conv_w, it.conv_ws = f32(w), f32(ws)
        it.dxa, it.dxn, it.dhid = f32(gd["dxa"]), f32(gd["dxn"]), f32(dhid)
        it.dln_g, it.dln_b, it.dw1 = f32(G["conv_offset.1.norm.weight"]), f32(G["conv_offset.1.norm.bias"]), f32(G["conv_offset.3.weight"])
        outs.append(dhid)
    if not prepared:
        for it, gd in zip(arr, groups):
            need = _lib.lib.micf_conv3_bwd_data_workspace(16, C, C)
            ws = _new(gd["xa"], need) if need > 0 else None
            keep.append(ws)
            it.conv_ws = f32(ws)
    need = _lib.lib.micf_offset_head_bwd_workspace(n, B, D, H, W)
    ws = defer_ws if defer_ws is not None else (scratch(groups[0]["xa"].device, need) if need > 0 else None)
    call("micf_offset_head_bwd", ctypes.cast(arr, ctypes.c_void_p), n, B, D, H, W, C, float(eps), 1 if prepared else 0, f32(ws),
         ws.numel() if ws is not None else 0, _dt(), 1 if defer_ws is not None else 0,
         cost=_cost(n * (2 * T * 27 * 2 * C * 16 + T * (40 * C + 800)), *[g["dxs"] for g in groups], *[g["xa"] for g in groups],
                    *[g["dxa"] for g in groups], *[g["dxa"] for g in groups], *[g["dxn"] for g in groups]))
    del keep
    return outs


def stn_fwd(src, flow, dims):
    B, D, H, W = dims
    out = torch.empty_like(src)
    call("micf_stn_fwd", f32(src), f32(flow), f32(out), B, D, H, W, src.shape[1])
    return out


def stn_bwd(dout, src, flow, dims):
    B, D, H, W = dims
    dsrc = torch.zeros_like(src)
    dflow = torch.empty_like(flow)
    call("micf_stn_bwd", f32(dout), f32(src), f32(flow), f32(dsrc), f32(dflow), B, D, H, W, src.shape[1])
    return dsrc, dflow


def patch_embed_fwd(vol, mod, w, bias, p):
    B, nmod, D, H, W = vol.shape
    E = w.shape[0]
    Dc, Hc, Wc = -(-D // p), -(-H // p), -(-W // p)
    y = _new(vol, B, Dc, Hc, Wc, E)
    call("micf_patch_embed_fwd", f32(vol), nmod, mod, f32(w), f32(bias), f32(y), B, D, H, W, E, p,
         cost=_cost(2 * y.numel() * p ** 3, y, w) if _lib.PROFILE is not None else None)
    return y


def patch_embed_bwd_weight(dy, vol, mod, dw, dbias, p):
    B, nmod, D, H, W = vol.shape
    E = dw.shape[0]
    call("micf_patch_embed_bwd_weight", f32(dy), f32(vol), nmod, mod, f32(dw), f32(dbias), B, D, H, W, E, p,
         cost=_cost(2 * dy.numel() * p ** 3, dy, dw))


def conv_down_fwd(x, w, bias):
    B, D, H, W, C = x.shape
    N = w.shape[0]
    y = _new(x, B, -(-D // 2), -(-H // 2), -(-W // 2), N)
    call("micf_conv_down_fwd", f32(x), f32(w), f32(bias), f32(y), B, D, H, W, C, N,
         cost=_cost(2 * y.numel() * 8 * C, x, w, y))
    return y


def conv_down_bwd_data(dy, w, xshape):
    B, D, H, W, C = xshape
    N = w.shape[0]
    dx = _new(dy, B, D, H, W, C)
    call("micf_conv_down_bwd_data", f32(dy), f32(w), f32(dx), B, D, H, W, C, N,
         cost=_cost(2 * dy.numel() * 8 * C, dy, w, dx))
    return dx


def conv_down_bwd_weight(dy, x, dw, dbias):
    B, D, H, W, C = x.shape
    N = dw.shape[0]
    call("micf_conv_down_bwd_weight", f32(dy), f32(x), f32(dw), f32(dbias), B, D, H, W, C, N,
         cost=_cost(2 * dy.numel() * 8 * C, dy, x, dw))


def conv_up_fwd(x, w, bias, k):
    B, D, H, W, C = x.shape
    N = w.shape[1]
    y = _new(x, B, D * k, H * k, W * k, N)
    call("micf_conv_up_fwd", f32(x), f32(w), f32(bias), f32(y), B, D, H, W, C, N, k,
         cost=_cost(2 * y.numel() * C, x, w, y))
    return y


def head_tail_transposed_up(w_up):
    Ci = w_up.shape[0]
    src = w_up.reshape(Ci, -1)
    dst = _new(w_up, src.shape[1], Ci)
    WeightPrepPlan([(src, None, dst)]).launch()
    return dst


def head_tail_compose(w_up, b_up, w_out, w_up_t=None):
    Ci, Cm, P = w_up.shape[0], w_up.shape[1], w_up.shape[2]
    Co = w_out.shape[0]
    rows = (P + 2) ** 3 * Co
    wb, bf = _new(w_up, rows, Ci), _new(w_up, rows)
    call("micf_head_tail_compose", f32(w_up), f32(b_up), f32(w_out), f32(wb), f32(bf), Ci, Cm, Co, P, f32(w_up_t),
         cost=_cost(2 * rows * (Ci + 1) * Cm * 4, w_up, w_out, wb))
    return wb, bf


def head_tail_fused_supported(dims, Ci, Co, P):
    _, Dc, Hc, Wc = dims
    return bool(_lib.lib.micf_head_tail_fused_supported(Dc, Hc, Wc, Ci, Co, P, _dt()))


def head_tail_pack(wb, bf, b_out, P):
    Ci = wb.shape[1]
    Co = b_out.shape[0]
    pf = torch.empty(_lib.lib.micf_head_tail_pack_bytes(Ci, 0) // 2, dtype=torch.bfloat16, device=wb.device)
    pq = torch.empty(_lib.lib.micf_head_tail_pack_bytes(Ci, 1) // 2, dtype=torch.bfloat16, device=wb.device)
    call("micf_head_tail_pack", f32(wb), f32(bf), f32(b_out), ptr(pf), ptr(pq), Ci, Co, P, cost=_cost(0, wb, pf, pq))
    return pf, pq


def head_tail_fwd_fused(x, pack_fwd, dims, Co, P):
    B, Dc, Hc, Wc = dims
    Ci = x.shape[-1]
    y = _new(x, B, Co, Dc * P, Hc * P, Wc * P)
    call("micf_head_tail_fwd_fused", f32(x), ptr(pack_fwd), f32(y), B, Dc, Hc, Wc, Ci, Co, P,
         cost=_cost(2 * x.shape[0] * (P + 2) ** 3 * Co * Ci, x, y, tag=f"{x.shape[0]}x{Ci}"))
    return y


def head_tail_fwd_fused_sw(x, pack_fwd, out, count, coords, dims, Co, P):
    n, Dc, Hc, Wc = dims
    Ci = x.shape[-1]
    VB, _, VD, VH, VW = out.shape
    assert coords.dtype == torch.int32 and coords.is_contiguous() and tuple(coords.shape) == (n, 4)
    call("micf_head_tail_fwd_fused_sw", f32(x), ptr(pack_fwd), f32(out), f32(count), ptr(coords), n, Dc, Hc, Wc, Ci, Co, P, VB, VD, VH, VW,
         cost=_cost(2 * x.shape[0] * (P + 2) ** 3 * Co * Ci, x, tag=f"{x.shape[0]}x{Ci}"))


def head_tail_fwd_loss_fused(x, pack_fwd, dims, Co, P, target):
    B, Dc, Hc, Wc = dims
    Ci = x.shape[-1]
    y = _new(x, B, Co, Dc * P, Hc * P, Wc * P)
    nparts = int(_lib.lib.micf_head_tail_loss_parts(B, Dc, Hc, Wc))
    part = _new(x, nparts, 32)
    sums = _new(x, Co * 4, dtype=torch.float64)
    loss = _new(x, 1)
    call("micf_head_tail_fwd_loss_fused", f32(x), ptr(pack_fwd), f32(y), ptr(target), 1 if target.dtype == torch.uint8 else 0, f32(part),
         ptr(sums), f32(loss), B, Dc, Hc, Wc, Ci, Co, P,
         cost=_cost(2 * x.shape[0] * (P + 2) ** 3 * Co * Ci + 40 * y.numel(), x, y, target, tag=f"{x.shape[0]}x{Ci}"))
    return y, loss, sums


def head_tail_bwd_data_fused(dy, pack_bwd, dims, Ci, P):
    B, Dc, Hc, Wc = dims
    Co = dy.shape[1]
    dx = _new(dy, B * Dc * Hc * Wc, Ci)
    call("micf_head_tail_bwd_data_fused", f32(dy), ptr(pack_bwd), f32(dx), B, Dc, Hc, Wc, Ci, Co, P,
         cost=_cost(2 * dx.shape[0] * (P + 2) ** 3 * Co * Ci, dy, dx, tag=f"{dx.shape[0]}x{Ci}"))
    return dx


def head_tail_bwd_weight_fused(dy, x, dims, P):
    B, Dc, Hc, Wc = dims
    Ci, Co = x.shape[-1], dy.shape[1]
    need = _lib.lib.micf_head_tail_bwd_weight_fused_workspace(B, Dc, Hc, Wc, Ci)
    if need == 0 or not head_tail_fused_supported(dims, Ci, Co, P):
        return None
    rows = (P + 2) ** 3 * Co
    dwb, dbf = _new(x, rows, Ci), _new(x, rows)
# ... 193 lines not shown
        call("micf_grad_wire_unpack", ptr(src), f32(dst), dst.numel(), cost=_cost(0, dst, dst))


_DT = {"fp32": 0, "bf16": 1}

FWD_W = (("ln1_g", "norm1.weight"), ("ln1_b", "norm1.bias"), ("bq", "{a}.q.bias"), ("bkv", "{a}.kv.bias"), ("bp", "{a}.proj.bias"),
         ("ln2_g", "norm2.weight"), ("ln2_b", "norm2.bias"), ("b1", "mlp.fc1.bias"), ("b2", "mlp.fc2.bias"))
FWD_WM = (("wq", "{a}.q.weight"), ("wkv", "{a}.kv.weight"), ("wp", "{a}.proj.weight"), ("w1", "mlp.fc1.weight"), ("w2", "mlp.fc2.weight"))
BWD_W = (("ln1_g", "norm1.weight"), ("ln2_g", "norm2.weight"))
BWD_WT = (("wqt", "{a}.q.weight"), ("wkvt", "{a}.kv.weight"), ("wpt", "{a}.proj.weight"), ("w1t", "mlp.fc1.weight"),
          ("w2t", "mlp.fc2.weight"))


def block_tile_tokens(dims, C, heads, hidden, backward=False):
    B, D, H, W = dims
    return int(_lib.lib.micf_block_tile_tokens(B, D, H, W, C, heads, hidden, 1 if backward else 0))


def blocked16(w):
    R, Cn = w.shape
    return w.reshape(R // 16, 16, Cn // 16, 16).permute(0, 2, 1, 3).contiguous().reshape(R, Cn)


class WeightPrepPlan:

    def __init__(self, triples, blocked=False):
        self.triples = list(triples)
        self.n = len(self.triples)
        self.arr = (_lib.WeightPrepItem * max(self.n, 1))()
        self.nbytes = 0
        for it, (src, dst, dst_t) in zip(self.arr, self.triples):
            outs = [t for t in (dst, dst_t) if t is not None]
            assert outs and len({t.dtype for t in outs}) == 1 and outs[0].dtype in (torch.float32, torch.bfloat16)
            it.src, it.dst, it.dst_t, it.rows, it.cols = f32(src), ptr(dst), ptr(dst_t), src.shape[0], src.shape[1]
            it.bf16 = (2 if blocked else 1) if outs[0].dtype == torch.bfloat16 else (3 if blocked else 0)
            self.nbytes += src.numel() * (4 + sum(t.element_size() for t in outs))

    def launch(self):
        if self.n:
            call("micf_weight_prep_grouped", ctypes.cast(self.arr, ctypes.c_void_p), self.n,
                 cost=(self.nbytes, 0) if _lib.PROFILE is not None else None)


class Conv3PrepPlan:

    def __init__(self, triples):
        self.triples = list(triples)
        self.n = len(self.triples)
        self.arr = (_lib.Conv3PrepItem * max(self.n, 1))()
        for it, (w, fwd, bwd) in zip(self.arr, self.triples):
            it.w, it.fwd, it.bwd, it.N, it.Cin = f32(w), f32(fwd), f32(bwd), w.shape[0], w.shape[1]

    def launch(self):
        if self.n:
            call("micf_conv3_weight_prep_grouped", ctypes.cast(self.arr, ctypes.c_void_p), self.n)


def conv3_prepared_like(w):
    N, Cin = w.shape[0], w.shape[1]
    nf, nb = _lib.lib.micf_conv3_fwd_workspace(N, Cin, 0), _lib.lib.micf_conv3_bwd_data_workspace(N, Cin, 0)
    mk = lambda n: torch.empty(n, dtype=torch.float32, device=w.device) if n > 0 else None
    return mk(nf), mk(nb)


_SHADOW = {("fp32", False): ("_micf_w32", False, torch.float32), ("fp32", True): ("_micf_wt", True, torch.float32),
           ("bf16", False): ("_micf_w16", False, torch.bfloat16),
           ("bf16", True): ("_micf_wt16", True, torch.bfloat16)}


ENGINE_SHADOWS = False


def shadow_spec(backward):
    return _SHADOW.get((compute_dtype(), bool(backward)))


def shadow_like(w, transposed, dtype):
    return torch.empty((w.shape[1], w.shape[0]) if transposed else tuple(w.shape), dtype=dtype, device=w.device)


PARAM_EPOCH = [0]


def _inference_cache(w, key, build):
    if torch.is_grad_enabled():
        return None
    cache = w.__dict__.setdefault("_micf_cache", {})
    ent = cache.get(key)
    stamp = (w._version, PARAM_EPOCH[0])
    if ent is None or ent[0] != stamp:
        ent = cache[key] = (stamp, build())
    return ent[1]


def _conv_layouts(w):
    f, b = (getattr(w, "_micf_c3f", None), getattr(w, "_micf_c3b", None)) if ENGINE_SHADOWS else (None, None)
    if f is None and b is None and w.dim() == 5 and w.shape[0] <= 16:
        def build():
            fb = conv3_prepared_like(w)
            if fb[0] is not None or fb[1] is not None:
                Conv3PrepPlan([(w, fb[0], fb[1])]).launch()
            return fb
        fb = _inference_cache(w, "conv3", build)
        if fb is not None:
            f, b = fb
    return f, b


def block_weights(P, attn, backward, only=None):
    fields = BWD_WT if backward else FWD_WM
    if only is not None:
        fields = tuple(f for f in fields if f[0] in only)
    spec = shadow_spec(backward)
    if spec is None:
        return {field: P[key.format(a=attn)] for field, key in fields}
    fspec, bspec = shadow_spec(False), shadow_spec(True)
    out, todo = {}, []
    for field, key in fields:
        w = P[key.format(a=attn)]
        sh = getattr(w, spec[0], None) if ENGINE_SHADOWS else None
        if sh is None:
            cache = w.__dict__.setdefault("_micf_cache", {})
            stamp = (w._version, PARAM_EPOCH[0], compute_dtype())
            ent = cache.get("shadows")
            if ent is None or ent[0] != stamp:
                fwd = shadow_like(w, fspec[1], fspec[2]) if fspec is not None else None
                bwd = shadow_like(w, bspec[1], bspec[2])
                ent = cache["shadows"] = (stamp, fwd, bwd)
                todo.append((w, fwd, bwd))
            sh = ent[2] if backward else ent[1]
        out[field] = sh
    if todo:
        WeightPrepPlan(todo, blocked=True).launch()
    return out


def _block_cost(nb, fl, groups, T, C, hidden, self_passes, cross_passes):
    if _lib.PROFILE is None:
        return None
    e = 2 if _dt() else 4
    s8d = 0
    for gd in groups:
        cross = gd.get("cross", gd.get("kvsrc") is not None or gd.get("hid") is not None)
        s8d += (cross_passes if cross else self_passes) * T * C * e + (4 * C * C + 2 * C * hidden) * e
    return (nb, fl, f"{len(groups)}x{T}x{C}" if DETAIL else None, s8d)


def block_fuses_sampler(C, heads):
    return bool(_lib.lib.micf_block_fuses_sampler(C, heads))


def block_saves_bf16(C, heads):
    return bool(_lib.lib.micf_block_saves_bf16(C, heads, _dt()))


def block_recomputes_h(C, heads):
    return bool(_lib.lib.micf_block_recomputes_h(C, heads))


def block_fwd(groups, dims, C, heads, eps, scale, persist_probe=None, save=True):
    B, D, H, W = dims
    T = B * D * H * W
    hidden = groups[0]["P"]["mlp.fc1.weight"].shape[0]
    arr = (_lib.BlockFwdGroup * 2)()
    outs = []
    h_dtype = torch.bfloat16 if _dt() else torch.float32
    st16 = block_saves_bf16(C, heads)
    sd = torch.bfloat16 if st16 else torch.float32
    no_h = block_recomputes_h(C, heads)
    keep = []
    nb = fl = 0
    y_all = _new(groups[0]["x"], len(groups) * T, C)
    for gi, (it, gd) in enumerate(zip(arr, groups)):
        x, P, a = gd["x"], gd["P"], gd["attn"]
        fused_sampler = gd.get("hid") is not None
        cross = gd.get("kvsrc") is not None or fused_sampler
        if not save and block_fuses_sampler(C, heads) and persist_probe is None:
            o = dict.fromkeys(("q", "kv", "o", "x1", "xn2", "h", "g", "stats", "xn", "kvs16", "flow", "xs32"))
            o["y"] = y_all[gi * T:(gi + 1) * T]
        else:
            o = {"y": y_all[gi * T:(gi + 1) * T], "q": _new(x, T, C, dtype=sd), "kv": _new(x, T, 2 * C, dtype=sd),
                 "o": _new(x, T, C, dtype=sd), "x1": _new(x, T, C), "xn2": _new(x, T, C, dtype=sd),
                 "h": None if no_h else _new(x, T, hidden, dtype=h_dtype), "g": _new(x, T, hidden, dtype=sd), "stats": _new(x, 4, T),
                 "xn": _new(x, T, C, dtype=sd) if (gd.get("want_xn", True) or st16) else None,
                 "kvs16": _new(x, T, C, dtype=sd) if (st16 and cross) else None,
                 "flow": _new(x, T, 3) if fused_sampler else None,
                 "xs32": _new(x, T, C) if (fused_sampler and not st16) else None}
        it.x, it.kvsrc, it.s1, it.s2 = f32(x), f32(gd.get("kvsrc")), f32(gd.get("s1")), f32(gd.get("s2"))
        if fused_sampler:
            it.hid, it.samp_src = f32(gd["hid"]), f32(gd["samp_src"])
            it.ln16_g, it.ln16_b, it.w1c = (f32(P[k]) for k in ("conv_offset.1.norm.weight", "conv_offset.1.norm.bias", "conv_offset.3.weight"))
        nl = gd.get("next_ln")
        if nl is not None:
            o["nln"] = (_new(x, T, C), _new(x, T), _new(x, T))
            it.nln_g, it.nln_b, it.zero16 = f32(nl[0]), f32(nl[1]), f32(nl[2])
            it.nln_y, it.nln_mean, it.nln_rstd = (f32(t) for t in o["nln"])
            nb += 4 * T * (C + 2)
        for field, key in FWD_W:
            setattr(it, field, f32(P[key.format(a=a)]))
        wts = block_weights(P, a, backward=False)
        keep.append(wts)
        for field, wt in wts.items():
            setattr(it, field, ptr(wt))
        for k, v in o.items():
            if k != "nln":
                setattr(it, k, ptr(v))
        outs.append(o)
        nb += 4 * T * C * (2 if cross else 1) + (64 * T if fused_sampler else 0) \
            + sum(v.numel() * v.element_size() for k, v in o.items() if v is not None and k != "nln") \
            + 12 * C * C * wt.element_size()
        fl += 2 * T * 12 * C * C + 4 * T * C * 8
    if persist_probe is not None:
        call("micf_block_fwd_persistent_probe", ctypes.cast(arr, ctypes.c_void_p), len(groups), B, D, H, W, C, heads, hidden, float(eps),
             float(scale), _dt(), int(persist_probe[0]), ptr(persist_probe[1]))
        return outs
    call("micf_block_fwd", ctypes.cast(arr, ctypes.c_void_p), len(groups), B, D, H, W, C, heads, hidden, float(eps), float(scale),
         _dt_attn(), cost=_block_cost(nb, fl, groups, T, C, hidden, 2, 3))
    return outs


def block_bwd(groups, dims, C, heads, scale):
    B, D, H, W = dims
    T = B * D * H * W
    hidden = groups[0]["P"]["mlp.fc1.weight"].shape[0]
    tm = block_tile_tokens(dims, C, heads, hidden, backward=True)
    tiles = (T + tm - 1) // tm
    arr = (_lib.BlockBwdGroup * 2)()
    outs = []
    keep = []
    nb = fl = 0
    st16 = block_saves_bf16(C, heads)
    sd = torch.bfloat16 if st16 else torch.float32
    dx_all = _new(groups[0]["dy"], len(groups) * T, C)
    copy_all = _new(groups[0]["dy"], len(groups) * T, C) if all(gd.get("want_copy") for gd in groups) else None
    for gi, (it, gd) in enumerate(zip(arr, groups)):
        dy, P, a, cross = gd["dy"], gd["P"], gd["attn"], gd["cross"]
        o = {"dx": dx_all[gi * T:(gi + 1) * T], "dxs": _new(dy, T, C) if cross else None, "dx1": _new(dy, T, C, dtype=sd),
             "dh": _new(dy, T, hidden, dtype=sd), "dq": _new(dy, T, C, dtype=sd), "dkv": _new(dy, T, 2 * C, dtype=sd),
             "ln2_part": _new(dy, tiles, 2 * C), "ln1_part": None if cross else _new(dy, tiles, 2 * C),
             "dx1_copy": (copy_all[gi * T:(gi + 1) * T] if copy_all is not None else _new(dy, T, C)) if gd.get("want_copy") else None,
             "dy16": _new(dy, T, C, dtype=sd) if st16 else None}
        for k in ("dy", "x", "x1", "stats", "s1", "s2"):
            setattr(it, k, f32(gd.get(k)))
        h = gd.get("h")
        if (h is not None and h.dtype != (torch.bfloat16 if _dt() else torch.float32)) or gd["q"].dtype != sd or gd["kv"].dtype != sd \
                or (h is None and gd["xn2"].dtype != sd):
            raise _lib.MicfError("block_bwd: the saved tensors were written in another arithmetic mode")
        it.h, it.q, it.kv = ptr(h), ptr(gd["q"]), ptr(gd["kv"])
        pre = gd.get("pre")
        if pre is not None:
            if not st16 or cross:
                raise _lib.MicfError("block_bwd: the LayerNorm-backward prologue needs a self block with bf16 storage")
            o["pre_part"] = _new(dy, tiles, 2 * C)
            it.pre_d, it.pre_x, it.pre_mean, it.pre_rstd, it.pre_g, it.pre_part = (f32(pre["d"]), f32(pre["x"]), f32(pre["mean"]),
                                                                                  f32(pre["rstd"]), f32(pre["gamma"]), f32(o["pre_part"]))
            nb += 4 * T * C * 2
        if h is None:
            w1 = block_weights(P, a, backward=False, only=("w1",))["w1"]
            keep.append(w1)
            it.xn2, it.w1, it.b1 = ptr(gd["xn2"]), ptr(w1), f32(P["mlp.fc1.bias"])
        for field, key in BWD_W:
            setattr(it, field, f32(P[key.format(a=a)]))
        wts = block_weights(P, a, backward=True)
        keep.append(wts)
        for field, wt in wts.items():
            setattr(it, field, ptr(wt))
        for k, v in o.items():
            setattr(it, k, ptr(v))
        nb += 4 * T * C * (2 if cross else 3) + sum(gd[k].numel() * gd[k].element_size() for k in ("q", "kv", "h" if h is not None else "xn2")) \
            + sum(v.numel() * v.element_size() for v in o.values() if v is not None) + 12 * C * C * wt.element_size()
        o["tiles"] = tiles
        outs.append(o)
        fl += 2 * T * 12 * C * C + 8 * T * C * 8
    call("micf_block_bwd", ctypes.cast(arr, ctypes.c_void_p), len(groups), B, D, H, W, C, heads, hidden, float(scale),
         _dt(), cost=_block_cost(nb, fl, groups, T, C, hidden, 3, 5))
    del keep
    return outs


def _coords(chunk):
    arr = (ctypes.c_int32 * (4 * len(chunk)))()
    for i, (b, z, y, x) in enumerate(chunk):
        arr[4 * i:4 * i + 4] = [b, z, y, x]
    return arr


def sw_window_batch(vol, chunk, roi):
    B, C, D, H, W = vol.shape
    rd, rh, rw = roi
    win = _new(vol, len(chunk), C, rd, rh, rw)
    arr = _coords(chunk)
    call("micf_sw_window_batch", f32(vol), f32(win), ctypes.cast(arr, ctypes.c_void_p), len(chunk), B, C, D, H, W, rd, rh, rw)
    return win


def sw_accumulate_batch(pred, out, count, chunk):
    B, K, D, H, W = out.shape
    rd, rh, rw = pred.shape[2:]
    arr = _coords(chunk)
    call("micf_sw_accumulate_batch", f32(pred), f32(out), f32(count), ctypes.cast(arr, ctypes.c_void_p), len(chunk), B, K, D, H, W,
         rd, rh, rw)


def intensity_stats(vol):
    B, Cm = vol.shape[:2]
    if vol.dtype not in (torch.float16, torch.float32):
        raise TypeError("raw volume must be float16 or float32")
    sums = torch.empty(B * Cm * 3, dtype=torch.float64, device=vol.device)
    call("micf_intensity_stats", ptr(vol), 1 if vol.dtype == torch.float16 else 0, ptr(sums), B, Cm, vol[0, 0].numel())
    return sums


def patch_rows_prepared(vol, sums, params, k):
    B, Cm, D, H, W = vol.shape
    rows = B * (-(-D // k)) * (-(-H // k)) * (-(-W // k))
    both = torch.empty((Cm * rows, k ** 3), dtype=torch.float32, device=vol.device)
    outs = [both[m * rows:(m + 1) * rows] for m in range(Cm)]
    call("micf_patch_rows_prepared", ptr(vol), 1 if vol.dtype == torch.float16 else 0, ptr(sums), f32(params), f32(outs[0]),
         f32(outs[1]) if Cm > 1 else None, B, Cm, D, H, W, k, cost=_cost(0, vol, *outs))
    return outs


def flip_labels(label_map, params):
    if params is None:
        return label_map
    B, D, H, W = label_map.shape
    out = torch.empty_like(label_map)
    dummy = torch.zeros(3 * B, dtype=torch.float64, device=label_map.device)
    call("micf_input_prepare", ptr(label_map), 0, ptr(dummy), f32(params), None, ptr(label_map), ptr(out), B, 1, D, H, W)
    return out


def input_prepare(vol, label_map=None, params=None):
    B, Cm, D, H, W = vol.shape
    if vol.dtype not in (torch.float16, torch.float32):
        raise TypeError("raw volume must be float16 or float32")
    half = 1 if vol.dtype == torch.float16 else 0
    sums = torch.empty(B * Cm * 3, dtype=torch.float64, device=vol.device)
    call("micf_intensity_stats", ptr(vol), half, ptr(sums), B, Cm, D * H * W)
    out = torch.empty((B, Cm, D, H, W), dtype=torch.float32, device=vol.device)
    lab_out = torch.empty_like(label_map) if label_map is not None else None
    if label_map is not None and label_map.dtype != torch.uint8:
        raise TypeError("label map must be uint8")
    call("micf_input_prepare", ptr(vol), half, ptr(sums), f32(params), f32(out), ptr(label_map), ptr(lab_out), B, Cm, D, H, W)
    return out, lab_out


def zero_(t):
    call("micf_zero", ptr(t), t.numel() * t.element_size())
    return t


def drop_path_rng(device, seed):
    return torch.tensor([int(seed) & 0x7FFFFFFFFFFFFFFF, 0], dtype=torch.int64, device=device)


def drop_path_draw(rng, keep, batch):
    n = keep.numel()
    out = _new(keep, n, batch)
    call("micf_drop_path_draw", ptr(rng), f32(keep), f32(out), n, batch)
    return out
```

Baseline: 234.3 pairs/s.

## Fuse offset-sampler adjoint into cross-attention block backward epilogue

```diff
diff --git a/include/micformer_hip.h b/include/micformer_hip.h
--- a/include/micformer_hip.h
+++ b/include/micformer_hip.h
@@ -313,6 +313,13 @@
   const float *pre_mean, *pre_rstd;
   const float* pre_g;
   float* pre_part;
+  const float* hid;
+  const float* samp_src;
+  const float* flow;
+  const float *ln16_g, *ln16_b, *w1c;
+  const float* ln16_eps;
+  float* dhid;
+  float* samp_ws;
 } micf_block_bwd_group;
 int micf_block_recomputes_h(int C, int heads);
 int micf_block_tile_tokens(int B, int D, int H, int W, int C, int heads, int hidden, int backward);
diff --git a/micformer_amd/_lib.py b/micformer_amd/_lib.py
--- a/micformer_amd/_lib.py
+++ b/micformer_amd/_lib.py
@@ -146,7 +146,8 @@
 class BlockBwdGroup(ctypes.Structure):
     FIELDS = ("dy", "x", "x1", "stats", "q", "kv", "h", "ln1_g", "ln2_g", "wqt", "wkvt", "wpt", "w1t", "w2t", "s1", "s2",
               "dx", "dxs", "dx1", "dh", "dq", "dkv", "ln1_part", "ln2_part", "dx1_copy", "dy16", "xn2", "w1", "b1",
-              "pre_d", "pre_x", "pre_mean", "pre_rstd", "pre_g", "pre_part")
+              "pre_d", "pre_x", "pre_mean", "pre_rstd", "pre_g", "pre_part",
+              "hid", "samp_src", "flow", "ln16_g", "ln16_b", "w1c", "ln16_eps", "dhid", "samp_ws")
     _fields_ = [(n, _VP) for n in FIELDS]
 
 
diff --git a/micformer_amd/csrc/block_bwd.hip b/micformer_amd/csrc/block_bwd.hip
--- a/micformer_amd/csrc/block_bwd.hip
+++ b/micformer_amd/csrc/block_bwd.hip
@@ -9,6 +9,8 @@
   int G, tiles, C, heads, hidden;
   float scale;
   int attn_mfma;
+  float eps16;
+  int part_stride;
 };
 
 template <int TM, int NW, int X4>
@@ -617,7 +619,26 @@
     const void* opt[] = {g.x, g.ln1_g, g.dxs, g.ln1_part, g.ln2_part, g.dx1_copy, g.dy16};
     for (const void* p : opt)
       if (p && (reinterpret_cast<uintptr_t>(p) & 15)) return MICF_EINVAL;
+    if (g.dhid) {
+      const void* sa[] = {g.hid, g.samp_src, g.flow, g.ln16_g, g.ln16_b, g.w1c, g.dhid, g.samp_ws};
+      for (const void* p : sa)
+        if (!p || (reinterpret_cast<uintptr_t>(p) & 15)) return MICF_EINVAL;
+      if (!g.ln16_eps || !g.dxs || g.samp_ws != groups[0].samp_ws) return MICF_EINVAL;
+    }
+    if (i > 0 && (g.dhid == nullptr) != (groups[0].dhid == nullptr)) return MICF_EINVAL;
     a.g[i] = g;
+  }
+  a.eps16 = 0.f; a.part_stride = 0;
+  const bool samp_adj = groups[0].dhid != nullptr;
+  if (samp_adj) {
+    int64_t per = 0;
+    a.eps16 = *groups[0].ln16_eps;
+    a.part_stride = offset_sample_partial_layout(B, D, H, W, C, &per);
+    if (a.part_stride <= 0) return MICF_EUNSUPPORTED;
+    for (int i = 0; i < ngroups; ++i) {
+      if (*groups[i].ln16_eps != a.eps16) return MICF_EINVAL;
+      a.g[i].samp_ws = groups[0].samp_ws + i * per;
+    }
   }
   if (ngroups == 1) a.g[1] = a.g[0];
   a.geo = make_tile_geo(B, D, H, W);
@@ -627,16 +648,18 @@
   hipStream_t s = (hipStream_t)stream;
   const int hd = C / heads, tj = TM / 16;
   if ((int64_t)2 * H * W * (TM / 8 + 1) * hidden * (int64_t)sizeof(float) >= (int64_t)1 << 32) return MICF_EUNSUPPORTED;
-  if (block_wide_tile_tokens(C, hd)) return block_bwd_wide(groups, ngroups, B, D, H, W, C, heads, scale, dtype, s);
+  if (block_wide_tile_tokens(C, hd)) return samp_adj ? MICF_EUNSUPPORTED : block_bwd_wide(groups, ngroups, B, D, H, W, C, heads, scale, dtype, s);
   {
     if (options().block_wave != 0 && C == 48 && hd == 16 && tj == 2 && dtype == MICF_DTYPE_BF16 && a.attn_mfma && a.g[0].h && a.g[1].h && (a.g[0].dxs != nullptr) == (a.g[1].dxs != nullptr) &&
         (a.g[0].pre_d != nullptr) == (a.g[1].pre_d != nullptr) && !(a.g[0].dxs && a.g[0].pre_d) &&
         a.geo.T * (int64_t)hidden * 2 < ((int64_t)1 << 31))
     {
       if (options().block_debug & 1) a.attn_mfma |= 2;
+      if (samp_adj && (a.tiles > a.part_stride || a.geo.T * (int64_t)C * 4 >= ((int64_t)1 << 32))) return MICF_EUNSUPPORTED;
       return wave48::launch_bwd_wave48(a, s);
     }
   }
+  if (samp_adj) return MICF_EUNSUPPORTED;
 #define MICF_BB(C_, HD_, TJ_) if (C == C_ && hd == HD_ && tj == TJ_) return launch_bwd<C_, HD_, TJ_>(a, dtype, s)
   MICF_BB(48, 16, 2); MICF_BB(96, 16, 2); MICF_BB(192, 16, 1);
   MICF_BB(96, 32, 1); MICF_BB(192, 32, 1); MICF_BB(384, 32, 1);
diff --git a/micformer_amd/csrc/block_wave_bwd.h b/micformer_amd/csrc/block_wave_bwd.h
--- a/micformer_amd/csrc/block_wave_bwd.h
+++ b/micformer_amd/csrc/block_wave_bwd.h
@@ -1,6 +1,7 @@
 #pragma once
 
 #include "block_wave.h"
+#include "sampler_common.h"
 
 namespace micf {
 namespace wave48 {
@@ -15,7 +16,8 @@
 constexpr int kBVec = kBKV + 18 * 512;
 constexpr int kBPark = kBVec + 3 * C * 4;
 constexpr int kParkFloats = 4 * (16 * 12 + 8);
-constexpr int kBwdLdsBytes = kBPark + NWAVE * kParkFloats * 4;
+constexpr int kBHead = kBPark + NWAVE * kParkFloats * 4;
+constexpr int kBwdLdsBytes = kBHead + 5 * kHid * 4;
 
 __device__ __forceinline__ void stage_weights_bwd(char* lds, const micf_block_bwd_group& g) {
   const uint16_t* wqt = static_cast<const uint16_t*>(g.wqt), *wkvt = static_cast<const uint16_t*>(g.wkvt), *wpt = static_cast<const uint16_t*>(g.wpt),
@@ -97,6 +99,100 @@
 __device__ __forceinline__ void unpack8(const u32x4v& u, float (&o)[8]) {
 #pragma unroll
   for (int w = 0; w < 4; ++w) { o[2 * w] = __uint_as_float(u[w] << 16); o[2 * w + 1] = __uint_as_float(u[w] & 0xFFFF0000u); }
+}
+
+constexpr int kAdjTapBatch = 8;
+__device__ __forceinline__ void sample_adjoint16(const micf_block_bwd_group& g, const TileGeo& geo, float eps, const float* PH, const Row12& dxs,
+                                                 int gt, int lane, bool store, float* tile, float& pw, float& pgb) {
+  asm volatile("" : "+v"(lane));
+  int gD = geo.D, gH = geo.H, gW = geo.W;
+  asm volatile("" : "+s"(gD), "+s"(gH), "+s"(gW));
+  const int li = lane & 15, lr = lane >> 4;
+  const int win = 2 * gt + (li >> 3);
+  const bool live0 = win < geo.nwin, live = live0 && store;
+  int b = 0, d = 0, hh = 0, w = 0;
+  geo.coords(live0 ? win : 0, li & 7, b, d, hh, w);
+  const uint32_t tk = (uint32_t)(((b * gD + d) * gH + hh) * gW + w);
+  const float4 hv = ld4g(at32(g.hid, (tk * kHid + 4 * lr) * 4u));
+  const float fl[3] = {*at32(g.flow, tk * 12u), *at32(g.flow, tk * 12u + 4u), *at32(g.flow, tk * 12u + 8u)};
+  const float mu = sum4((hv.x + hv.y) + (hv.z + hv.w)) * (1.f / kHid);
+  const float d0 = hv.x - mu, d1 = hv.y - mu, d2 = hv.z - mu, d3 = hv.w - mu;
+  const float rs = 1.0f / sqrtf(sum4((d0 * d0 + d1 * d1) + (d2 * d2 + d3 * d3)) * (1.f / kHid) + eps);
+  const float xh[4] = {d0 * rs, d1 * rs, d2 * rs, d3 * rs};
+  const float4 lg4 = *reinterpret_cast<const float4*>(PH + 4 * lr), lb4 = *reinterpret_cast<const float4*>(PH + kHid + 4 * lr);
+  const float lg[4] = {lg4.x, lg4.y, lg4.z, lg4.w}, lb[4] = {lb4.x, lb4.y, lb4.z, lb4.w};
+  float ln[4], gl[4];
+#pragma unroll
+  for (int i = 0; i < 4; ++i) { ln[i] = xh[i] * lg[i] + lb[i]; gl[i] = gelu_f(ln[i]); }
+  const Taps tp = make_taps(d, hh, w, fl, gD, gH, gW);
+  uint32_t row0 = (uint32_t)b * (uint32_t)(gD * gH * gW);
+  int lin[8]; bool okq[8];
+#pragma unroll
+  for (int q = 0; q < 8; ++q) {
+    lin[q] = 0;
+    okq[q] = tp.finite && corner(tp, q >> 2, (q >> 1) & 1, q & 1, gD, gH, gW, lin[q]);
+  }
+  const float wx1 = tp.cx - tp.x0, wx0 = (tp.x0 + 1.f) - tp.cx, wy1 = tp.cy - tp.y0, wy0 = (tp.y0 + 1.f) - tp.cy,
+              wz1 = tp.cz - tp.z0, wz0 = (tp.z0 + 1.f) - tp.cz;
+  float gz = 0.f, gy = 0.f, gx = 0.f;
+#pragma unroll
+  for (int pc = 0; pc < 3; ++pc) {
+    const int co = pc < 2 ? 8 * lr + 4 * pc : 32 + 4 * lr;
+#pragma unroll
+    for (int q0 = 0; q0 < 8; q0 += kAdjTapBatch) {
+      float4 tv[kAdjTapBatch];
+#pragma unroll
+      for (int u = 0; u < kAdjTapBatch; ++u) tv[u] = ld4g(at32(g.samp_src, ((row0 + (uint32_t)lin[q0 + u]) * C + co) * 4u));
+#pragma unroll
+      for (int u = 0; u < kAdjTapBatch; ++u) {
+        const int q = q0 + u;
+        const bool dz = (q >> 2) != 0, dy = ((q >> 1) & 1) != 0, dx = (q & 1) != 0;
+        const float wx = dx ? wx1 : wx0, wy = dy ? wy1 : wy0, wz = dz ? wz1 : wz0;
+        const float val = tv[u].x * dxs.v[4 * pc] + tv[u].y * dxs.v[4 * pc + 1] + tv[u].z * dxs.v[4 * pc + 2] + tv[u].w * dxs.v[4 * pc + 3];
+        gx += okq[q] ? (dx ? val : -val) * wy * wz : 0.f;
+        gy += okq[q] ? (dy ? val : -val) * wx * wz : 0.f;
+        gz += okq[q] ? (dz ? val : -val) * wx * wy : 0.f;
+      }
+      asm volatile("" : "+v"(row0), "+v"(gx), "+v"(gy), "+v"(gz));
+    }
+  }
+  gz = sum4(gz); gy = sum4(gy); gx = sum4(gx);
+  float go3[3];
+  go3[0] = (2.f * ((float)gD / 2.f * gz)) / (float)(gD - 1);
+  go3[1] = (2.f * ((float)gH / 2.f * gy)) / (float)(gH - 1);
+  go3[2] = (2.f * ((float)gW / 2.f * gx)) / (float)(gW - 1);
+  const float* w1 = PH + 2 * kHid;
+  float dln[4], gd[4];
+#pragma unroll
+  for (int i = 0; i < 4; ++i) {
+    float dgl = 0.f;
+#pragma unroll
+    for (int ax = 0; ax < 3; ++ax) dgl += w1[ax * kHid + 4 * lr + i] * go3[ax];
+    dln[i] = dgl * gelu_grad_f(ln[i]);
+    gd[i] = lg[i] * dln[i];
+  }
+  const float ma = sum4((gd[0] + gd[1]) + (gd[2] + gd[3])) * (1.f / kHid);
+  const float mb = sum4((gd[0] * xh[0] + gd[1] * xh[1]) + (gd[2] * xh[2] + gd[3] * xh[3])) * (1.f / kHid);
+  if (live)
+    *reinterpret_cast<float4*>(at32(g.dhid, (tk * kHid + 4 * lr) * 4u)) =
+        make_float4(rs * (gd[0] - ma - xh[0] * mb), rs * (gd[1] - ma - xh[1] * mb), rs * (gd[2] - ma - xh[2] * mb), rs * (gd[3] - ma - xh[3] * mb));
+  float v[12];
+#pragma unroll
+  for (int ax = 0; ax < 3; ++ax)
+#pragma unroll
+    for (int i = 0; i < 4; ++i) v[4 * ax + i] = live ? go3[ax] * gl[i] : 0.f;
+  park12(tile, lr, li, v);
+  pw += colsum16(tile, lane);
+  asm volatile("" : "+v"(pw));
+#pragma unroll
+  for (int i = 0; i < 4; ++i) { v[i] = live ? dln[i] * xh[i] : 0.f; v[4 + i] = live ? dln[i] : 0.f; }
+  {
+    float* pt = tile + lr * 200 + li * 12;
+    *reinterpret_cast<float4*>(pt) = make_float4(v[0], v[1], v[2], v[3]);
+    *reinterpret_cast<float4*>(pt + 4) = make_float4(v[4], v[5], v[6], v[7]);
+  }
+  pgb += colsum16(tile, lane);
+  asm volatile("" : "+v"(pgb));
 }
 
 template <bool CROSS, bool PRE>
@@ -115,8 +211,13 @@
   const int ngroup16 = (a.geo.nwin + 1) >> 1;
   constexpr bool cross = CROSS, pre = PRE;
   const f32x4 z4 = {0.f, 0.f, 0.f, 0.f};
+  if (cross && g.dhid) {
+    float* PH = reinterpret_cast<float*>(wlds + kBHead);
+    for (int e = tid; e < 5 * kHid; e += NTHR) PH[e] = e < kHid ? g.ln16_g[e] : (e < 2 * kHid ? g.ln16_b[e - kHid] : g.w1c[e - 2 * kHid]);
+  }
   lds_barrier();
 
+  float pw = 0.f, pgb = 0.f;
   for (int unit = wg * NWAVE + wave; unit < a.tiles; unit += nwg * NWAVE) {
     float pg_pre = 0.f, pb_pre = 0.f, pg2 = 0.f, pb2 = 0.f, pg1 = 0.f, pb1 = 0.f;
 #pragma unroll 1
@@ -331,6 +432,8 @@
           dxq.store(at32(g.dx, rowC * 4u), lr);
           dxs.store(at32(g.dxs, rowC * 4u), lr);
         }
+        if (g.dhid)
+          sample_adjoint16(g, a.geo, a.eps16, reinterpret_cast<const float*>(wlds + kBHead), dxs, gt, lane0, !(a.attn_mfma & 2), tile, pw, pgb);
       }
     }
     if (lane0 < C) {
@@ -338,6 +441,18 @@
       if (g.ln2_part) { g.ln2_part[row + lane0] = pg2; g.ln2_part[row + C + lane0] = pb2; }
       if (!cross && g.ln1_part) { g.ln1_part[row + lane0] = pg1; g.ln1_part[row + C + lane0] = pb1; }
       if (pre) { g.pre_part[row + lane0] = pg_pre; g.pre_part[row + C + lane0] = pb_pre; }
+    }
+  }
+  int lane1 = lane0;
+  asm volatile("" : "+v"(lane1));
+  if (cross && g.dhid && lane1 < C) {
+    const int wid = wg * NWAVE + wave, nwb = nwg * NWAVE, e = lane1 & 7;
+    const int row_w = lane1 < 32 ? (e >> 2) * kHid + 4 * (lane1 >> 3) + (e & 3) : lane1;
+    const int row_gb = (3 + (e >> 2)) * kHid + 4 * (lane1 >> 3) + (e & 3);
+    float* part = g.samp_ws;
+    for (int col = wid; col < a.part_stride; col += nwb) {
+      part[(int64_t)row_w * a.part_stride + col] = col == wid ? pw : 0.f;
+      if (lane1 < 32) part[(int64_t)row_gb * a.part_stride + col] = col == wid ? pgb : 0.f;
     }
   }
 }
diff --git a/micformer_amd/csrc/common.h b/micformer_amd/csrc/common.h
--- a/micformer_amd/csrc/common.h
+++ b/micformer_amd/csrc/common.h
@@ -16,6 +16,7 @@
   int block_wave = 1;
   int block_recompute_h = 0;
   int block_debug = 0;
+  int block_sample_bwd = 1;
   int sample_tile = 1;
   int sample_e = -1;
   int cell_cap = -1;
@@ -64,7 +65,8 @@
 };
 int offset_sample_fwd_groups(const SampleFwdSet* sets, int n, int B, int D, int H, int W, int C, float eps, hipStream_t stream);
 int offset_sample_bwd_groups(SampleBwdSet* sets, int n, int B, int D, int H, int W, int C, float eps, float* workspace,
-                             int64_t workspace_floats, hipStream_t s, int phase = 0);
+                             int64_t workspace_floats, hipStream_t s, int phase = 0, bool token_half_done = false);
+int offset_sample_partial_layout(int B, int D, int H, int W, int C, int64_t* per_group);
 struct SampleFinishCall { const SampleBwdSet* sets; int n, B, D, H, W, C; float* workspace; int64_t workspace_floats; };
 int offset_sample_finish_many(const SampleFinishCall* calls, int ncalls, hipStream_t s);
 
diff --git a/micformer_amd/csrc/misc.hip b/micformer_amd/csrc/misc.hip
--- a/micformer_amd/csrc/misc.hip
+++ b/micformer_amd/csrc/misc.hip
@@ -93,6 +93,7 @@
   Options& o = micf::options();
   const struct { const char* n; int* v; } table[] = {
       {"block_wave", &o.block_wave}, {"block_recompute_h", &o.block_recompute_h}, {"block_debug", &o.block_debug},
+      {"block_sample_bwd", &o.block_sample_bwd},
       {"sample_tile", &o.sample_tile}, {"sample_e", &o.sample_e}, {"cell_cap", &o.cell_cap},
       {"tile_cap_hits", &o.tile_cap_hits}, {"tile_cap_cell", &o.tile_cap_cell}, {"tile_cap_voxel", &o.tile_cap_voxel}};
   for (const auto& e : table)
diff --git a/micformer_amd/csrc/offset_head.hip b/micformer_amd/csrc/offset_head.hip
--- a/micformer_amd/csrc/offset_head.hip
+++ b/micformer_amd/csrc/offset_head.hip
@@ -93,7 +93,7 @@
                          CellLists{nullptr, nullptr, nullptr, nullptr, 0, nullptr}, nullptr};
     cs[i] = Conv3BwdSet{g.dhid, g.conv_w, g.conv_ws, g.dxn, g.dxa};
   }
-  int rc = offset_sample_bwd_groups(ss, ngroups, B, D, H, W, C, eps, workspace, workspace_floats, s, defer_finish ? 1 : 0);
+  int rc = offset_sample_bwd_groups(ss, ngroups, B, D, H, W, C, eps, workspace, workspace_floats, s, (defer_finish & 1) ? 1 : 0, (defer_finish & 2) != 0);
   if (rc != MICF_OK) return rc;
   rc = MICF_EUNSUPPORTED;
   if (groups[0].conv_ws && (ngroups == 1 || groups[1].conv_ws))
diff --git a/micformer_amd/csrc/offset_sample.hip b/micformer_amd/csrc/offset_sample.hip
--- a/micformer_amd/csrc/offset_sample.hip
+++ b/micformer_amd/csrc/offset_sample.hip
@@ -636,6 +636,41 @@
                                   q.partials, nwaves, ts.e, (int)blockIdx.x);
 }
 
+__global__ void __launch_bounds__(256) sample_far_scatter_kernel(const SampleBwdSets p, Geo g, int C, int near_e) {
+  const SampleBwdSet& q = p.s[blockIdx.y];
+  const int lane = threadIdx.x & 63;
+  const int64_t T = g.tokens(), t = (int64_t)blockIdx.x * 256 + threadIdx.x;
+  bool far = false;
+  if (t < T) {
+    int b, d, hh, w; g.decode((int)t, b, d, hh, w);
+    const float fl[3] = {q.flow[t * 3 + 0], q.flow[t * 3 + 1], q.flow[t * 3 + 2]};
+    const Taps tp = make_taps(d, hh, w, fl, g.D, g.H, g.W);
+    far = tp.finite && !near_token(tp, d, hh, w, near_e);
+  }
+  unsigned long long m = __ballot(far);
+  while (m) {
+    const int64_t tj = t - lane + (__ffsll(m) - 1);
+    m &= m - 1;
+    int b, d, hh, w; g.decode((int)tj, b, d, hh, w);
+    const float fl[3] = {q.flow[tj * 3 + 0], q.flow[tj * 3 + 1], q.flow[tj * 3 + 2]};
+    const Taps tp = make_taps(d, hh, w, fl, g.D, g.H, g.W);
+    const int64_t boff = (int64_t)b * g.D * g.H * g.W * C;
+    for (int c = lane; c < C; c += 64) {
+      const float go = q.dxs[tj * C + c];
+#pragma unroll
+      for (int k = 0; k < 8; ++k) {
+        const int dz = k >> 2, dy = (k >> 1) & 1, dx = k & 1;
+        int lin;
+        if (!corner(tp, dz, dy, dx, g.D, g.H, g.W, lin)) continue;
+        const float wx = dx ? tp.cx - tp.x0 : (tp.x0 + 1.f) - tp.cx;
+        const float wy = dy ? tp.cy - tp.y0 : (tp.y0 + 1.f) - tp.cy;
+        const float wz = dz ? tp.cz - tp.z0 : (tp.z0 + 1.f) - tp.cz;
+        atomicAdd(q.dxa + boff + (int64_t)lin * C + c, wx * wy * wz * go);
+      }
+    }
+  }
+}
+
 __global__ void __launch_bounds__(256) sample_gather_kernel(const SampleBwdSets p, Geo g, int C) {
   const SampleBwdSet& q = p.s[blockIdx.y];
   sample_gather_body(q.dxs, q.flow, q.dxa, g, C, q.cl);
@@ -800,6 +835,16 @@
   sh.blocks = ceil_div(T, (sh.quad ? 4 * sh.wpb : 4) * sh.tpw);
 }
 
+int micf::offset_sample_partial_layout(int B, int D, int H, int W, int C, int64_t* per_group) {
+  if (B <= 0 || D <= 0 || H <= 0 || W <= 0 || C <= 0) return 0;
+  const Geo g{B, D, H, W};
+  BwdShape sh;
+  bwd_shape(g, C, true, sh);
+  if (!sh.tiles) return 0;
+  if (per_group) *per_group = partial_floats(g.tokens());
+  return sh.blocks * sh.wpb;
+}
+
 extern "C" int64_t micf_offset_sample_bwd_workspace(int B, int D, int H, int W) {
   if (B <= 0 || D <= 0 || H <= 0 || W <= 0) return 0;
   const int64_t T = (int64_t)B * D * H * W;
@@ -812,7 +857,7 @@
 }
 
 int micf::offset_sample_bwd_groups(SampleBwdSet* sets, int n, int B, int D, int H, int W, int C, float eps, float* workspace,
-                             int64_t workspace_floats, hipStream_t s, int phase) {
+                             int64_t workspace_floats, hipStream_t s, int phase, bool token_half_done) {
   if (!sets || n < 1 || n > 2 || B <= 0 || D <= 0 || H <= 0 || W <= 0 || C <= 0) return MICF_EINVAL;
   const Geo g{B, D, H, W};
   const int64_t T = g.tokens();
@@ -858,6 +903,19 @@
     hipLaunchKernelGGL(sample_finish_kernel, dim3(5 * kHid, n), dim3(256), 0, s, p, g, C, nwaves);
     MICF_RETURN_LAUNCH();
   }
+  if (token_half_done) {
+    if (!have_ws) return MICF_EINVAL;
+    if (!tiles) return MICF_EUNSUPPORTED;
+    if (!ts.whole) {
+      hipLaunchKernelGGL(sample_far_scatter_kernel, dim3((unsigned)ceil_div(T, (int64_t)256), n), dim3(256), 0, s, p, g, C, ts.e);
+      if (hipGetLastError() != hipSuccess) return MICF_ELAUNCH;
+    }
+    hipLaunchKernelGGL(sample_gather_tile_kernel, dim3((unsigned)(8 * ((ts.ntiles + 7) / 8)), n), dim3(256), tile_lds, s, p, g, C, ts);
+    if (hipGetLastError() != hipSuccess) return MICF_ELAUNCH;
+    if (phase == 1) return MICF_OK;
+    hipLaunchKernelGGL(sample_finish_kernel, dim3(5 * kHid, n), dim3(256), 0, s, p, g, C, nwaves);
+    MICF_RETURN_LAUNCH();
+  }
   if (cells && hipMemsetAsync(counters, 0, sizeof(int) * (size_t)(n * (nc + 4)), s) != hipSuccess) return MICF_ELAUNCH;
   const int mode = tiles ? kTile : (cells ? kCells : kScatter);
   const dim3 grid(blocks, n), blk(64 * wpb);
diff --git a/micformer_amd/functional.py b/micformer_amd/functional.py
--- a/micformer_amd/functional.py
+++ b/micformer_amd/functional.py
@@ -1051,6 +1051,7 @@
 OVERLAP_CROSS_HEADS = True
 GROUP_CROSS_HEADS = True
 FUSE_SAMPLER = True
+FUSE_SAMPLER_BWD = True
 
 
 def _conv_offset_wgrad(side, dhid, xn, xa, G, dims):
@@ -1155,6 +1156,15 @@
         groups = [{"dy": dys[i], "x": None, "x1": svs[i]["x1"], "stats": svs[i]["stats"], "q": svs[i]["q"], "kv": svs[i]["kv"],
                    "h": svs[i]["h"], "xn2": svs[i]["xn2"], "P": Ps[i], "attn": "cross_attn", "s1": scales[i][0], "s2": scales[i][1], "cross": True,
                    "want_copy": True} for i in (0, 1)]
+        defer_ws = head_ws = None
+        fuse_adj = GROUP_CROSS_HEADS and FUSE_SAMPLER_BWD and ops.block_bwd_runs_sampler_adjoint(C, heads)
+        if GROUP_CROSS_HEADS and all(sides) and CTX.defer_calls and CTX.defer_wgrad and ops.offset_head_finish_deferrable(dims):
+            defer_ws = torch.empty(ops.offset_head_bwd_workspace(2, dims), dtype=torch.float32, device=xs[0].device)
+        if fuse_adj:
+            head_ws = defer_ws if defer_ws is not None else torch.empty(ops.offset_head_bwd_workspace(2, dims), dtype=torch.float32,
+                                                                         device=xs[0].device)
+            for i in (0, 1):
+                groups[i]["samp"] = {"hid": hds[i][3], "samp_src": xs[1 - i], "flow": hds[i][4], "eps": eps, "ws": head_ws}
         bos = ops.block_bwd(groups, dims, C, heads, (C // heads) ** -0.5)
         acc = [bos[0]["dx1_copy"], bos[1]["dx1_copy"]]
         for i in (0, 1):
@@ -1164,10 +1174,10 @@
         if GROUP_CROSS_HEADS:
             hgroups = [{"dxs": bos[i]["dxs"], "hid": hds[i][3], "flow": hds[i][4], "xa": xs[1 - i], "P": Ps[i],
                         "G": Gs[i], "dxa": acc[1 - i], "dxn": bos[i]["dx"]} for i in (0, 1)]
-            defer_ws = None
-            if all(sides) and CTX.defer_calls and CTX.defer_wgrad and ops.offset_head_finish_deferrable(dims):
-                defer_ws = torch.empty(ops.offset_head_bwd_workspace(2, dims), dtype=torch.float32, device=xs[0].device)
-            dhids = ops.offset_head_bwd(hgroups, dims, eps, defer_ws=defer_ws)
+            if fuse_adj:
+                dhids = ops.offset_head_bwd(hgroups, dims, eps, defer_ws=defer_ws, dhids=[bos[i]["dhid"] for i in (0, 1)], ws=head_ws)
+            else:
+                dhids = ops.offset_head_bwd(hgroups, dims, eps, defer_ws=defer_ws)
             if defer_ws is not None:
                 def fin():
                     ops.offset_head_bwd_finish(hgroups, dhids, dims, defer_ws)
diff --git a/micformer_amd/ops.py b/micformer_amd/ops.py
--- a/micformer_amd/ops.py
+++ b/micformer_amd/ops.py
@@ -478,7 +478,7 @@
         call("micf_offset_head_bwd_finish_grouped", ctypes.addressof(arr), len(part))
 
 
-def offset_head_bwd(groups, dims, eps, defer_ws=None):
+def offset_head_bwd(groups, dims, eps, defer_ws=None, dhids=None, ws=None):
     B, D, H, W = dims
     T, C = groups[0]["xa"].shape
     n = len(groups)
@@ -487,26 +487,30 @@
     for it, gd in zip(arr, groups):
         P, G = gd["P"], gd["G"]
         w = P["conv_offset.0.weight"]
-        ws = _conv_layouts(w)[1]
-        prepared = (ws is not None) if prepared is None else (prepared and ws is not None)
-        keep.append(ws)
-        dhid = _new(gd["xa"], T, 16)
+        cws = _conv_layouts(w)[1]
+        prepared = (cws is not None) if prepared is None else (prepared and cws is not None)
+        keep.append(cws)
+        dhid = _new(gd["xa"], T, 16) if dhids is None else dhids[len(outs)]
         it.dxs, it.hid, it.flow, it.xa = f32(gd["dxs"]), f32(gd["hid"]), f32(gd["flow"]), f32(gd["xa"])
         it.ln_g, it.ln_b, it.w1 = f32(P["conv_offset.1.norm.weight"]), f32(P["conv_offset.1.norm.bias"]), f32(P["conv_offset.3.weight"])
-        it.conv_w, it.conv_ws = f32(w), f32(ws)
+        it.conv_w, it.conv_ws = f32(w), f32(cws)
         it.dxa, it.dxn, it.dhid = f32(gd["dxa"]), f32(gd["dxn"]), f32(dhid)
         it.dln_g, it.dln_b, it.dw1 = f32(G["conv_offset.1.norm.weight"]), f32(G["conv_offset.1.norm.bias"]), f32(G["conv_offset.3.weight"])
         outs.append(dhid)
     if not prepared:
         for it, gd in zip(arr, groups):
             need = _lib.lib.micf_conv3_bwd_data_workspace(16, C, C)
-            ws = _new(gd["xa"], need) if need > 0 else None
-            keep.append(ws)
-            it.conv_ws = f32(ws)
+            cws = _new(gd["xa"], need) if need > 0 else None
+            keep.append(cws)
+            it.conv_ws = f32(cws)
     need = _lib.lib.micf_offset_head_bwd_workspace(n, B, D, H, W)
-    ws = defer_ws if defer_ws is not None else (scratch(groups[0]["xa"].device, need) if need > 0 else None)
+    if dhids is not None:
+        if ws is None or (defer_ws is not None and ws is not defer_ws):
+            raise _lib.MicfError("offset_head_bwd: dhids need the workspace block_bwd wrote")
+    else:
+        ws = defer_ws if defer_ws is not None else (scratch(groups[0]["xa"].device, need) if need > 0 else None)
     call("micf_offset_head_bwd", ctypes.cast(arr, ctypes.c_void_p), n, B, D, H, W, C, float(eps), 1 if prepared else 0, f32(ws),
-         ws.numel() if ws is not None else 0, _dt(), 1 if defer_ws is not None else 0,
+         ws.numel() if ws is not None else 0, _dt(), (1 if defer_ws is not None else 0) | (2 if dhids is not None else 0),
          cost=_cost(n * (2 * T * 27 * 2 * C * 16 + T * (40 * C + 800)), *[g["dxs"] for g in groups], *[g["xa"] for g in groups],
                     *[g["dxa"] for g in groups], *[g["dxa"] for g in groups], *[g["dxn"] for g in groups]))
     del keep
@@ -1006,6 +1010,11 @@
 
 def block_saves_bf16(C, heads):
     return bool(_lib.lib.micf_block_saves_bf16(C, heads, _dt()))
+
+
+def block_bwd_runs_sampler_adjoint(C, heads):
+    return (C == 48 and C // heads == 16 and _dt() != 0 and not block_recomputes_h(C, heads)
+            and all(_lib.get_option(k) != 0 for k in ("block_sample_bwd", "block_wave", "sample_tile")))
 
 
 def block_recomputes_h(C, heads):
@@ -1109,6 +1118,17 @@
             it.pre_d, it.pre_x, it.pre_mean, it.pre_rstd, it.pre_g, it.pre_part = (f32(pre["d"]), f32(pre["x"]), f32(pre["mean"]),
                                                                                   f32(pre["rstd"]), f32(pre["gamma"]), f32(o["pre_part"]))
             nb += 4 * T * C * 2
+        samp = gd.get("samp")
+        if samp is not None:
+            if not cross or not block_bwd_runs_sampler_adjoint(C, heads):
+                raise _lib.MicfError("block_bwd: no sampler-adjoint epilogue for this block / shape / arithmetic mode")
+            o["dhid"] = _new(dy, T, 16)
+            eps16 = ctypes.c_float(float(samp["eps"]))
+            keep.append(eps16)
+            it.hid, it.samp_src, it.flow = f32(samp["hid"]), f32(samp["samp_src"]), f32(samp["flow"])
+            it.ln16_g, it.ln16_b, it.w1c = (f32(P[k]) for k in ("conv_offset.1.norm.weight", "conv_offset.1.norm.bias", "conv_offset.3.weight"))
+            it.ln16_eps, it.samp_ws = ctypes.addressof(eps16), f32(samp["ws"])
+            nb += 4 * T * (16 + 3 + 8 * C)
         if h is None:
             w1 = block_weights(P, a, backward=False, only=("w1",))["w1"]
             keep.append(w1)
```

Result: no change. 235.6 pairs/s, median of 6 (+0.5%).
